# liulab-dfci/TRUST4

Measured on AMD Instinct MI355X. Metric: stage-1 assembly read pairs/sec (150 bp PE), whole stage 1, higher is better.
Workload: dtype int32/u64

## Files before the change

trust4_amd/build.py:

```python
import os
import subprocess
import sys

HERE = os.path.dirname(os.path.abspath(__file__))
SRC = os.path.join(HERE, "csrc", "t4_api.hip")
SRC_HOST = os.path.join(HERE, "csrc", "t4_assembler.cpp")
OUT = os.path.join(HERE, "libt4hip.so")
DEPS = [SRC, SRC_HOST, os.path.join(HERE, "host", "trust4_main.cpp"), os.path.join(HERE, "host", "fastq_extractor_main.cpp"),
        os.path.join(HERE, "host", "bam_extractor_main.cpp"), os.path.join(HERE, "host", "bam_reader.h"), os.path.join(HERE, "host", "read_format.h"),
        os.path.join(HERE, "host", "seq_reader.h"), os.path.join(HERE, "host", "process_read.h"), os.path.join(HERE, "csrc", "t4_internal.h"),
        os.path.join(HERE, "csrc", "t4_kernels.h"), os.path.join(HERE, "csrc", "t4_wide.h"), os.path.join(HERE, "csrc", "t4_device.h"),
        os.path.join(os.path.dirname(HERE), "include", "trust4_hip.h")]
FLAGS = ["--offload-arch=gfx950", "-O3", "-std=c++17", "-ffp-contract=off", "-fPIC", "-shared"]


def build(force=False, verbose=False):
    if not force and os.path.exists(OUT) and all(os.path.getmtime(OUT) >= os.path.getmtime(d) for d in DEPS):
        return OUT
    hipcc = os.environ.get("HIPCC", "/opt/rocm/bin/hipcc")
    cmd = [hipcc] + FLAGS + ["-o", OUT, SRC, SRC_HOST, "-lz", "-lpthread", "-ldl"]
    if verbose:
        print(" ".join(cmd))
    subprocess.run(cmd, check=True)
    build_driver(verbose)
    return OUT


def build_driver(verbose=False):
    out_dir = os.path.join(HERE, "bin")
    os.makedirs(out_dir, exist_ok=True)
    out = None
    for name, src in (("fastq-extractor-hip", "fastq_extractor_main.cpp"), ("bam-extractor-hip", "bam_extractor_main.cpp"), ("trust4-hip", "trust4_main.cpp")):
        out = os.path.join(out_dir, name)
        cmd = ["g++", "-O2", "-std=c++17", "-o", out, os.path.join(HERE, "host", src), "-L" + HERE, "-lt4hip", "-Wl,-rpath," + HERE,
               "-Wl,-rpath,$ORIGIN/..", "-lz", "-lpthread"]
        if verbose:
            print(" ".join(cmd))
        subprocess.run(cmd, check=True)
    return out


if __name__ == "__main__":
    build(force="--force" in sys.argv, verbose=True)
```

trust4_amd/csrc/t4_api.hip:

```cpp
#include <hip/hip_runtime.h>
#include <math.h>
#include <stdarg.h>
#include <stdio.h>
#include <string.h>
#include <zlib.h>

#include <algorithm>
#include <atomic>
#include <chrono>
#include <map>
#include <memory>
#include <mutex>
#include <string>
#include <thread>
#include <unordered_map>
#include <vector>

#ifdef __HIPCC__
#include <dlfcn.h>
#include <rccl/rccl.h>
#include <type_traits>
#include <unistd.h>
#endif
#include "../../include/trust4_hip.h"
#include "t4_kernels.h"
#include "t4_internal.h"

static_assert(sizeof(t4_overlap) == sizeof(T4OverlapOut), "overlap layout");
static_assert(sizeof(t4_hit) == sizeof(T4HitOut), "hit layout");
static_assert(sizeof(t4k::OvRec) == 40, "OvRec layout");
static_assert(sizeof(T4IndexView) % 16 == 0, "view stride");

namespace {

const int TIER_CAP[T4_NTIER - 1] = {1024, 2048, 3072, 4096, 8192};
const int TIER_THREADS[T4_NTIER] = {128, 256, 256, 256, 512, 512};
const int TIER_BLOCKS_PER_CU[T4_NTIER] = {8, 4, 3, 2, 1, 2};
const int G_CAP = 262144, G_MAXOV = 16384;
constexpr int G_THREADS = 512;

struct HostSeq {
  std::string name, cons;
  std::vector<int32_t> pw;
  int barcode;
  bool isRef;
};

}

struct AqCall {
  bool active = false;
  T4IndexView base; const T4IndexView *views = nullptr; bool hasViewOf = false, smallFirst = false, lean = false;
  int n = 0, skipRepeats = 0, wpk = 0, wnm = 0, attempt = 0, nFirst = 0, nDirect = 0, threads = 512;
  unsigned char *tierHint = nullptr;
  std::vector<unsigned char> allGlobal;
  size_t oPk, oNm, oLen, oBc, oSt, oLs, oVw, oFa, oOnly, oForce, oCs, oWide, oWideA, inBytes, pCb, pCc, pS8, pCnt, pSta, pNext, pNext2, pBase, pTick, pStab, pAux, pN4, pTail, pWctl, pWplan, pWstat, pWctlA, pWplanA, pWstatA, outBytes;
  bool hasOnly = false, hasForce = false, wantCands = false;
  bool keepExtAux = false;
  bool extendLater = false, wide = false, onlyRestricted = false;
  bool sweep2Done = false;
  int nWideSlots = 0;
  bool lazyDone = false, lazyStage = false;
  int wideSafety = 32;
  T4BatchView bv; T4QueryArgs qa; T4Work wk;
  std::chrono::steady_clock::time_point tf0;
};

struct t4_ctx {
  int device = 0, cus = 0;
  hipStream_t stream = 0;
  hipStream_t stream2 = 0;
  hipEvent_t evIn = 0, evG = 0;
  hipEvent_t ev[4] = {0, 0, 0, 0};
  std::string err;
  t4_stats stats;
  int maxGrid = 0;
  int *dpRows = nullptr;
  unsigned char *dpDir = nullptr;
  unsigned long long *gKeys = nullptr;
  unsigned *gPairs = nullptr, *gCand = nullptr;
  int *gOv = nullptr, *gFin = nullptr;
  unsigned short *gOrd = nullptr;
  int gGrid = 0;
  unsigned long long *hitsKeys = nullptr;
  int hitsGrid = 0;
  int *lists = nullptr, *listCounts = nullptr, *status = nullptr, *counts = nullptr;
  long long listCap = 0;
  unsigned long long *hitCounter = nullptr;
  T4OverlapOut *result = nullptr;
  size_t resultCap = 0, resultBytes = 0;
  int aqCap = 0, aqWpk = 0, aqWnm = 0, aqMax = 0;
  unsigned char *aqIn = nullptr, *aqOut = nullptr;
  unsigned char *aqInHost = nullptr, *aqOutHost = nullptr;
  unsigned char *aqInHostDev = nullptr, *aqOutHostDev = nullptr;
  unsigned *aqFlagHost = nullptr, *aqFlagDev = nullptr;
  unsigned *aqDoneCtr = nullptr;
  unsigned aqSeq = 0;
  size_t aqInBytes = 0, aqOutBytes = 0;
  unsigned char *aqPool = nullptr, *aqPoolDev = nullptr;
  int aqPoolCap = 0;
  unsigned char *candPool = nullptr; T4Cand *candPoolDev = nullptr;
  int candCap = 0, candGrows = 0;
  int64_t candRecords = 0;
  T4OverlapOut *aqRecDev = nullptr;
  int *aqRecRead = nullptr;
  int aqRecCap = 0;
  int *aqExtAux = nullptr;
  int aqExtAuxCap = 0;
  int64_t assignWide[2] = {0, 0};
  int64_t aqCalls = 0, aqReads = 0, aqGlobalLaunches = 0, aqGlobalReads = 0, aqRecords = 0;
  double aqSecPack = 0, aqSecFirst = 0, aqSecGlobal = 0;
  double aqSecLaunch[8] = {0, 0, 0, 0, 0, 0, 0, 0};
  int aqPoolGrows = 0;
  const int32_t *aqLastStable = nullptr;
  const int32_t *aqLastTicks = nullptr; int aqLastN = 0;
  double aqLastMs = 0;
  AqCall aq;
  uint64_t syncEpoch = 1;
  struct AqEnv {
    bool forceGlobal;
    int capLimit, extendDefer, poolCap, candCap, wideMinHits;
    AqEnv() {
      auto num = [](const char *n, int d) { const char *e = getenv(n); return e ? atoi(e) : d; };
      forceGlobal = getenv("T4_AQ_FORCE_GLOBAL") != nullptr;
      capLimit = num("T4_AQ_CAP_LIMIT", 0); poolCap = num("T4_AQ_POOL_CAP", 0); candCap = num("T4_AQ_CAND_CAP", 1 << 18);
      extendDefer = num("T4_AQ_EXTEND_DEFER", 16);
      wideMinHits = num("T4_WIDE_MIN_HITS", 3072);
    }
  } aqEnv;
  T4Wide wide;
  bool wideInit = false;
  unsigned char *grpPoolHost = nullptr;
  int64_t wideReads = 0, wideParts = 0, wideRetries = 0, wideGroups = 0;
  int64_t aqDeferredReads = 0;
  int64_t wideCalls = 0, wideCallsDeferred = 0, wideCallsDirect = 0;
  int wideSafetyKeep = 32, wideCallsSinceRepeat = 0;
  int64_t wideFlagCounts[6] = {0, 0, 0, 0, 0, 0};
  int wideRecentParts = 0;
  double aqKernelMs = 0;
  int64_t aqHits = 0;
};

struct t4_index {
  t4_ctx *ctx;
  int k, considerBarcode;
  int hitLenRequired = 31, radius = 10;
  double novelSim = 0.9, refSim = 0.75, repeatSim = 0.95;
  int nomatchGapLimit;
  std::vector<HostSeq> seqs;
  std::unordered_map<std::string, int> dedup;
  bool committed = false;
  uint2 *dTable = nullptr;
  T4HashEnt *dHtab = nullptr;
  int2 *dPost = nullptr;
  T4SeqInfo *dSeqs = nullptr;
  char *dCons = nullptr;
  T4PW *dPw = nullptr;
  T4IndexView view;
  bool live = false;
  T4HashEntC *dCtab = nullptr;
  int64_t capTable = 0, capPost = 0, capBase = 0;
  int capSeq = 0, liveNseq = 0;
  unsigned char *stHost = nullptr, *stDev = nullptr, *stHostDev = nullptr;
  size_t stCap = 0;
  hipEvent_t stEvent = 0;
  bool stPending = false;
  uint64_t stEpoch = 0;
};

struct t4_batch {
  t4_ctx *ctx;
  long long n = 0;
  int wpk = 0, wnm = 0, maxLen = 0;
  unsigned *dPk = nullptr, *dNm = nullptr;
  int *dLen = nullptr, *dBarcode = nullptr;
  T4BatchView view;
};

namespace {

int fail(t4_ctx *c, int code, const char *fmt, ...) {
  char buf[512];
  va_list ap;
  va_start(ap, fmt);
  vsnprintf(buf, sizeof buf, fmt, ap);
  va_end(ap);
  if (c) c->err = buf;
  return code;
}

#define HIPCHK(ctx, call)                                                                   \
  do {                                                                                      \
    hipError_t e_ = (call);                                                                 \
    if (e_ != hipSuccess) return fail((ctx), T4_ERR_HIP, "%s: %s", #call, hipGetErrorString(e_)); \
  } while (0)

template <class T> int devAlloc(t4_ctx *c, T **p, size_t count) {
  if (*p) { (void)hipFree(*p); *p = nullptr; }
  HIPCHK(c, hipMalloc(p, sizeof(T) * (count ? count : 1)));
  return T4_OK;
}
template <class T> struct DevBuf {
  T *p = nullptr;
  DevBuf() = default;
  DevBuf(DevBuf &&o) : p(o.p) { o.p = nullptr; }
  ~DevBuf() { if (p) (void)hipFree(p); }
  int alloc(t4_ctx *c, size_t count) { return devAlloc(c, &p, count); }
  operator T *() const { return p; }
};
template <class T> struct AsIs { typedef T type; };
template <class... P> void launch(void (*kernel)(P...), int grid, int block, hipStream_t stream, typename AsIs<P>::type... args) {
  hipLaunchKernelGGL(kernel, dim3(grid), dim3(block), 0, stream, args...);
}

int chainType(const char *n) {
  if (n[0] == 'I') { if (n[2] == 'H') return 0; if (n[2] == 'K') return 1; if (n[2] == 'L') return 2; }
  else if (n[0] == 'T') { if (n[2] == 'A') return 3; if (n[2] == 'B') return 4; if (n[2] == 'G') return 5; if (n[2] == 'D') return 6; }
  return 8;
}
// ... 118 lines not shown
  if (hipGetDeviceCount(&ndev) != hipSuccess || ndev <= 0 || device_ordinal < 0 || device_ordinal >= ndev) return T4_ERR_HIP;
  if (hipSetDevice(device_ordinal) != hipSuccess) return T4_ERR_HIP;
  t4_ctx *c = new t4_ctx();
  c->device = device_ordinal;
  hipDeviceProp_t prop;
  if (hipGetDeviceProperties(&prop, device_ordinal) != hipSuccess) { delete c; return T4_ERR_HIP; }
  c->cus = prop.multiProcessorCount;
  if (hipStreamCreate(&c->stream) != hipSuccess) { delete c; return T4_ERR_HIP; }
  for (int i = 0; i < 4; ++i) if (hipEventCreate(&c->ev[i]) != hipSuccess) { delete c; return T4_ERR_HIP; }
  memset(&c->stats, 0, sizeof c->stats);
  if (hipMalloc(&c->listCounts, sizeof(int) * 16) != hipSuccess || hipMalloc(&c->hitCounter, sizeof(unsigned long long)) != hipSuccess) { delete c; return T4_ERR_HIP; }
  if (hipHostMalloc(&c->aqFlagHost, 64, hipHostMallocMapped) != hipSuccess || hipHostGetDevicePointer((void **)&c->aqFlagDev, c->aqFlagHost, 0) != hipSuccess ||
      hipMalloc(&c->aqDoneCtr, sizeof(unsigned)) != hipSuccess || hipMemset(c->aqDoneCtr, 0, sizeof(unsigned)) != hipSuccess) { delete c; return T4_ERR_HIP; }
  *c->aqFlagHost = 0;
  *out = c;
  return T4_OK;
}

void t4_destroy(t4_ctx *c) {
  if (!c) return;
  (void)hipSetDevice(c->device);
#ifdef T4_PHASE_TIMING
  if (getenv("T4_PHASE_DUMP")) {
    unsigned long long ph[T4_NPHASE];
    if (hipMemcpyFromSymbol(ph, HIP_SYMBOL(t4k::g_phaseCycles), sizeof(ph)) == hipSuccess) {
      static const char *names[32] = {"other", "seed:lookup", "expand", "sort", "stats", "runs", "bigsort", "chain", "ovsort", "score", "prefilter", "final", "annotate", "score:quick", "score:banded", "score:finish", "extend:ungapped", "after-extend", "extend:list", "extend:dp4", "extend:dp1", "extend:combine", "seed:replay", "seed:scan", "extend:launch", "-", "-", "-", "-", "-", "-", "-"};
      unsigned long long tot = 0;
      for (int i = 0; i < T4_NPHASE; ++i) tot += ph[i];
      for (int i = 0; i < T4_NPHASE; ++i) if (ph[i]) fprintf(stderr, "phase %-16s %-7s %6.2f%%  %.3e cycles\n", names[i & 31], i < 32 ? "lds" : "global", 100.0 * (double)ph[i] / (double)tot, (double)ph[i]);
    }
    static unsigned long long cls[4 * T4_NPHASE];
    if (hipMemcpyFromSymbol(cls, HIP_SYMBOL(t4k::g_phaseByOverlaps), sizeof(cls)) == hipSuccess) {
      static const char *names[32] = {"other", "seed:lookup", "expand", "sort", "stats", "runs", "bigsort", "chain", "ovsort", "score", "prefilter", "final", "annotate", "score:quick", "score:banded", "score:finish", "extend:ungapped", "after-extend", "extend:list", "extend:dp4", "extend:dp1", "extend:combine", "seed:replay", "seed:scan", "extend:launch", "-", "-", "-", "-", "-", "-", "-"};
      static const char *cname[4] = {"<5 overlaps", "5-19 overlaps", "20-64 overlaps", ">64 overlaps"};
      for (int k = 0; k < 4; ++k) {
        unsigned long long tot = 0;
        for (int i = 0; i < T4_NPHASE; ++i) tot += cls[k * T4_NPHASE + i];
        if (!tot) continue;
        fprintf(stderr, "AddRead queries with %s: %.3e cycles in the query kernel\n", cname[k], (double)tot);
        for (int i = 0; i < T4_NPHASE; ++i) if (cls[k * T4_NPHASE + i] * 200 >= tot) fprintf(stderr, "   %-16s %-7s %6.2f%%\n", names[i & 31], i < 32 ? "lds" : "global", 100.0 * (double)cls[k * T4_NPHASE + i] / (double)tot);
      }
    }
    unsigned long long dc[8];
    if (hipMemcpyFromSymbol(dc, HIP_SYMBOL(t4k::g_dbgCount), sizeof(dc)) == hipSuccess)
      fprintf(stderr, "debug counters: gap jobs %llu, banded %llu, wave-DP steps %llu, scratch fallbacks %llu; overhang DPs %llu, of which %llu leave the diagonal\n", dc[0], dc[1], dc[2], dc[3], dc[6], dc[7]);
  }
#endif
  void *ptrs[] = {c->dpRows, c->dpDir, c->gKeys, c->gPairs, c->gCand, c->gOv, c->gFin, c->gOrd, c->hitsKeys, c->lists,
                  c->listCounts, c->status, c->counts, c->hitCounter, c->result, c->aqIn, c->aqOut};
  if (c->aqInHost) (void)hipHostFree(c->aqInHost);
  if (c->aqOutHost) (void)hipHostFree(c->aqOutHost);
  if (c->aqFlagHost) (void)hipHostFree(c->aqFlagHost);
  if (c->aqDoneCtr) (void)hipFree(c->aqDoneCtr);
  if (c->aqPool) (void)hipHostFree(c->aqPool);
  if (c->candPool) (void)hipHostFree(c->candPool);
  if (c->aqRecDev) (void)hipFree(c->aqRecDev);
  if (c->aqRecRead) (void)hipFree(c->aqRecRead);
  if (c->aqExtAux) (void)hipFree(c->aqExtAux);
  if (c->wideInit) {
    void *wp[] = {c->wide.seed, c->wide.bounds, c->wide.pCnt, c->wide.pRead, c->wide.pKeys, c->wide.gSize, c->wide.gInfo, c->wide.gCount, c->wide.gOff, c->wide.pRec,
                  c->wide.pRecCnt, c->wide.uniqPref, c->wide.mKeys, c->wide.mOrd, c->wide.sortTmp, c->wide.requeue};
    for (void *p : wp) if (p) (void)hipFree(p);
    if (c->grpPoolHost) (void)hipHostFree(c->grpPoolHost);
  }
  for (void *p : ptrs) if (p) (void)hipFree(p);
  for (int i = 0; i < 4; ++i) if (c->ev[i]) (void)hipEventDestroy(c->ev[i]);
  if (c->stream) (void)hipStreamDestroy(c->stream);
  if (c->stream2) (void)hipStreamDestroy(c->stream2);
  if (c->evIn) (void)hipEventDestroy(c->evIn);
  if (c->evG) (void)hipEventDestroy(c->evG);
  delete c;
}

int t4_sync(t4_ctx *c) {
  if (!c) return T4_ERR_ARG;
  HIPCHK(c, hipStreamSynchronize(c->stream));
  return T4_OK;
}
const char *t4_last_error(t4_ctx *c) { return c ? c->err.c_str() : "null ctx"; }
int t4_device_cus(t4_ctx *c) { return c ? c->cus : 0; }
int t4_ctx_device(t4_ctx *c) { return c ? c->device : 0; }
#ifdef T4_PHASE_TIMING
int t4_debug_phase_cycles(unsigned long long *out16) {
  unsigned long long zero[T4_NPHASE] = {0};
  if (hipMemcpyFromSymbol(out16, HIP_SYMBOL(t4k::g_phaseCycles), sizeof(zero)) != hipSuccess) return T4_ERR_HIP;
  if (hipMemcpyToSymbol(HIP_SYMBOL(t4k::g_phaseCycles), zero, sizeof(zero)) != hipSuccess) return T4_ERR_HIP;
  return T4_OK;
}
int t4_debug_counters(unsigned long long *out8) {
  unsigned long long zero[8] = {0};
  if (hipMemcpyFromSymbol(out8, HIP_SYMBOL(t4k::g_dbgCount), sizeof(zero)) != hipSuccess) return T4_ERR_HIP;
  if (hipMemcpyToSymbol(HIP_SYMBOL(t4k::g_dbgCount), zero, sizeof(zero)) != hipSuccess) return T4_ERR_HIP;
  return T4_OK;
}
#endif
int t4_debug_phase_reset(void) {
#ifdef T4_PHASE_TIMING
  unsigned long long zero[T4_NPHASE] = {0};
  if (hipMemcpyToSymbol(HIP_SYMBOL(t4k::g_phaseCycles), zero, sizeof(zero)) != hipSuccess) return T4_ERR_HIP;
#endif
  return T4_OK;
}
int t4_last_stats(t4_ctx *c, t4_stats *out) {
  if (!c || !out) return T4_ERR_ARG;
  *out = c->stats;
  return T4_OK;
// ... 209 lines not shown
    strncpy(nm, s.name.c_str(), 7);
    int gt = geneType(nm);
    f.geneType = gt < 0 ? 255 : (unsigned char)gt;
    f.name0 = (unsigned char)nm[0]; f.name1 = (unsigned char)nm[1]; f.name2 = (unsigned char)nm[2]; f.name3 = (unsigned char)nm[3];
    f.pwOff = -1;
    if (!s.isRef) {
      hasNovel = true;
      f.pwOff = (int)pw.size();
      for (int i = 0; i < f.len; ++i) pw.push_back(t4PwByte(s.pw[4 * i], s.pw[4 * i + 1], s.pw[4 * i + 2], s.pw[4 * i + 3]));
      pw.push_back(t4PwByte(0, 0, 0, 0));
    }
  }
  int r;
  void *old[] = {ix->dTable, ix->dHtab, ix->dPost, ix->dSeqs, ix->dCons, ix->dPw};
  for (void *p : old) if (p) (void)hipFree(p);
  ix->dTable = nullptr; ix->dHtab = nullptr; ix->dPost = nullptr; ix->dSeqs = nullptr; ix->dCons = nullptr; ix->dPw = nullptr;
  if ((r = devAlloc(c, &ix->dPost, post.size()))) return r;
  if ((r = devAlloc(c, &ix->dSeqs, infos.size()))) return r;
  if ((r = devAlloc(c, &ix->dCons, cons.size() + 16))) return r;
  if ((r = devAlloc(c, &ix->dPw, pw.size()))) return r;
  if (direct) { if ((r = devAlloc(c, &ix->dTable, table.size()))) return r; }
  else { if ((r = devAlloc(c, &ix->dHtab, htab.size()))) return r; }
  if (!post.empty()) HIPCHK(c, hipMemcpy(ix->dPost, post.data(), sizeof(int2) * post.size(), hipMemcpyHostToDevice));
  if (!infos.empty()) HIPCHK(c, hipMemcpy(ix->dSeqs, infos.data(), sizeof(T4SeqInfo) * infos.size(), hipMemcpyHostToDevice));
  if (!cons.empty()) HIPCHK(c, hipMemcpy(ix->dCons, cons.data(), cons.size(), hipMemcpyHostToDevice));
  if (!pw.empty()) HIPCHK(c, hipMemcpy(ix->dPw, pw.data(), sizeof(T4PW) * pw.size(), hipMemcpyHostToDevice));
  if (direct) HIPCHK(c, hipMemcpy(ix->dTable, table.data(), sizeof(uint2) * table.size(), hipMemcpyHostToDevice));
  else HIPCHK(c, hipMemcpy(ix->dHtab, htab.data(), sizeof(T4HashEnt) * htab.size(), hipMemcpyHostToDevice));
  T4IndexView &v = ix->view;
  memset(&v, 0, sizeof v);
  v.k = K; v.nseq = (int)ix->seqs.size(); v.direct = direct ? 1 : 0; v.considerBarcode = ix->considerBarcode;
  v.hashMask = hashMask; v.table = ix->dTable; v.htab = ix->dHtab; v.post = ix->dPost; v.seqs = ix->dSeqs;
  v.cons = ix->dCons; v.pw = ix->dPw;
  v.radius = ix->radius; v.hitLenRequired = ix->hitLenRequired; v.nomatchGapLimit = ix->nomatchGapLimit;
  v.firstIsRef = (!ix->seqs.empty() && ix->seqs[0].isRef) ? 1 : 0;
  for (const HostSeq &q : ix->seqs) if (q.isRef) { hasRef = true; break; }
  v.hasNovel = hasNovel ? (hasRef ? 1 : 2) : 0;
  { int maxLen = 0; for (const HostSeq &q : ix->seqs) if ((int)q.cons.size() > maxLen) maxLen = (int)q.cons.size(); v.key32 = t4Key32Bits(v.nseq, maxLen); }
  v.novelSim = ix->novelSim; v.refSim = ix->refSim; v.repeatSim = ix->repeatSim;
  ix->committed = true;
  return T4_OK;
}
}

namespace {
template <class T> int growKeep(t4_ctx *c, T **p, int64_t keep, int64_t want) {
  T *np = nullptr;
  HIPCHK(c, hipMalloc(&np, sizeof(T) * (size_t)(want > 0 ? want : 1)));
  if (*p && keep > 0) HIPCHK(c, hipMemcpyAsync(np, *p, sizeof(T) * (size_t)keep, hipMemcpyDeviceToDevice, c->stream));
  if (*p) { HIPCHK(c, hipStreamSynchronize(c->stream)); (void)hipFree(*p); }
  *p = np;
  return T4_OK;
}
}

extern "C" {

int t4_index_apply_delta(t4_index *ix, const t4_index_delta *d) {
  if (!ix || !d) return T4_ERR_ARG;
  t4_ctx *c = ix->ctx;
  (void)hipSetDevice(c->device);
  if (ix->considerBarcode) return fail(c, T4_ERR_ARG, "t4_index_apply_delta: the index of a live set is not keyed by barcode");
  if (!ix->live && (!ix->seqs.empty() || ix->committed)) return fail(c, T4_ERR_STATE, "t4_index_apply_delta on an index that was filled through t4_index_add_*");
  if (d->table_slots < 2 || (d->table_slots & (d->table_slots - 1))) return fail(c, T4_ERR_ARG, "table_slots must be a power of two");
  if (d->nseq < 0 || d->nseq > T4_MAX_SEQS) return fail(c, T4_ERR_UNSUPPORTED, "more than %d sequences", T4_MAX_SEQS);
  if (d->max_seq_len > T4_MAX_SEQLEN) return fail(c, T4_ERR_UNSUPPORTED, "contig longer than %d", T4_MAX_SEQLEN);
  if (d->post_cap > 0xFFFFFFFFll) return fail(c, T4_ERR_UNSUPPORTED, "more than 2^32 postings");
  int r;
  if (!ix->stEvent) HIPCHK(c, hipEventCreate(&ix->stEvent));
  if (d->table_slots != ix->capTable || d->table_rebuilt) {
    if (d->table_slots != ix->capTable) {
      if (ix->dCtab) { HIPCHK(c, hipStreamSynchronize(c->stream)); (void)hipFree(ix->dCtab); ix->dCtab = nullptr; }
      HIPCHK(c, hipMalloc(&ix->dCtab, sizeof(T4HashEntC) * (size_t)d->table_slots));
      ix->capTable = d->table_slots;
    }
    HIPCHK(c, hipMemsetAsync(ix->dCtab, 0xFF, sizeof(T4HashEntC) * (size_t)ix->capTable, c->stream));
  }
  if (d->post_cap > ix->capPost) { int64_t want = d->post_cap + d->post_cap / 2; if ((r = growKeep(c, &ix->dPost, ix->capPost, want))) return r; ix->capPost = want; }
  if (d->seq_cap > ix->capSeq) { int want = d->seq_cap + d->seq_cap / 2; if ((r = growKeep(c, &ix->dSeqs, (int64_t)ix->capSeq, (int64_t)want))) return r; ix->capSeq = want; }
  if (d->base_cap > ix->capBase) {
    int64_t want = d->base_cap + d->base_cap / 2;
    if ((r = growKeep(c, &ix->dCons, ix->capBase, want))) return r;
    if ((r = growKeep(c, &ix->dPw, ix->capBase, want))) return r;
    ix->capBase = want;
  }
  auto al8 = [](size_t x) { return (x + 7) & ~(size_t)7; };
  int64_t postTotal = 0, baseTotal = 0;
  for (int64_t i = 0; i < d->n_post_runs; ++i) {
    if (d->post_at[i] < 0 || d->post_len[i] < 0 || d->post_at[i] + d->post_len[i] > ix->capPost) return fail(c, T4_ERR_ARG, "posting run %lld outside the image", (long long)i);
    postTotal += d->post_len[i];
  }
  for (int64_t i = 0; i < d->n_base_runs; ++i) {
    if (d->base_at[i] < 0 || d->base_len[i] < 0 || d->base_at[i] + d->base_len[i] > ix->capBase) return fail(c, T4_ERR_ARG, "base run %lld outside the image", (long long)i);
    baseTotal += d->base_len[i];
  }
  const size_t nDesc = (size_t)d->n_slots + (size_t)d->n_post_runs + (size_t)d->n_seqs + 2 * (size_t)d->n_base_runs;
  if (nDesc == 0) goto view;
  {
    size_t bytes = al8(sizeof(T4CopyDesc) * nDesc) + sizeof(T4HashEntC) * (size_t)d->n_slots + 8 * (size_t)postTotal + al8(sizeof(T4SeqInfo)) * (size_t)d->n_seqs;
    for (int64_t i = 0; i < d->n_base_runs; ++i) bytes += 2 * al8((size_t)d->base_len[i]);
    if (ix->stPending && ix->stEpoch == c->syncEpoch) { HIPCHK(c, hipStreamSynchronize(c->stream)); ++c->syncEpoch; }
    ix->stPending = false;
    if (bytes > ix->stCap) {
      if (ix->stHost) (void)hipHostFree(ix->stHost);
      if (ix->stDev) { HIPCHK(c, hipStreamSynchronize(c->stream)); (void)hipFree(ix->stDev); }
      ix->stHost = nullptr; ix->stDev = nullptr;
      ix->stCap = bytes * 2 > ((size_t)1 << 20) ? bytes * 2 : ((size_t)1 << 20);
      HIPCHK(c, hipHostMalloc(&ix->stHost, ix->stCap, hipHostMallocMapped));
      HIPCHK(c, hipHostGetDevicePointer((void **)&ix->stHostDev, ix->stHost, 0));
      HIPCHK(c, hipMalloc(&ix->stDev, ix->stCap));
    }
    T4CopyDesc *desc = (T4CopyDesc *)ix->stHost;
    size_t at = al8(sizeof(T4CopyDesc) * nDesc), nd = 0;
    for (int64_t i = 0; i < d->n_slots; ++i) {
      if (d->slot[i] < 0 || d->slot[i] >= ix->capTable) return fail(c, T4_ERR_ARG, "table slot %lld outside the table", (long long)d->slot[i]);
      T4HashEntC e; e.code = d->slot_code[i]; e.start = d->slot_start[i]; e.cnt = d->slot_cnt[i];
      memcpy(ix->stHost + at, &e, sizeof e);
      desc[nd].srcOff = at; desc[nd].dst = (unsigned char *)(ix->dCtab + d->slot[i]); desc[nd].bytes = sizeof e; ++nd;
      at += sizeof e;
    }
    int64_t pAt = 0;
    for (int64_t i = 0; i < d->n_post_runs; ++i) {
      const size_t b = 8 * (size_t)d->post_len[i];
      memcpy(ix->stHost + at, d->post_data + 2 * pAt, b);
      desc[nd].srcOff = at; desc[nd].dst = (unsigned char *)(ix->dPost + d->post_at[i]); desc[nd].bytes = b; ++nd;
      at += b; pAt += d->post_len[i];
    }
    for (int i = 0; i < d->n_seqs; ++i) {
      const int id = d->seq_id[i];
      if (id < 0 || id >= ix->capSeq || id >= d->nseq) return fail(c, T4_ERR_ARG, "sequence id %d outside the image", id);
      const t4_seq_record &q = d->seq[i];
      if (q.len < 0 || q.base_off < 0 || q.base_off + q.len + 1 > ix->capBase || q.base_off > 0x7FFFFFFFll) return fail(c, T4_ERR_ARG, "sequence %d outside the base arena", id);
      T4SeqInfo f;
      memset(&f, 0, sizeof f);
      f.consOff = (int)q.base_off; f.len = q.len; f.pwOff = (int)q.base_off; f.barcode = q.barcode; f.isRef = 0;
      char nm[9] = {0, 0, 0, 0, 0, 0, 0, 0, 0};
      memcpy(nm, q.name, 8);
      const int gt = geneType(nm);
      f.geneType = gt < 0 ? 255 : (unsigned char)gt;
      f.name0 = (unsigned char)nm[0]; f.name1 = (unsigned char)nm[1]; f.name2 = (unsigned char)nm[2]; f.name3 = (unsigned char)nm[3];
      memset(ix->stHost + at, 0, al8(sizeof f));
      memcpy(ix->stHost + at, &f, sizeof f);
      desc[nd].srcOff = at; desc[nd].dst = (unsigned char *)(ix->dSeqs + id); desc[nd].bytes = sizeof f; ++nd;
      at += al8(sizeof f);
    }
    int64_t bAt = 0;
    for (int64_t i = 0; i < d->n_base_runs; ++i) {
      const size_t b = (size_t)d->base_len[i];
      memcpy(ix->stHost + at, d->base_cons + bAt, b);
      desc[nd].srcOff = at; desc[nd].dst = (unsigned char *)(ix->dCons + d->base_at[i]); desc[nd].bytes = b; ++nd;
      at += al8(b);
      memcpy(ix->stHost + at, d->base_pw + bAt, b);
      desc[nd].srcOff = at; desc[nd].dst = (unsigned char *)(ix->dPw + d->base_at[i]); desc[nd].bytes = b; ++nd;
      at += al8(b);
      bAt += d->base_len[i];
    }
    const bool direct = at <= ((size_t)1 << 18);
    if (!direct) HIPCHK(c, hipMemcpyAsync(ix->stDev, ix->stHost, at, hipMemcpyHostToDevice, c->stream));
    ix->stPending = true; ix->stEpoch = c->syncEpoch;
    int grid = (int)((nd + 3) / 4);
    if (grid > c->cus * 8) grid = c->cus * 8;
    const unsigned char *stg = direct ? ix->stHostDev : ix->stDev;
    hipLaunchKernelGGL(t4k::deltaKernel, dim3(grid), dim3(256), 0, c->stream, stg, (const T4CopyDesc *)stg, (int)nd);
    HIPCHK(c, hipGetLastError());
  }
view:
  ix->live = true; ix->committed = true; ix->liveNseq = d->nseq;
  T4IndexView &v = ix->view;
  memset(&v, 0, sizeof v);
  v.k = ix->k; v.nseq = d->nseq; v.direct = 3; v.considerBarcode = 0;
  v.hashMask = (unsigned long long)ix->capTable - 1; v.ctab = ix->dCtab; v.post = ix->dPost; v.seqs = ix->dSeqs; v.cons = ix->dCons; v.pw = ix->dPw;
  v.radius = ix->radius; v.hitLenRequired = ix->hitLenRequired; v.nomatchGapLimit = ix->nomatchGapLimit;
  v.firstIsRef = 0; v.hasNovel = 2;
  v.key32 = t4Key32Bits(d->nseq, d->max_seq_len);
  v.novelSim = ix->novelSim; v.refSim = ix->refSim; v.repeatSim = ix->repeatSim;
  return T4_OK;
}

int t4_index_size(const t4_index *ix) { return ix ? (ix->live ? ix->liveNseq : (int)ix->seqs.size()) : 0; }
int t4_index_seq_len(const t4_index *ix, int i) { return (ix && i >= 0 && i < (int)ix->seqs.size()) ? (int)ix->seqs[i].cons.size() : -1; }
const char *t4_index_seq_name(const t4_index *ix, int i) { return (ix && i >= 0 && i < (int)ix->seqs.size()) ? ix->seqs[i].name.c_str() : nullptr; }
const char *t4_index_seq_consensus(const t4_index *ix, int i) { return (ix && i >= 0 && i < (int)ix->seqs.size()) ? ix->seqs[i].cons.c_str() : nullptr; }

int t4_reads_upload(t4_ctx *c, const char *bases, const int64_t *offsets, const int32_t *barcode, int64_t n, t4_batch **out) {
  return t4_reads_upload_flags(c, bases, offsets, barcode, n, 0, out);
}

int t4_reads_upload_flags(t4_ctx *c, const char *bases, const int64_t *offsets, const int32_t *barcode, int64_t n, int flags, t4_batch **out) {
  if (!c || !out || n < 0 || (n > 0 && (!bases || !offsets))) return T4_ERR_ARG;
  *out = nullptr;
  (void)hipSetDevice(c->device);
  int maxLen = 0;
  for (int64_t i = 0; i < n; ++i) {
    int64_t l = offsets[i + 1] - offsets[i];
    if (l < 0) return fail(c, T4_ERR_ARG, "offsets not monotone at read %lld", (long long)i);
    if (l > T4_MAXL) return fail(c, T4_ERR_UNSUPPORTED, "read %lld is %lld bp; this engine takes reads up to %d bp", (long long)i, (long long)l, T4_MAXL);
    if (l > maxLen) maxLen = (int)l;
  }
  std::unique_ptr<t4_batch, void (*)(t4_batch *)> b(new t4_batch(), t4_batch_destroy);
  b->ctx = c; b->n = n; b->maxLen = maxLen;
  b->wpk = (maxLen + 15) / 16; b->wnm = (maxLen + 31) / 32;
  if (b->wpk == 0) b->wpk = 1;
  if (b->wnm == 0) b->wnm = 1;
  std::vector<unsigned> pk((size_t)n * b->wpk, 0u), nm((size_t)n * b->wnm, 0u);
  std::vector<int> len((size_t)n);
  std::atomic<long long> badRead(-1);
  auto packRange = [&](int64_t lo, int64_t hi) {
    for (int64_t i = lo; i < hi; ++i) {
      const char *s = bases + offsets[i];
      int l = (int)(offsets[i + 1] - offsets[i]);
      len[i] = l;
      unsigned *p = pk.data() + (size_t)i * b->wpk, *m = nm.data() + (size_t)i * b->wnm;
      for (int j = 0; j < l; ++j) {
        int v = nucNum(s[j]);
        if (v < 0) {
          if (s[j] == 'N') { m[j >> 5] |= 1u << (j & 31); v = 0; }
          else if ((flags & T4_READS_KMERS_ONLY) && s[j] >= 'A' && s[j] <= 'Z') v = 3;
          else { long long none = -1; badRead.compare_exchange_strong(none, (long long)i); return; }
        }
        p[j >> 4] |= (unsigned)v << ((j & 15) * 2);
      }
    }
  };
  {
    const int packThreads = getenv("T4_PACK_THREADS") ? atoi(getenv("T4_PACK_THREADS")) : 8;
    const long long packMin = getenv("T4_PACK_MIN") ? atoll(getenv("T4_PACK_MIN")) : 65536;
    int nt = n >= packMin ? packThreads : 1;
    const unsigned hw = std::thread::hardware_concurrency();
    if (hw > 0 && (unsigned)nt > hw) nt = (int)hw;
    if (nt <= 1) packRange(0, n);
    else {
      std::vector<std::thread> pool;
      for (int t = 0; t < nt; ++t) pool.emplace_back(packRange, n * t / nt, n * (t + 1) / nt);
      for (auto &th : pool) th.join();
    }
  }
  if (badRead.load() >= 0) {
    const long long i = badRead.load();
    char bad = '?';
    for (int64_t j = offsets[i]; j < offsets[i + 1]; ++j) { const char ch = bases[j]; if (nucNum(ch) < 0 && ch != 'N' && !((flags & T4_READS_KMERS_ONLY) && ch >= 'A' && ch <= 'Z')) { bad = ch; break; } }
    return fail(c, T4_ERR_UNSUPPORTED, "read %lld has base '%c' (alphabet is ACGTN)", i, bad);
  }
  int r;
  if ((r = devAlloc(c, &b->dPk, pk.size() + 4)) || (r = devAlloc(c, &b->dNm, nm.size() + 4)) || (r = devAlloc(c, &b->dLen, len.size()))) return r;
  if (n > 0) {
    HIPCHK(c, hipMemcpy(b->dPk, pk.data(), sizeof(unsigned) * pk.size(), hipMemcpyHostToDevice));
    HIPCHK(c, hipMemcpy(b->dNm, nm.data(), sizeof(unsigned) * nm.size(), hipMemcpyHostToDevice));
    HIPCHK(c, hipMemcpy(b->dLen, len.data(), sizeof(int) * len.size(), hipMemcpyHostToDevice));
  }
  if (barcode) {
    if ((r = devAlloc(c, &b->dBarcode, (size_t)n))) return r;
    if (n > 0) HIPCHK(c, hipMemcpy(b->dBarcode, barcode, sizeof(int) * (size_t)n, hipMemcpyHostToDevice));
  }
  b->view.pk = b->dPk; b->view.nm = b->dNm; b->view.len = b->dLen; b->view.barcode = b->dBarcode;
  b->view.wpk = b->wpk; b->view.wnm = b->wnm; b->view.n = n;
  *out = b.release();
  return T4_OK;
}

void t4_batch_destroy(t4_batch *b) {
  if (!b) return;
  void *ptrs[] = {b->dPk, b->dNm, b->dLen, b->dBarcode};
  for (void *p : ptrs) if (p) (void)hipFree(p);
  delete b;
}
int64_t t4_batch_size(const t4_batch *b) { return b ? b->n : 0; }

}

namespace {

template <int CAP, int MAXOV, int NT>
void launchTier(int grid, hipStream_t st, const T4IndexView &iv, const T4BatchView &bv, const T4Work &wk, const T4QueryArgs &qa) {
  if (qa.views) hipLaunchKernelGGL((t4k::queryKernel<CAP, MAXOV, NT, 2>), dim3(grid), dim3(NT), 0, st, iv, bv, wk, qa);
  else if (qa.mode == 5) hipLaunchKernelGGL((t4k::queryKernel<CAP, MAXOV, NT, 3>), dim3(grid), dim3(NT), 0, st, iv, bv, wk, qa);
  else if (qa.mode >= 2 && qa.mode <= 4) hipLaunchKernelGGL((t4k::queryKernel<CAP, MAXOV, NT, 1>), dim3(grid), dim3(NT), 0, st, iv, bv, wk, qa);
  else hipLaunchKernelGGL((t4k::queryKernel<CAP, MAXOV, NT, 0>), dim3(grid), dim3(NT), 0, st, iv, bv, wk, qa);
}

int runQuery(t4_index *ix, t4_batch *b, T4QueryArgs qa, bool useBarcode, bool noHits = false, std::vector<int> *statusOut = nullptr) {
  t4_ctx *c = ix->ctx;
  if (!ix->committed) return fail(c, T4_ERR_STATE, "index not committed");
  if (b->ctx != c) return fail(c, T4_ERR_ARG, "batch belongs to another ctx");
  (void)hipSetDevice(c->device);
  const long long n = b->n;
  memset(&c->stats, 0, sizeof c->stats);
  c->stats.reads = n;
  if (n == 0) return T4_OK;
  int r;
  int grids[T4_NTIER];
  int maxGrid = 1;
  for (int t = 0; t < T4_NTIER; ++t) {
    grids[t] = c->cus * TIER_BLOCKS_PER_CU[t];
    if (grids[t] * TIER_THREADS[t] > maxGrid) maxGrid = grids[t] * TIER_THREADS[t];
  }
  if ((r = ensureScratch(c, maxGrid))) return r;
  if ((r = ensurePerCall(c, n))) return r;
  HIPCHK(c, hipMemsetAsync(c->listCounts, 0, sizeof(int) * 16, c->stream));
  HIPCHK(c, hipMemsetAsync(c->status, 0, sizeof(int) * (size_t)n, c->stream));
  HIPCHK(c, hipMemsetAsync(c->hitCounter, 0, sizeof(unsigned long long), c->stream));
  HIPCHK(c, hipEventRecord(c->ev[0], c->stream));
  T4TierCaps caps;
  for (int t = 0; t < T4_NTIER - 1; ++t) caps.cap[t] = TIER_CAP[t];
  if (noHits) caps.cap[0] = 1 << 30;
  int binGrid = c->cus * 8;
  if ((long long)binGrid > n) binGrid = (int)n;
  hipLaunchKernelGGL(t4k::binKernel, dim3(binGrid), dim3(64), 0, c->stream, ix->view, b->view, useBarcode ? 1 : 0,
                     caps, c->lists, c->listCounts, (long long)n);
  HIPCHK(c, hipGetLastError());
  HIPCHK(c, hipEventRecord(c->ev[1], c->stream));
  c->stats.launches = 1;
  int hostCounts[8];
  for (int t = 0; t < T4_NTIER; ++t) {
    HIPCHK(c, hipMemcpyAsync(hostCounts, c->listCounts, sizeof(int) * 8, hipMemcpyDeviceToHost, c->stream));
    HIPCHK(c, hipStreamSynchronize(c->stream));
    int cnt = hostCounts[t];
    c->stats.tier_reads[t] = cnt;
    if (cnt == 0) continue;
    T4Work wk;
    memset(&wk, 0, sizeof wk);
    wk.list = c->lists + (size_t)t * n; wk.nList = cnt;
    wk.nextList = t + 1 < T4_NTIER ? c->lists + (size_t)(t + 1) * n : nullptr;
    wk.nextCount = t + 1 < T4_NTIER ? c->listCounts + (t + 1) : nullptr;
    wk.workNext = getenv("T4_STATIC_STRIDE") ? nullptr : c->listCounts + 8 + t;
    wk.status = c->status; wk.hitCounter = c->hitCounter;
    wk.dpRows = c->dpRows; wk.dpDir = c->dpDir;
    int grid = grids[t] < cnt ? grids[t] : cnt;
    if (t == T4_NTIER - 1) {
      if ((r = ensureGlobalTier(c, grids[T4_NTIER - 1]))) return r;
      wk.gKeys = c->gKeys; wk.gPairs = c->gPairs; wk.gCand = c->gCand; wk.gOv = c->gOv; wk.gFin = c->gFin; wk.gOrd = c->gOrd;
      wk.gCap = G_CAP; wk.gMaxOv = G_MAXOV;
      launchTier<0, 0, G_THREADS>(grid, c->stream, ix->view, b->view, wk, qa);
    }
    else if (t == 0) launchTier<1024, 64, 128>(grid, c->stream, ix->view, b->view, wk, qa);
    else if (t == 1) launchTier<2048, 128, 256>(grid, c->stream, ix->view, b->view, wk, qa);
// ... 17 lines not shown
  for (long long i = 0; i < n; ++i)
    if (status[i] != 0)
      return fail(c, T4_ERR_UNSUPPORTED, "read %lld exceeds the engine limits (status %d: %s)", i, status[i],
                  status[i] == 2 ? "more than 262144 k-mer hits or 16384 overlaps" : "a posting list beyond 10000 entries, or gap DP or contig count beyond scratch");
  return T4_OK;
}

int ensureResult(t4_ctx *c, size_t records) {
  if (records <= c->resultCap) return T4_OK;
  c->resultCap = 0;
  int r = devAlloc(c, &c->result, records);
  if (r) return r;
  c->resultCap = records;
  return T4_OK;
}

}

extern "C" {

int t4_overlaps(t4_index *ix, t4_batch *b, int strand, int skip_repeats, int max_per_read, int32_t *counts, t4_overlap *out) {
  if (!ix || !b || max_per_read <= 0) return T4_ERR_ARG;
  t4_ctx *c = ix->ctx;
  int r;
  if ((r = ensurePerCall(c, b->n))) return r;
  if ((r = ensureResult(c, (size_t)b->n * max_per_read))) return r;
  T4QueryArgs qa;
  memset(&qa, 0, sizeof qa);
  qa.mode = 0; qa.strand = strand; qa.skipRepeats = skip_repeats; qa.maxPerRead = max_per_read;
  qa.counts = c->counts; qa.out = c->result;
  if ((r = runQuery(ix, b, qa, true))) return r;
  if (counts && b->n) HIPCHK(c, hipMemcpy(counts, c->counts, sizeof(int) * (size_t)b->n, hipMemcpyDeviceToHost));
  if (out && b->n) HIPCHK(c, hipMemcpy(out, c->result, sizeof(t4_overlap) * (size_t)b->n * max_per_read, hipMemcpyDeviceToHost));
  return T4_OK;
}

int t4_annotate_rough(t4_index *ref, t4_batch *b, t4_overlap *out) {
  if (!ref || !b) return T4_ERR_ARG;
  t4_ctx *c = ref->ctx;
  int r;
  if ((r = ensureResult(c, (size_t)b->n * 4))) return r;
  T4QueryArgs qa;
  memset(&qa, 0, sizeof qa);
  qa.mode = 1; qa.strand = 0; qa.skipRepeats = 0; qa.maxPerRead = 4; qa.counts = nullptr; qa.out = c->result;
  if ((r = runQuery(ref, b, qa, false))) return r;
  if (out && b->n) HIPCHK(c, hipMemcpy(out, c->result, sizeof(t4_overlap) * (size_t)b->n * 4, hipMemcpyDeviceToHost));
  return T4_OK;
}

int t4_hits(t4_index *ix, t4_batch *b, int strand, int allow_total_skip, int64_t *hit_offsets, t4_hit *hits, int64_t hits_cap) {
  if (!ix || !b || !hit_offsets) return T4_ERR_ARG;
  t4_ctx *c = ix->ctx;
  if (!ix->committed) return fail(c, T4_ERR_STATE, "index not committed");
  (void)hipSetDevice(c->device);
  const long long n = b->n;
  hit_offsets[0] = 0;
  if (n == 0) return T4_OK;
  int r;
  int grid = c->cus * 2;
  if ((long long)grid > n) grid = (int)n;
  const int HCAP = 65536;
  if (grid > c->hitsGrid) { c->hitsGrid = 0; if ((r = devAlloc(c, &c->hitsKeys, (size_t)grid * HCAP))) return r; c->hitsGrid = grid; }
  if ((r = ensurePerCall(c, n))) return r;
  DevBuf<long long> dOff;
  DevBuf<T4HitOut> dHits;
  if ((r = dOff.alloc(c, (size_t)n + 1))) return r;
  HIPCHK(c, hipMemsetAsync(c->status, 0, sizeof(int) * (size_t)n, c->stream));
  launch(t4k::hitsKernel, grid, 64, c->stream, ix->view, b->view, strand, allow_total_skip, 0, dOff,
                     (T4HitOut *)nullptr, c->hitsKeys, HCAP, c->status);
  HIPCHK(c, hipGetLastError());
  std::vector<long long> off((size_t)n + 1);
  HIPCHK(c, hipMemcpyAsync(off.data(), dOff, sizeof(long long) * ((size_t)n + 1), hipMemcpyDeviceToHost, c->stream));
  HIPCHK(c, hipStreamSynchronize(c->stream));
  off[0] = 0;
  for (long long i = 0; i < n; ++i) off[i + 1] += off[i];
  for (long long i = 0; i <= n; ++i) hit_offsets[i] = off[i];
  std::vector<int> status((size_t)n);
  HIPCHK(c, hipMemcpy(status.data(), c->status, sizeof(int) * (size_t)n, hipMemcpyDeviceToHost));
  for (long long i = 0; i < n; ++i) if (status[i]) return fail(c, T4_ERR_UNSUPPORTED, "read %lld has more than %d hits", i, HCAP);
  if (hits) {
    if (hits_cap < off[n]) return fail(c, T4_ERR_ARG, "hits_cap %lld < %lld", (long long)hits_cap, off[n]);
    if ((r = dHits.alloc(c, (size_t)off[n]))) return r;
    HIPCHK(c, hipMemcpyAsync(dOff, off.data(), sizeof(long long) * ((size_t)n + 1), hipMemcpyHostToDevice, c->stream));
    launch(t4k::hitsKernel, grid, 64, c->stream, ix->view, b->view, strand, allow_total_skip, 1, dOff,
                       dHits, c->hitsKeys, HCAP, c->status);
    HIPCHK(c, hipGetLastError());
    if (off[n]) HIPCHK(c, hipMemcpyAsync(hits, dHits, sizeof(t4_hit) * (size_t)off[n], hipMemcpyDeviceToHost, c->stream));
    HIPCHK(c, hipStreamSynchronize(c->stream));
  }
  return T4_OK;
}


int t4_gap_dp_align(t4_ctx *c, int kind, int impl, int n, const int64_t *t_off, const int64_t *p_off, const void *t_data,
                    const char *p_chars, int32_t *out4, signed char *align, int align_stride);
int t4_gap_dp(t4_ctx *c, int kind, int impl, int n, const int64_t *t_off, const int64_t *p_off, const void *t_data,
              const char *p_chars, int32_t *out4) {
  return t4_gap_dp_align(c, kind, impl, n, t_off, p_off, t_data, p_chars, out4, nullptr, 0);
}
int t4_gap_dp_align(t4_ctx *c, int kind, int impl, int n, const int64_t *t_off, const int64_t *p_off, const void *t_data,
                    const char *p_chars, int32_t *out4, signed char *align, int align_stride) {
  if (!c || n < 0 || (n > 0 && (!t_off || !p_off || !t_data || !p_chars || !out4)) || (kind != 0 && kind != 1)) return T4_ERR_ARG;
  if (align && (align_stride < 2 || impl != 4 || kind != 1)) return T4_ERR_ARG;
  if (n == 0) return T4_OK;
  (void)hipSetDevice(c->device);
  int grid = (n + 63) / 64;
// ... 350 lines not shown

int t4_assign(t4_index *ix, t4_batch *b, int strand, int32_t *ret, t4_overlap *out) {
  if (!ix || !b) return T4_ERR_ARG;
  t4_ctx *c = ix->ctx;
  if (ix->committed && ix->view.firstIsRef) return fail(c, T4_ERR_UNSUPPORTED, "t4_assign needs a contig set (ExtendOverlap aligns against posWeight)");
  int r;
  if ((r = ensurePerCall(c, b->n))) return r;
  if ((r = ensureResult(c, (size_t)b->n))) return r;
  T4QueryArgs qa;
  memset(&qa, 0, sizeof qa);
  qa.mode = 2; qa.strand = strand; qa.skipRepeats = 0; qa.maxPerRead = 1; qa.counts = nullptr; qa.out = c->result; qa.ret = c->counts;
  if ((r = runQuery(ix, b, qa, true))) return r;
  if (ret && b->n) HIPCHK(c, hipMemcpy(ret, c->counts, sizeof(int) * (size_t)b->n, hipMemcpyDeviceToHost));
  if (out && b->n) HIPCHK(c, hipMemcpy(out, c->result, sizeof(t4_overlap) * (size_t)b->n, hipMemcpyDeviceToHost));
  return T4_OK;
}

int t4_assign_strands(t4_index *ix, t4_batch *b, const int32_t *strands, int32_t *ret, t4_overlap *out) {
  if (!ix || !b || (b->n > 0 && !strands)) return T4_ERR_ARG;
  t4_ctx *c = ix->ctx;
  if (ix->committed && ix->view.firstIsRef) return fail(c, T4_ERR_UNSUPPORTED, "t4_assign_strands needs a contig set (ExtendOverlap aligns against posWeight)");
  if (b->n == 0) return T4_OK;
  (void)hipSetDevice(c->device);
  int r;
  if ((r = ensurePerCall(c, b->n))) return r;
  if ((r = ensureResult(c, (size_t)b->n))) return r;
  DevBuf<int> dSt;
  if ((r = dSt.alloc(c, (size_t)b->n))) return r;
  HIPCHK(c, hipMemcpy(dSt, strands, sizeof(int) * (size_t)b->n, hipMemcpyHostToDevice));
  T4QueryArgs qa;
  memset(&qa, 0, sizeof qa);
  qa.mode = 2; qa.strand = 0; qa.strandPerRead = dSt; qa.skipRepeats = 0; qa.maxPerRead = 1; qa.counts = nullptr; qa.out = c->result; qa.ret = c->counts;
  if ((r = runQuery(ix, b, qa, true))) return r;
  if (ret) HIPCHK(c, hipMemcpy(ret, c->counts, sizeof(int) * (size_t)b->n, hipMemcpyDeviceToHost));
  if (out) HIPCHK(c, hipMemcpy(out, c->result, sizeof(t4_overlap) * (size_t)b->n, hipMemcpyDeviceToHost));
  return T4_OK;
}

}

namespace {
int assignWidePass2(t4_index *ix, t4_batch *b, const std::vector<int64_t> &todo, int strand, const int32_t *strands, int32_t *ret, t4_overlap *out);
const int ASSIGN_WIDE_BATCH = 256;
}

extern "C" {

int t4_assign_wide(t4_index *ix, t4_batch *b, int strand, const int32_t *strands, int32_t *ret, t4_overlap *out) {
  if (!ix || !b) return T4_ERR_ARG;
  t4_ctx *c = ix->ctx;
  c->assignWide[0] = c->assignWide[1] = 0;
  if (ix->committed && ix->view.firstIsRef) return fail(c, T4_ERR_UNSUPPORTED, "t4_assign_wide needs a contig set (ExtendOverlap aligns against posWeight)");
  if (!ix->committed) return fail(c, T4_ERR_STATE, "index not committed");
  if (b->ctx != c) return fail(c, T4_ERR_ARG, "batch belongs to another ctx");
  if (c->aq.active) return fail(c, T4_ERR_STATE, "an AddRead query is already in flight on this ctx");
  if (b->n == 0) return T4_OK;
  (void)hipSetDevice(c->device);
  const size_t n = (size_t)b->n;
  std::vector<int64_t> todo;
  if (getenv("T4_ASSIGN_WIDE_ALL")) {
    todo.resize(n);
    for (size_t i = 0; i < n; ++i) todo[i] = (int64_t)i;
  } else {
    int r;
    if ((r = ensurePerCall(c, b->n))) return r;
    if ((r = ensureResult(c, n))) return r;
    DevBuf<int> dSt;
    if (strands) {
      if ((r = dSt.alloc(c, n))) return r;
      HIPCHK(c, hipMemcpy(dSt, strands, sizeof(int) * n, hipMemcpyHostToDevice));
    }
    T4QueryArgs qa;
    memset(&qa, 0, sizeof qa);
    qa.mode = 2; qa.strand = strands ? 0 : strand; qa.strandPerRead = strands ? (const int *)dSt : nullptr; qa.skipRepeats = 0; qa.maxPerRead = 1;
    qa.counts = nullptr; qa.out = c->result; qa.ret = c->counts;
    std::vector<int> status;
    if ((r = runQuery(ix, b, qa, true, false, &status))) return r;
    if (ret) HIPCHK(c, hipMemcpy(ret, c->counts, sizeof(int) * n, hipMemcpyDeviceToHost));
    if (out) HIPCHK(c, hipMemcpy(out, c->result, sizeof(t4_overlap) * n, hipMemcpyDeviceToHost));
    for (size_t i = 0; i < n; ++i) if (status[i] != 0) todo.push_back((int64_t)i);
  }
  c->assignWide[0] = (int64_t)(n - todo.size()); c->assignWide[1] = (int64_t)todo.size();
  if (todo.empty()) return T4_OK;
  return assignWidePass2(ix, b, todo, strand, strands, ret, out);
}

int t4_assign_wide_stats(t4_ctx *c, int64_t *out2) {
  if (!c || !out2) return T4_ERR_ARG;
  out2[0] = c->assignWide[0]; out2[1] = c->assignWide[1];
  return T4_OK;
}

int t4_posweight_recompute(t4_index *ix, t4_batch *b, const t4_overlap *assign, const int32_t *mult, int32_t *posweight, int64_t posweight_cap) {
  return t4_consensus_recompute(ix, b, assign, mult, posweight, posweight_cap, nullptr, 0, nullptr);
}

int t4_consensus_recompute(t4_index *ix, t4_batch *b, const t4_overlap *assign, const int32_t *mult, int32_t *posweight, int64_t posweight_cap,
                           char *consensus, int64_t consensus_cap, int64_t *changed) {
  if (!ix || !b || (b->n > 0 && !assign) || !posweight) return T4_ERR_ARG;
  t4_ctx *c = ix->ctx;
  if (!ix->committed) return fail(c, T4_ERR_STATE, "index not committed");
  if (ix->live) return fail(c, T4_ERR_UNSUPPORTED, "t4_posweight_recompute takes a committed contig set (the extendedSeq of main.cpp:2047), not a live one");
  if (b->ctx != c) return fail(c, T4_ERR_ARG, "batch belongs to another ctx");
  int64_t bases = 0;
  for (const HostSeq &q : ix->seqs) { if (q.isRef) return fail(c, T4_ERR_UNSUPPORTED, "t4_posweight_recompute needs a contig set"); bases += (int64_t)q.cons.size(); }
  if (posweight_cap < 4 * bases) return fail(c, T4_ERR_ARG, "posweight buffer holds %lld values, the set needs %lld", (long long)posweight_cap, (long long)(4 * bases));
  if (consensus && consensus_cap < bases) return fail(c, T4_ERR_ARG, "consensus buffer holds %lld bases, the set has %lld", (long long)consensus_cap, (long long)bases);
  if (changed) *changed = 0;
  if (bases == 0) return T4_OK;
  (void)hipSetDevice(c->device);
  int r;
  DevBuf<int> dCnt, dMult;
  DevBuf<T4OverlapOut> dAs;
  DevBuf<char> dCons;
  DevBuf<unsigned long long> dChanged;
  const size_t n = (size_t)b->n;
  const size_t cols = (size_t)bases + ix->seqs.size();
  if ((r = dCnt.alloc(c, cols * 4))) return r;
  HIPCHK(c, hipMemsetAsync(dCnt, 0, sizeof(int) * cols * 4, c->stream));
  if (n > 0) {
    if ((r = dAs.alloc(c, n))) return r;
    HIPCHK(c, hipMemcpyAsync(dAs, assign, sizeof(t4_overlap) * n, hipMemcpyHostToDevice, c->stream));
    if (mult) {
      if ((r = dMult.alloc(c, n))) return r;
      HIPCHK(c, hipMemcpyAsync(dMult, mult, sizeof(int) * n, hipMemcpyHostToDevice, c->stream));
    }
    const int grid = (int)(n < (size_t)c->cus * 32 ? n : (size_t)c->cus * 32);
    launch(t4k::posWeightAccumulateKernel, grid, 64, c->stream, ix->view, b->view, (const T4OverlapOut *)dAs, (const int *)dMult, dCnt);
    HIPCHK(c, hipGetLastError());
  }
  {
    const int nseq = (int)ix->seqs.size();
    const int grid = nseq < c->cus * 8 ? nseq : c->cus * 8;
    launch(t4k::posWeightFinishKernel, grid > 0 ? grid : 1, 256, c->stream, ix->view, dCnt);
    HIPCHK(c, hipGetLastError());
  }
  std::vector<char> allCons;
  unsigned long long nChanged = 0;
  if (consensus) {
    if ((r = dCons.alloc(c, cols))) return r;
    if ((r = dChanged.alloc(c, 1))) return r;
    HIPCHK(c, hipMemsetAsync(dChanged, 0, sizeof(unsigned long long), c->stream));
    const int nseq = (int)ix->seqs.size();
    const int grid = nseq < c->cus * 8 ? nseq : c->cus * 8;
    launch(t4k::consensusArgmaxKernel, grid > 0 ? grid : 1, 256, c->stream, ix->view, (const int *)dCnt, dCons, dChanged);
    HIPCHK(c, hipGetLastError());
    allCons.resize(cols);
    HIPCHK(c, hipMemcpyAsync(allCons.data(), dCons, cols, hipMemcpyDeviceToHost, c->stream));
    HIPCHK(c, hipMemcpyAsync(&nChanged, dChanged, sizeof nChanged, hipMemcpyDeviceToHost, c->stream));
  }
  std::vector<int32_t> all(cols * 4);
  HIPCHK(c, hipMemcpyAsync(all.data(), dCnt, sizeof(int) * cols * 4, hipMemcpyDeviceToHost, c->stream));
  HIPCHK(c, hipStreamSynchronize(c->stream));
  if (changed) *changed = (int64_t)nChanged;
  {
    size_t from = 0, to = 0;
    for (const HostSeq &q : ix->seqs) {
      const size_t ln = q.cons.size();
      if (ln) memcpy(posweight + 4 * to, all.data() + 4 * from, sizeof(int32_t) * 4 * ln);
      if (ln && consensus) memcpy(consensus + to, allCons.data() + from, ln);
      from += ln + 1; to += ln;
    }
  }
  return T4_OK;
}

int t4_extend(t4_index *ix, t4_batch *b, int max_per_read, const int32_t *counts, const t4_overlap *in, double mismatch_factor,
              int32_t *ret, t4_overlap *out) {
  if (!ix || !b || max_per_read <= 0 || (b->n > 0 && (!counts || !in))) return T4_ERR_ARG;
  t4_ctx *c = ix->ctx;
  if (ix->committed && ix->view.firstIsRef) return fail(c, T4_ERR_UNSUPPORTED, "t4_extend needs a contig set (ExtendOverlap aligns against posWeight)");
  if (max_per_read > 128) return fail(c, T4_ERR_UNSUPPORTED, "t4_extend takes at most 128 overlaps per read");
  const size_t n = (size_t)b->n, m = n * max_per_read;
  if (n == 0) return T4_OK;
  (void)hipSetDevice(c->device);
  int r;
  if ((r = ensurePerCall(c, b->n))) return r;
  if ((r = ensureResult(c, m))) return r;
  DevBuf<T4OverlapOut> dIn;
  DevBuf<int> dCnt, dRet;
  if ((r = dIn.alloc(c, m)) || (r = dCnt.alloc(c, n)) || (r = dRet.alloc(c, m))) return r;
  HIPCHK(c, hipMemcpy(dIn, in, sizeof(t4_overlap) * m, hipMemcpyHostToDevice));
  HIPCHK(c, hipMemcpy(dCnt, counts, sizeof(int) * n, hipMemcpyHostToDevice));
  HIPCHK(c, hipMemset(dRet, 0, sizeof(int) * m));
  T4QueryArgs qa;
  memset(&qa, 0, sizeof qa);
  qa.mode = 3; qa.maxPerRead = max_per_read; qa.out = c->result; qa.in = dIn; qa.inCounts = dCnt; qa.ret = dRet; qa.mismatchFactor = mismatch_factor;
  if ((r = runQuery(ix, b, qa, true, true))) return r;
  if (ret) HIPCHK(c, hipMemcpy(ret, dRet, sizeof(int) * m, hipMemcpyDeviceToHost));
  if (out) HIPCHK(c, hipMemcpy(out, c->result, sizeof(t4_overlap) * m, hipMemcpyDeviceToHost));
  return T4_OK;
}

}

namespace {
struct AqResult { const int32_t *counts, *base; const t4_overlap *ov, *ext; const int32_t *ret; };
int aqLaunch(t4_ctx *c);
int aqBegin(t4_ctx *c, const T4IndexView &base, const T4IndexView *views, const int32_t *viewOf, bool smallFirst, int n, const char *bases,
            const int64_t *offsets, const int32_t *barcodes, const int32_t *strands, int skip_repeats, const double *factors,
            unsigned char *tierHint = nullptr, bool lean = false, const int32_t *onlySeq = nullptr, const int32_t *forceMin = nullptr, int wantCands = 0) {
  (void)hipSetDevice(c->device);
  AqCall &q = c->aq;
  if (q.active) return fail(c, T4_ERR_STATE, "an AddRead query is already in flight on this ctx");
  int maxLen = 1;
  for (int i = 0; i < n; ++i) {
    int64_t l = offsets[i + 1] - offsets[i];
    if (l < 0 || l > T4_MAXL) return fail(c, T4_ERR_UNSUPPORTED, "read %d is %lld bp; this engine takes reads up to %d bp", i, (long long)l, T4_MAXL);
    if (l > maxLen) maxLen = (int)l;
  }
  q.lean = lean;
  q.base = base; q.views = views; q.hasViewOf = viewOf != nullptr; q.smallFirst = smallFirst; q.n = n; q.skipRepeats = skip_repeats; q.tierHint = tierHint; q.attempt = 0;
  const int wpk = (maxLen + 15) / 16, wnm = (maxLen + 31) / 32;
  q.wpk = wpk; q.wnm = wnm;
  auto al8 = [](size_t x) { return (x + 7) & ~(size_t)7; };
  q.oPk = 0; q.oNm = al8(q.oPk + sizeof(unsigned) * (size_t)n * wpk); q.oLen = al8(q.oNm + sizeof(unsigned) * (size_t)n * wnm);
  q.oBc = al8(q.oLen + sizeof(int) * (size_t)n); q.oSt = al8(q.oBc + sizeof(int) * (size_t)n); q.oLs = al8(q.oSt + sizeof(int) * (size_t)n);
  q.oVw = al8(q.oLs + sizeof(int) * (size_t)n); q.oFa = al8(q.oVw + sizeof(int) * (size_t)n); q.oOnly = al8(q.oFa + sizeof(double) * (size_t)n);
  q.oForce = al8(q.oOnly + sizeof(int) * (size_t)n);
  q.oCs = al8(q.oForce + sizeof(int) * (size_t)n);
  q.oWide = al8(q.oCs + sizeof(T4CandArgs)); q.hasOnly = onlySeq != nullptr; q.hasForce = forceMin != nullptr; q.wantCands = (wantCands & 1) != 0; q.keepExtAux = (wantCands & 2) != 0;
  q.oWideA = al8(q.oWide + sizeof(T4Wide)); q.inBytes = al8(q.oWideA + sizeof(T4Wide));
  q.pCnt = 0; q.pSta = al8(q.pCnt + sizeof(int) * (size_t)n); q.pNext = al8(q.pSta + sizeof(int) * (size_t)n);
  q.pNext2 = al8(q.pNext + sizeof(int) * (size_t)n); q.pBase = al8(q.pNext2 + sizeof(int) * (size_t)n);
  q.pTick = al8(q.pBase + sizeof(int) * (size_t)n); q.pStab = al8(q.pTick + sizeof(int) * (size_t)n); q.pAux = al8(q.pStab + sizeof(int) * (size_t)n);
  q.pN4 = al8(q.pAux + sizeof(int) * (size_t)n); q.pCb = al8(q.pN4 + sizeof(int) * (size_t)n); q.pCc = al8(q.pCb + sizeof(int) * (size_t)n);
  q.pS8 = al8(q.pCc + sizeof(int) * (size_t)n); q.pTail = al8(q.pS8 + sizeof(int) * T4_QSTATS * (size_t)n);
  const size_t nW = (size_t)n * (skip_repeats ? 2 : 1);
  q.nWideSlots = (int)nW;
  q.pWctl = q.pTail + 48; q.pWplan = q.pWctl + 32; q.pWstat = al8(q.pWplan + sizeof(T4WidePlan) * nW);
  q.pWctlA = al8(q.pWstat + sizeof(int) * T4_WIDE_STAT * nW); q.pWplanA = q.pWctlA + 32; q.pWstatA = al8(q.pWplanA + sizeof(T4WidePlan) * nW);
  q.outBytes = al8(q.pWstatA + sizeof(int) * T4_WIDE_STAT * nW);
  q.wideSafety = c->wideSafetyKeep;
  if (q.inBytes > c->aqInBytes) {
    if (c->aqIn) (void)hipFree(c->aqIn);
    if (c->aqInHost) (void)hipHostFree(c->aqInHost);
    c->aqIn = nullptr; c->aqInHost = nullptr;
    HIPCHK(c, hipMalloc(&c->aqIn, q.inBytes * 2));
    HIPCHK(c, hipHostMalloc(&c->aqInHost, q.inBytes * 2, hipHostMallocMapped));
    HIPCHK(c, hipHostGetDevicePointer((void **)&c->aqInHostDev, c->aqInHost, 0));
    c->aqInBytes = q.inBytes * 2;
  }
  if (q.outBytes > c->aqOutBytes) {
    if (c->aqOut) (void)hipFree(c->aqOut);
    if (c->aqOutHost) (void)hipHostFree(c->aqOutHost);
    c->aqOut = nullptr; c->aqOutHost = nullptr;
    HIPCHK(c, hipMalloc(&c->aqOut, q.outBytes * 2));
    HIPCHK(c, hipHostMalloc(&c->aqOutHost, q.outBytes * 2, hipHostMallocMapped));
    HIPCHK(c, hipHostGetDevicePointer((void **)&c->aqOutHostDev, c->aqOutHost, 0));
    c->aqOutBytes = q.outBytes * 2;
  }
  auto tNow = [] { return std::chrono::steady_clock::now(); };
  auto tSince = [](std::chrono::steady_clock::time_point t0) { return std::chrono::duration<double>(std::chrono::steady_clock::now() - t0).count(); };
  auto tp0 = tNow();
  unsigned char *h = c->aqInHost;
  memset(h, 0, q.inBytes);
  unsigned *pk = (unsigned *)(h + q.oPk), *nm = (unsigned *)(h + q.oNm);
  int *len = (int *)(h + q.oLen), *bc = (int *)(h + q.oBc), *st = (int *)(h + q.oSt), *ls = (int *)(h + q.oLs), *vw = (int *)(h + q.oVw);
  double *fa = (double *)(h + q.oFa);
  for (int i = 0; i < n; ++i) {
    const char *s = bases + offsets[i];
    int l = (int)(offsets[i + 1] - offsets[i]);
    len[i] = l; bc[i] = barcodes ? barcodes[i] : -1; st[i] = strands[i]; fa[i] = factors[i]; vw[i] = viewOf ? viewOf[i] : 0;
    ((int *)(h + q.oOnly))[i] = onlySeq ? onlySeq[i] : -1;
    ((int *)(h + q.oForce))[i] = forceMin ? forceMin[i] : 0;
    unsigned *p = pk + (size_t)i * wpk, *qn = nm + (size_t)i * wnm;
    for (int j = 0; j < l; ++j) {
      int v = nucNum(s[j]);
      if (v < 0) {
        if (s[j] != 'N') return fail(c, T4_ERR_UNSUPPORTED, "read %d has base '%c' (alphabet is ACGTN)", i, s[j]);
        qn[j >> 5] |= 1u << (j & 31); v = 0;
      }
      p[j >> 4] |= (unsigned)v << ((j & 15) * 2);
    }
  }
  q.wide = !views && !smallFirst && base.hasNovel == 2 && !getenv("T4_WIDE_OFF");
  q.onlyRestricted = false;
  if (onlySeq) {
    bool anyWhole = false;
    for (int i = 0; i < n && !anyWhole; ++i) anyWhole = onlySeq[i] < 0;
    if (!anyWhole) { q.wide = false; q.onlyRestricted = !views && !smallFirst; }
  }
  const bool forceGlobal = c->aqEnv.forceGlobal;
  if (forceGlobal && !smallFirst) { q.allGlobal.assign((size_t)n, 1); q.tierHint = tierHint = q.allGlobal.data(); q.wide = false; }
  auto direct = [&](int i) { return tierHint && tierHint[i] && !smallFirst && !(onlySeq && onlySeq[i] >= 0) && !(q.wide && base.considerBarcode && barcodes && barcodes[i] != -1); };
  int nFirst = 0, nDirect = 0;
  for (int i = 0; i < n; ++i) if (!direct(i)) ls[nFirst++] = i;
  for (int i = 0; i < n; ++i) if (direct(i)) ls[nFirst + nDirect++] = i;
  q.nFirst = nFirst; q.nDirect = nDirect;
  c->aqSecPack += tSince(tp0);
  const int r = aqLaunch(c);
  if (r == T4_OK) q.active = true;
  return r;
}

void aqLaunchDeferredWide(t4_ctx *c) {
  AqCall &q = c->aq;
  T4Wide w;
  memcpy(&w, c->aqInHost + q.oWide, sizeof w);
  const int cus = c->cus > 0 ? c->cus : 1;
  auto clampi = [](int v, int lo, int hi) { return v < lo ? lo : v > hi ? hi : v; };
  const int *ctl = (const int *)(c->aqOutHost + q.pWctl);
  const int gParts = clampi(ctl[1] + 1, 4, cus * 2), gReads = clampi(ctl[0], 1, cus < 64 ? cus : 64);
  hipLaunchKernelGGL(t4k::wideScatterKernel, dim3(clampi(8 * gParts, 16, cus * 8)), dim3(256), 0, c->stream, q.base, w);
  hipLaunchKernelGGL((t4k::wideSortKernel<8192>), dim3(gParts), dim3(512), 0, c->stream, q.base, w);
  hipLaunchKernelGGL(t4k::wideStatsKernel, dim3(gReads), dim3(512), 0, c->stream, q.base, w);
  hipLaunchKernelGGL((t4k::wideChainKernel<8192, 1 << T4_WIDE_OVBITS>), dim3(gParts < cus ? gParts : cus), dim3(512), 0, c->stream, q.base, q.bv, q.wk, q.qa, w);
  hipLaunchKernelGGL(t4k::wideMergeKernel, dim3(gReads), dim3(512), 0, c->stream, q.base, q.bv, q.wk, q.qa, w);
}
int aqLaunchEpilogue(t4_ctx *c) {
  AqCall &q = c->aq;
  const unsigned long long outW = q.outBytes >> 3;
  int grid = (int)((outW + 4095) / 4096);
  if (grid < 1) grid = 1;
  if (grid > 64) grid = 64;
  ++c->aqSeq;
  if (c->aqSeq == 0) c->aqSeq = 1;
  hipLaunchKernelGGL(t4k::aqEpilogueKernel, dim3(grid), dim3(256), 0, c->stream, (const unsigned long long *)c->aqOut, (unsigned long long *)c->aqOutHostDev, outW,
                     c->aqDoneCtr, c->aqFlagDev, c->aqSeq);
  HIPCHK(c, hipGetLastError());
  return T4_OK;
}

int aqLaunch(t4_ctx *c) {
  AqCall &q = c->aq;
  const int n = q.n, nFirst = q.nFirst, nDirect = q.nDirect;
  const bool smallFirst = q.smallFirst;
  int r;
  if (!c->aqPool) {
    const int poolCap0 = c->aqEnv.poolCap;
    if (!c->aqPoolCap) c->aqPoolCap = poolCap0 > 0 ? poolCap0 : 1 << 16;
    const size_t rec = (size_t)c->aqPoolCap;
    HIPCHK(c, hipHostMalloc(&c->aqPool, rec * (2 * sizeof(t4_overlap) + sizeof(int32_t)), hipHostMallocMapped));
    HIPCHK(c, hipHostGetDevicePointer((void **)&c->aqPoolDev, c->aqPool, 0));
  }
  const size_t rec = (size_t)c->aqPoolCap;
  if (q.wantCands && !c->candPool) {
    if (!c->candCap) c->candCap = c->aqEnv.candCap > 0 ? c->aqEnv.candCap : 1 << 18;
    HIPCHK(c, hipHostMalloc(&c->candPool, sizeof(T4Cand) * (size_t)c->candCap, hipHostMallocMapped));
    HIPCHK(c, hipHostGetDevicePointer((void **)&c->candPoolDev, c->candPool, 0));
  }
  q.tf0 = std::chrono::steady_clock::now();
  auto tl_ = q.tf0;
  auto lapL = [&](int i) { const auto t = std::chrono::steady_clock::now(); c->aqSecLaunch[i] += std::chrono::duration<double>(t - tl_).count(); tl_ = t; };
  if (q.wide) {
    if ((r = ensureWide(c, q.nWideSlots, 1, 1))) return r;
    T4Wide w = wideHalf(c, 0), wa = wideHalf(c, 1);
    w.enabled = 1; w.safetyNum = q.wideSafety; w.firstRead = w.firstPart = 0;
    { const int lim = c->aqEnv.capLimit; w.minHits = lim > 0 ? lim : c->aqEnv.wideMinHits; }
    w.ctl = (int *)(c->aqOut + q.pWctl); w.plan = (T4WidePlan *)(c->aqOut + q.pWplan); w.stat = (int *)(c->aqOut + q.pWstat);
    memcpy(c->aqInHost + q.oWide, &w, sizeof w);
    wa.enabled = 1; wa.safetyNum = w.safetyNum; wa.minHits = w.minHits; wa.firstRead = wa.firstPart = 0;
    wa.ctl = (int *)(c->aqOut + q.pWctlA); wa.plan = (T4WidePlan *)(c->aqOut + q.pWplanA); wa.stat = (int *)(c->aqOut + q.pWstatA);
    memcpy(c->aqInHost + q.oWideA, &wa, sizeof wa);
  }
  {
    T4CandArgs cs;
    memset(&cs, 0, sizeof cs);
    cs.stats8 = (int *)(c->aqOut + q.pS8);
    if (q.hasForce) cs.forceMin = (const int *)(c->aqIn + q.oForce);
    if (q.keepExtAux) {
      if (c->aqExtAuxCap < c->aqPoolCap) {
        c->aqExtAuxCap = 0;
        if ((r = devAlloc(c, &c->aqExtAux, (size_t)c->aqPoolCap))) return r;
        c->aqExtAuxCap = c->aqPoolCap;
      }
      cs.extAux = c->aqExtAux;
    }
    if (q.wantCands) {
      cs.candOut = c->candPoolDev; cs.candCap = c->candCap; cs.candCursor = (unsigned *)(c->aqOut + q.pTail + 32); cs.candOverflow = (int *)(c->aqOut + q.pTail + 36);
      cs.candBase = (int *)(c->aqOut + q.pCb); cs.candCnt = (int *)(c->aqOut + q.pCc);
    }
    memcpy(c->aqInHost + q.oCs, &cs, sizeof cs);
  }
  lapL(0);
  {
    const unsigned long long inW = q.inBytes >> 3, outW = q.outBytes >> 3;
    const unsigned long long most = inW > outW ? inW : outW;
// ... 67 lines not shown
    if (q.wide) {
      T4Wide wa;
      memcpy(&wa, c->aqInHost + q.oWideA, sizeof wa);
      const int cus = c->cus > 0 ? c->cus : 1;
      auto clampi = [](int v, int lo, int hi) { return v < lo ? lo : v > hi ? hi : v; };
      const int gParts = clampi(2 * c->wideRecentParts + 4 * nDirect + 4, 4, cus * 2), gReads = clampi(nDirect, 1, cus < 64 ? cus : 64);
      hipLaunchKernelGGL(t4k::wideSeedKernel, dim3(nDirect < cus ? nDirect : cus), dim3(512), 0, c->stream2, q.base, bv, wd, qa, wa, wd.list, nDirect, q.skipRepeats ? 1 : 0);
      hipLaunchKernelGGL(t4k::wideScatterKernel, dim3(clampi(8 * gParts, 16, cus * 8)), dim3(256), 0, c->stream2, q.base, wa);
      hipLaunchKernelGGL((t4k::wideSortKernel<8192>), dim3(gParts), dim3(512), 0, c->stream2, q.base, wa);
      hipLaunchKernelGGL(t4k::wideStatsKernel, dim3(gReads), dim3(512), 0, c->stream2, q.base, wa);
      hipLaunchKernelGGL((t4k::wideChainKernel<8192, 1 << T4_WIDE_OVBITS>), dim3(gParts < cus ? gParts : cus), dim3(512), 0, c->stream2, q.base, bv, wd, qa, wa);
      hipLaunchKernelGGL(t4k::wideMergeKernel, dim3(gReads), dim3(512), 0, c->stream2, q.base, bv, wd, qa, wa);
    } else {
      wd.gKeys = c->gKeys; wd.gPairs = c->gPairs; wd.gCand = c->gCand; wd.gOv = c->gOv; wd.gFin = c->gFin; wd.gOrd = c->gOrd;
      wd.gCap = G_CAP; wd.gMaxOv = G_MAXOV;
      launchTier<0, 0, G_THREADS>(nDirect, c->stream2, q.base, bv, wd, qa);
      ++c->aqGlobalLaunches; c->aqGlobalReads += nDirect;
    }
    HIPCHK(c, hipGetLastError());
    HIPCHK(c, hipEventRecord(c->evG, c->stream2));
  }
  lapL(2);
  if (nFirst > 0) {
    if (smallFirst) launchTier<1024, 128, 256>(grid0, c->stream, q.base, bv, wk, qa);
    else {
      T4Work wf = wk;
      const size_t skip = q.wide ? 0 : (size_t)nDirect;
      wf.gKeys = c->gKeys + skip * G_CAP; wf.gPairs = c->gPairs + skip * G_CAP * 2; wf.gCand = c->gCand;
      wf.gOv = c->gOv + skip * G_MAXOV * 10; wf.gFin = c->gFin + skip * G_MAXOV * 10; wf.gOrd = c->gOrd + skip * G_MAXOV;
      wf.gCap = G_CAP; wf.gMaxOv = G_MAXOV;
      launchTier<8192, 512, 512>(grid0, c->stream, q.base, bv, wf, qa);
    }
    HIPCHK(c, hipGetLastError());
  }
  lapL(3);
  if (nDirect > 0 && !q.wide) HIPCHK(c, hipStreamWaitEvent(c->stream, c->evG, 0));
  q.lazyDone = false; q.lazyStage = false; q.sweep2Done = false;
  if (q.wide) {
    if (nDirect > 0) HIPCHK(c, hipStreamWaitEvent(c->stream, c->evG, 0));
  }
  if (extendLater) {
    const int grid = c->cus * 16;
    hipLaunchKernelGGL(t4k::extendKernel, dim3(grid), dim3(64), 0, c->stream, q.base, bv, qa, 0);
    HIPCHK(c, hipGetLastError());
  }
  lapL(4);
  HIPCHK(c, hipEventRecord(c->ev[1], c->stream));
  lapL(5);
  r = aqLaunchEpilogue(c);
  lapL(6);
  return r;
}

int aqWait(t4_ctx *c) {
  const unsigned want = c->aqSeq;
  for (unsigned long long spin = 1;; ++spin) {
    if (__atomic_load_n(c->aqFlagHost, __ATOMIC_ACQUIRE) == want) return T4_OK;
    if ((spin & 0xFFFFull) == 0) {
      const hipError_t e = hipStreamQuery(c->stream);
      if (e == hipSuccess) {
        if (__atomic_load_n(c->aqFlagHost, __ATOMIC_ACQUIRE) == want) return T4_OK;
        return fail(c, T4_ERR_HIP, "the stream of an AddRead query call is idle but its epilogue never reported (word %u, expected %u)", *c->aqFlagHost, want);
      }
      if (e != hipErrorNotReady) return fail(c, T4_ERR_HIP, "AddRead query call: %s", hipGetErrorString(e));
    }
  }
}

int aqDone(t4_ctx *c) {
  if (!c->aq.active) return 1;
  return __atomic_load_n(c->aqFlagHost, __ATOMIC_ACQUIRE) == c->aqSeq ? 1 : 0;
}

int aqEnd(t4_ctx *c, AqResult *res) {
  AqCall &q = c->aq;
  if (!q.active) return fail(c, T4_ERR_STATE, "no AddRead query in flight on this ctx");
  q.active = false;
  (void)hipSetDevice(c->device);
  auto tNow = [] { return std::chrono::steady_clock::now(); };
  auto tSince = [](std::chrono::steady_clock::time_point t0) { return std::chrono::duration<double>(std::chrono::steady_clock::now() - t0).count(); };
  const int n = q.n;
  const bool smallFirst = q.smallFirst;
  const size_t pTail = q.pTail, pNext = q.pNext, pNext2 = q.pNext2, outBytes = q.outBytes;
  T4Work &wk = q.wk;
  T4QueryArgs &qa = q.qa;
  T4BatchView &bv = q.bv;
  int r;
  for (;;) {
    if ((r = aqWait(c))) return r;
    if ((c->aqSeq & 255u) == 0) HIPCHK(c, hipStreamSynchronize(c->stream));
    ++c->syncEpoch;
    {
      float ms = 0;
      hipError_t ee = hipEventElapsedTime(&ms, c->ev[0], c->ev[1]);
      if (ee == hipErrorNotReady) { (void)hipEventSynchronize(c->ev[1]); ee = hipEventElapsedTime(&ms, c->ev[0], c->ev[1]); }
      if (ee == hipSuccess) { c->aqKernelMs += ms; c->aqLastMs = q.lazyStage ? c->aqLastMs + ms : ms; }
    }
    if (q.wide && !q.lazyDone) {
      q.lazyDone = true;
      const int *ctl0 = (const int *)(c->aqOutHost + q.pWctl);
      if (ctl0[0] > 0 && !ctl0[2] && !*(const int *)(c->aqOutHost + q.pWctlA + 8)) {
        const int recsBefore = (int)*(const unsigned *)(c->aqOutHost + pTail + 24);
        q.lazyStage = true;
        HIPCHK(c, hipEventRecord(c->ev[0], c->stream));
        aqLaunchDeferredWide(c);
        HIPCHK(c, hipGetLastError());
        if (q.extendLater) {
          hipLaunchKernelGGL(t4k::extendKernel, dim3(c->cus * 16), dim3(64), 0, c->stream, q.base, bv, qa, recsBefore < c->aqPoolCap ? recsBefore : c->aqPoolCap);
          HIPCHK(c, hipGetLastError());
        }
        HIPCHK(c, hipEventRecord(c->ev[1], c->stream));
        if ((r = aqLaunchEpilogue(c))) return r;
        continue;
      }
    }
    if (q.wide && q.skipRepeats && !q.sweep2Done) {
      q.sweep2Done = true;
      const int *ctl0 = (const int *)(c->aqOutHost + q.pWctl), *ctlA0 = (const int *)(c->aqOutHost + q.pWctlA);
      const int nq0 = ctl0[4], nqA = ctlA0[4];
      if (nq0 + nqA > 0 && !ctl0[2] && !ctlA0[2]) {
        T4Wide w, wa;
        memcpy(&w, c->aqInHost + q.oWide, sizeof w);
        memcpy(&wa, c->aqInHost + q.oWideA, sizeof wa);
        const int *list0 = w.requeue, *listA = wa.requeue;
        w.firstRead = ctl0[0]; w.firstPart = ctl0[1];
        const int recsBefore = (int)*(const unsigned *)(c->aqOutHost + pTail + 24);
        const int cus = c->cus > 0 ? c->cus : 1;
        auto clampi = [](int v, int lo, int hi) { return v < lo ? lo : v > hi ? hi : v; };
        const int nq = nq0 + nqA;
        const int gParts = clampi(2 * c->wideRecentParts + 4 * nq + 4, 4, cus * 2), gReads = clampi(nq, 1, cus < 64 ? cus : 64);
        q.lazyStage = true;
        HIPCHK(c, hipEventRecord(c->ev[0], c->stream));
        if (nq0 > 0) hipLaunchKernelGGL(t4k::wideSeedKernel, dim3(nq0 < cus ? nq0 : cus), dim3(512), 0, c->stream, q.base, bv, wk, qa, w, list0, nq0, 0);
        if (nqA > 0) hipLaunchKernelGGL(t4k::wideSeedKernel, dim3(nqA < cus ? nqA : cus), dim3(512), 0, c->stream, q.base, bv, wk, qa, w, listA, nqA, 0);
        hipLaunchKernelGGL(t4k::wideScatterKernel, dim3(clampi(8 * gParts, 16, cus * 8)), dim3(256), 0, c->stream, q.base, w);
        hipLaunchKernelGGL((t4k::wideSortKernel<8192>), dim3(gParts), dim3(512), 0, c->stream, q.base, w);
        hipLaunchKernelGGL(t4k::wideStatsKernel, dim3(gReads), dim3(512), 0, c->stream, q.base, w);
        hipLaunchKernelGGL((t4k::wideChainKernel<8192, 1 << T4_WIDE_OVBITS>), dim3(gParts < cus ? gParts : cus), dim3(512), 0, c->stream, q.base, bv, wk, qa, w);
        hipLaunchKernelGGL(t4k::wideMergeKernel, dim3(gReads), dim3(512), 0, c->stream, q.base, bv, wk, qa, w);
        HIPCHK(c, hipGetLastError());
        if (q.extendLater) {
          hipLaunchKernelGGL(t4k::extendKernel, dim3(c->cus * 16), dim3(64), 0, c->stream, q.base, bv, qa, recsBefore < c->aqPoolCap ? recsBefore : c->aqPoolCap);
          HIPCHK(c, hipGetLastError());
        }
        HIPCHK(c, hipEventRecord(c->ev[1], c->stream));
// ... 169 lines not shown
  if (b->dBarcode) { bc.resize(n); HIPCHK(c, hipMemcpy(bc.data(), b->dBarcode, sizeof(int) * n, hipMemcpyDeviceToHost)); }
  DevBuf<int> dRet;
  DevBuf<T4OverlapOut> dOut;
  int r;
  if ((r = dRet.alloc(c, ASSIGN_WIDE_BATCH)) || (r = dOut.alloc(c, ASSIGN_WIDE_BATCH))) return r;
  std::string bases;
  std::vector<int64_t> off;
  std::vector<int32_t> bcs, sts, hRet(ASSIGN_WIDE_BATCH);
  std::vector<double> factors;
  std::vector<t4_overlap> hOut(ASSIGN_WIDE_BATCH);
  for (size_t at = 0; at < todo.size(); at += ASSIGN_WIDE_BATCH) {
    const int m = (int)(todo.size() - at < (size_t)ASSIGN_WIDE_BATCH ? todo.size() - at : (size_t)ASSIGN_WIDE_BATCH);
    bases.clear(); off.assign(1, 0); bcs.clear(); sts.clear(); factors.clear();
    for (int j = 0; j < m; ++j) {
      const size_t i = (size_t)todo[at + j];
      const unsigned *p = pk.data() + i * wpk, *q = nm.data() + i * wnm;
      for (int x = 0; x < len[i]; ++x) bases.push_back(((q[x >> 5] >> (x & 31)) & 1u) ? 'N' : "ACGT"[(p[x >> 4] >> ((x & 15) * 2)) & 3u]);
      off.push_back((int64_t)bases.size());
      const int barcode = bc.empty() ? -1 : bc[i];
      bcs.push_back(barcode); sts.push_back(strands ? strands[i] : strand); factors.push_back(barcode == -1 ? 1.0 : 2.0);
    }
    if ((r = aqBegin(c, ix->view, nullptr, nullptr, false, m, bases.c_str(), off.data(), bc.empty() ? nullptr : bcs.data(), sts.data(), 0, factors.data(),
                     nullptr, false, nullptr, nullptr, 2))) return r;
    AqResult res;
    if ((r = aqEnd(c, &res))) return r;
    const AqCall &q = c->aq;
    const size_t rec = (size_t)c->aqPoolCap;
    const T4OverlapOut *ov = (const T4OverlapOut *)c->aqPoolDev;
    launch(t4k::assignPickKernel, m, T4_PICK_THREADS, c->stream, m, (const int *)(c->aqOut + q.pCnt), (const int *)(c->aqOut + q.pBase),
           (const int *)(c->aqIn + q.oLen), ov, ov + rec, (const int *)(ov + 2 * rec), c->aqExtAux, c->aqPoolCap, dRet, dOut);
    HIPCHK(c, hipGetLastError());
    HIPCHK(c, hipMemcpyAsync(hRet.data(), dRet, sizeof(int) * (size_t)m, hipMemcpyDeviceToHost, c->stream));
    HIPCHK(c, hipMemcpyAsync(hOut.data(), dOut, sizeof(t4_overlap) * (size_t)m, hipMemcpyDeviceToHost, c->stream));
    HIPCHK(c, hipStreamSynchronize(c->stream));
    ++c->syncEpoch;
    for (int j = 0; j < m; ++j) {
      if (ret) ret[todo[at + j]] = hRet[j];
      if (out) out[todo[at + j]] = hOut[j];
    }
  }
  return T4_OK;
}
}

extern "C" {

int t4_add_query_stats(t4_ctx *c, int64_t *out5) {
  if (!c || !out5) return T4_ERR_ARG;
  out5[0] = c->aqCalls; out5[1] = c->aqReads; out5[2] = c->aqGlobalLaunches; out5[3] = c->aqGlobalReads; out5[4] = c->aqRecords;
  out5[5] = (int64_t)(c->aqKernelMs * 1e3); out5[6] = c->aqHits;
  if (getenv("T4_TIMING")) fprintf(stderr, "timing: AddRead query path host seconds: pack %.3f, first launch to sync %.3f, overflow tiers %.3f; result pool grown %d times\n", c->aqSecPack, c->aqSecFirst, c->aqSecGlobal, c->aqPoolGrows);
  if (getenv("T4_TIMING")) fprintf(stderr, "timing: AddRead query path, host seconds inside the launch: preparation %.3f, prologue %.3f, second stream %.3f, query kernel %.3f, wide + extension %.3f, two event records %.3f, epilogue %.3f\n",
                                   c->aqSecLaunch[0], c->aqSecLaunch[1], c->aqSecLaunch[2], c->aqSecLaunch[3], c->aqSecLaunch[4], c->aqSecLaunch[5], c->aqSecLaunch[6]);
  if (getenv("T4_TIMING")) fprintf(stderr, "timing: wide query: %lld calls with the wide pipeline behind the query kernel, %lld of them had a read deferred to it; %lld with reads on the second stream\n", (long long)c->wideCalls, (long long)c->wideCallsDeferred, (long long)c->wideCallsDirect);
  if (getenv("T4_TIMING")) fprintf(stderr, "timing: wide query: %lld calls repeated -- partition pool %lld, keys of a partition %lld, overlaps of a partition %lld, dependency records %lld; partitions planned %d/16 full at the end\n",
                                   (long long)c->wideRetries, (long long)c->wideFlagCounts[1], (long long)c->wideFlagCounts[2], (long long)c->wideFlagCounts[3], (long long)c->wideFlagCounts[4], 16 * 16 / (c->wideSafetyKeep > 0 ? c->wideSafetyKeep : 32));
  return T4_OK;
}

int t4_add_query_last_call(t4_ctx *c, double *kernel_ms, const int32_t **ticks10ns, int *n) {
  if (!c) return T4_ERR_ARG;
  if (kernel_ms) *kernel_ms = c->aqLastMs;
  if (ticks10ns) *ticks10ns = c->aqLastTicks;
  if (n) *n = c->aqLastN;
  return T4_OK;
}

int t4_add_query_groups(t4_ctx *c, int i, const t4_grp **groups, int *n, int *huge, int *n4) {
  if (!c || !groups || !n) return T4_ERR_ARG;
  const AqCall &q = c->aq;
  if (!q.wide || !c->aqOutHost) return 0;
  const unsigned char *o = c->aqOutHost;
  for (int half = 0; half < 2; ++half) {
    const int *ctl = (const int *)(o + (half ? q.pWctlA : q.pWctl));
    const T4WidePlan *plan = (const T4WidePlan *)(o + (half ? q.pWplanA : q.pWplan));
    const int *stat = (const int *)(o + (half ? q.pWstatA : q.pWstat));
    const int nw = ctl[0] < q.nWideSlots ? ctl[0] : q.nWideSlots;
    for (int w = 0; w < nw; ++w) {
      if (plan[w].read != i) continue;
      *groups = (const t4_grp *)c->grpPoolHost + (half ? (size_t)c->wide.grpCap : 0) + plan[w].grpBase;
      *n = stat[(size_t)w * T4_WIDE_STAT + WS_GROUPS];
      if (huge) *huge = plan[w].huge;
      if (n4) *n4 = stat[(size_t)w * T4_WIDE_STAT + WS_N4];
      return 1;
    }
  }
  return 0;
}

int t4_add_query_last_aux(t4_ctx *c, const int32_t **aux, const int32_t **n4, const int32_t **status, int *n) {
  if (!c || !c->aqOutHost) return T4_ERR_ARG;
  const AqCall &q = c->aq;
  if (aux) *aux = (const int32_t *)(c->aqOutHost + q.pAux);
  if (n4) *n4 = (const int32_t *)(c->aqOutHost + q.pN4);
  if (status) *status = (const int32_t *)(c->aqOutHost + q.pSta);
  if (n) *n = q.n;
  return T4_OK;
}

int t4_add_query_wide_stats(t4_ctx *c, int64_t *out4) {
  if (!c || !out4) return T4_ERR_ARG;
  out4[0] = c->wideReads; out4[1] = c->wideParts; out4[2] = c->wideRetries; out4[3] = c->wideGroups;
  return T4_OK;
}

int t4_add_query_defer_stats(t4_ctx *c, int64_t *out1) {
  if (!c || !out1) return T4_ERR_ARG;
  out1[0] = c->aqDeferredReads;
  return T4_OK;
}

int t4_add_query_last_stable(t4_ctx *c, const int32_t **flags, int *n) {
  if (!c || !flags) return T4_ERR_ARG;
  *flags = c->aqLastStable;
  if (n) *n = c->aqLastN;
  return T4_OK;
}

int t4_assign_pick(t4_ctx *c, int n_reads, const int32_t *counts, const int32_t *base, const int32_t *lens, int64_t n_rec, const t4_overlap *ov,
                   const t4_overlap *ext, const int32_t *ret, const int32_t *aux, int32_t *out_ret, t4_overlap *out) {
  if (!c || n_reads < 0 || n_rec < 0 || n_rec > 0x7FFFFFFF || (n_reads > 0 && (!counts || !base || !lens || !out_ret || !out)) || (n_rec > 0 && (!ov || !ext || !ret || !aux))) return T4_ERR_ARG;
  if (n_reads == 0) return T4_OK;
  (void)hipSetDevice(c->device);
  const size_t n = (size_t)n_reads, m = (size_t)n_rec;
  DevBuf<int> dCnt, dBase, dLen, dRet, dAux, dOutRet;
  DevBuf<T4OverlapOut> dOv, dExt, dOut;
  int r;
  if ((r = dCnt.alloc(c, n)) || (r = dBase.alloc(c, n)) || (r = dLen.alloc(c, n)) || (r = dOutRet.alloc(c, n)) || (r = dOut.alloc(c, n)) ||
      (r = dOv.alloc(c, m)) || (r = dExt.alloc(c, m)) || (r = dRet.alloc(c, m)) || (r = dAux.alloc(c, m))) return r;
  HIPCHK(c, hipMemcpy(dCnt, counts, sizeof(int) * n, hipMemcpyHostToDevice));
  HIPCHK(c, hipMemcpy(dBase, base, sizeof(int) * n, hipMemcpyHostToDevice));
  HIPCHK(c, hipMemcpy(dLen, lens, sizeof(int) * n, hipMemcpyHostToDevice));
  if (m) {
    HIPCHK(c, hipMemcpy(dOv, ov, sizeof(t4_overlap) * m, hipMemcpyHostToDevice));
    HIPCHK(c, hipMemcpy(dExt, ext, sizeof(t4_overlap) * m, hipMemcpyHostToDevice));
    HIPCHK(c, hipMemcpy(dRet, ret, sizeof(int) * m, hipMemcpyHostToDevice));
    HIPCHK(c, hipMemcpy(dAux, aux, sizeof(int) * m, hipMemcpyHostToDevice));
  }
  launch(t4k::assignPickKernel, n_reads, T4_PICK_THREADS, c->stream, n_reads, dCnt, dBase, dLen, dOv, dExt, dRet, dAux, (int)n_rec, dOutRet, dOut);
  HIPCHK(c, hipGetLastError());
  HIPCHK(c, hipStreamSynchronize(c->stream));
  HIPCHK(c, hipMemcpy(out_ret, dOutRet, sizeof(int) * n, hipMemcpyDeviceToHost));
  HIPCHK(c, hipMemcpy(out, dOut, sizeof(t4_overlap) * n, hipMemcpyDeviceToHost));
  return T4_OK;
}

int t4_add_query_pool(t4_index *ix, int n, const char *bases, const int64_t *offsets, const int32_t *barcodes, const int32_t *strands,
                      int skip_repeats, const double *factors, const int32_t **counts, const int32_t **base, const t4_overlap **ov,
                      const t4_overlap **ext, const int32_t **ext_ret, unsigned char *tier_hint) {
  if (!ix || n <= 0 || !bases || !offsets || !strands || !factors || !counts || !base || !ov || !ext || !ext_ret) return T4_ERR_ARG;
  t4_ctx *c = ix->ctx;
  if (!ix->committed) return fail(c, T4_ERR_STATE, "index not committed");
  if (ix->view.firstIsRef) return fail(c, T4_ERR_UNSUPPORTED, "t4_add_query needs a contig set");
  AqResult res;
  int r = addQueryPool(c, ix->view, nullptr, nullptr, false, n, bases, offsets, barcodes, strands, skip_repeats, factors, &res, tier_hint, true);
  if (r) return r;
  *counts = res.counts; *base = res.base; *ov = res.ov; *ext = res.ext; *ext_ret = res.ret;
  return T4_OK;
}

int t4_add_query_pool_begin2(t4_index *ix, int n, const char *bases, const int64_t *offsets, const int32_t *barcodes, const int32_t *strands,
                             int skip_repeats, const double *factors, unsigned char *tier_hint, const int32_t *only_seq, const int32_t *force_min, int want_cands) {
  if (!ix || n <= 0 || !bases || !offsets || !strands || !factors) return T4_ERR_ARG;
  t4_ctx *c = ix->ctx;
  if (!ix->committed) return fail(c, T4_ERR_STATE, "index not committed");
  if (ix->view.firstIsRef) return fail(c, T4_ERR_UNSUPPORTED, "t4_add_query needs a contig set");
  return aqBegin(c, ix->view, nullptr, nullptr, false, n, bases, offsets, barcodes, strands, skip_repeats, factors, tier_hint, true, only_seq, force_min, want_cands);
}
int t4_add_query_last_cands(t4_ctx *c, const t4_cand **pool, const int32_t **base, const int32_t **cnt, const int32_t **stats8, int *n) {
  if (!c || !c->aqOutHost) return T4_ERR_ARG;
  const AqCall &q = c->aq;
  static_assert(sizeof(t4_cand) == sizeof(T4Cand) && sizeof(T4Cand) == 24 && T4_QUERY_STATS == T4_QSTATS, "candidate record layout");
  if (pool) *pool = q.wantCands ? (const t4_cand *)c->candPool : nullptr;
  if (base) *base = (const int32_t *)(c->aqOutHost + q.pCb);
  if (cnt) *cnt = q.wantCands ? (const int32_t *)(c->aqOutHost + q.pCc) : nullptr;
  if (stats8) *stats8 = (const int32_t *)(c->aqOutHost + q.pS8);
  if (n) *n = q.n;
  return T4_OK;
}
int t4_add_query_pool_done(t4_ctx *c) { return c ? aqDone(c) : 1; }
int t4_add_query_pool_end(t4_ctx *c, const int32_t **counts, const int32_t **base, const t4_overlap **ov, const t4_overlap **ext, const int32_t **ext_ret) {
  if (!c || !counts || !base || !ov || !ext || !ext_ret) return T4_ERR_ARG;
  AqResult res;
  int r = aqEnd(c, &res);
  if (r) return r;
  *counts = res.counts; *base = res.base; *ov = res.ov; *ext = res.ext; *ext_ret = res.ret;
  return T4_OK;
}

int t4_add_query(t4_index *ix, int n, const char *bases, const int64_t *offsets, const int32_t *barcodes, const int32_t *strands,
                 int skip_repeats, const double *factors, int max_per_read, int32_t *counts, t4_overlap *ov, t4_overlap *ext, int32_t *ext_ret) {
  if (!ix || n < 0 || max_per_read <= 0 || (n > 0 && (!bases || !offsets || !strands || !factors || !counts || !ov || !ext || !ext_ret))) return T4_ERR_ARG;
  t4_ctx *c = ix->ctx;
  if (!ix->committed) return fail(c, T4_ERR_STATE, "index not committed");
  if (ix->view.firstIsRef) return fail(c, T4_ERR_UNSUPPORTED, "t4_add_query needs a contig set");
  if (n == 0) return T4_OK;
  return addQueryImpl(c, ix->view, nullptr, nullptr, false, n, bases, offsets, barcodes, strands, skip_repeats, factors, max_per_read, counts, ov, ext, ext_ret);
}

}

struct t4_cellstore {
  t4_ctx *ctx = nullptr;
  int k = 9, hitLenRequired = 31, radius = 10, nomatchGapLimit = 0;
  double novelSim = 0.9;
  struct Slot { unsigned char *base = nullptr; size_t cap = 0, imgBytes = 0; bool live = false; bool pending = false; };
  std::vector<Slot> slots;
  std::vector<int> freeIds;
  std::vector<unsigned char *> chunks;
  size_t chunkUsed = 0;
  std::map<size_t, std::vector<unsigned char *>> freeBySize;
  T4IndexView *dViews = nullptr;
  int viewCap = 0;
  unsigned char *stHost = nullptr, *stDev = nullptr;
  size_t stCap = 0, stUsed = 0;
  std::vector<T4CopyDesc> descs;
  T4CopyDesc *dDescs = nullptr;
  size_t descCap = 0;
  std::vector<T4TableBuild> builds;
  std::vector<int> buildSlots;
  std::vector<unsigned char> ctlHost;
  int *dBuildErr = nullptr, *hBuildErr = nullptr;
  int64_t imagesBuilt = 0, keysShipped = 0, tableBytesBuilt = 0;
  std::vector<T4BytePatch> patches;
  T4BytePatch *dPatches = nullptr;
  size_t patchCap = 0;
  int64_t bytesPatched = 0;
  int64_t bytesStaged = 0;
  bool bigFirst = false;
  std::mutex mu;
  static constexpr size_t CHUNK = (size_t)256 << 20;
};

namespace {
int cellAlloc(t4_cellstore *cs, size_t cap, unsigned char **out) {
  auto it = cs->freeBySize.find(cap);
  if (it != cs->freeBySize.end() && !it->second.empty()) { *out = it->second.back(); it->second.pop_back(); return T4_OK; }
  if (cap > t4_cellstore::CHUNK) return fail(cs->ctx, T4_ERR_UNSUPPORTED, "a per-barcode set image of %zu bytes exceeds the arena chunk", cap);
  if (cs->chunks.empty() || cs->chunkUsed + cap > t4_cellstore::CHUNK) {
    unsigned char *p = nullptr;
    HIPCHK(cs->ctx, hipMalloc(&p, t4_cellstore::CHUNK));
    cs->chunks.push_back(p); cs->chunkUsed = 0;
  }
  *out = cs->chunks.back() + cs->chunkUsed;
  cs->chunkUsed += cap;
  return T4_OK;
}
// ... 590 lines not shown
```

trust4_amd/csrc/t4_assembler.cpp:

```cpp
#include <stdio.h>
#include <string.h>

#include <algorithm>
#include <atomic>
#include <chrono>
#include <condition_variable>
#include <deque>
#include <functional>
#include <mutex>
#include <thread>
#include <map>
#include <memory>
#include <string>
#include <unordered_map>
#include <tuple>
#include <vector>

#include "../../include/trust4_hip.h"
#include "t4_internal.h"

namespace {

inline unsigned char t4PwByte(int a, int c, int g, int t) {
  const int sum = a + c + g + t;
// ... 715 lines not shown
    int sum = w.c[0] + w.c[1] + w.c[2] + w.c[3];
    {
      const int s1 = sum + 1;
      bool flip = sum == 0 || (unsigned)(sum - 3 * w.c[base]) < 2u;
      for (int x = 0; x < 4; ++x) flip = flip || (x != base && 3 * w.c[x] == s1);
      if (!flip) { ++w.c[base]; return; }
    }
    unsigned before = sum == 0 ? 16u : 0u, after = 0;
    for (int x = 0; x < 4; ++x) before |= (sum < 3 * w.c[x]) ? (1u << x) : 0u;
    ++w.c[base]; ++sum;
    for (int x = 0; x < 4; ++x) after |= (sum < 3 * w.c[x]) ? (1u << x) : 0u;
    if (before == after) return;
    const int pos = (int)(&w - seqs[seqIdx].pw.data());
    if (live()) { markBaseDirty(seqIdx, pos); evRegion(seqIdx, pos, pos + 1); return; }
    if (owner && !dirty && slot >= 0) {
      invalidateCell();
      patches.push_back(PwPatch{seqIdx, pos, (unsigned char)after});
      return;
    }
    structuralChange(seqIdx);
  }
  int prefetch(int n, const char *const *reads, const int *strands, const int *barcodes, int repetitive);
  int prefetchLive(int n, const char *const *reads, const int *strands, const int *barcodes, int repetitive);
  void buildGroups(Cached &e);
  void registerKmers(Cached &e, int slot, int shard = -1);
  struct DeltaRec {
    std::vector<int64_t> slot; std::vector<uint64_t> slotCode; std::vector<uint32_t> slotStart, slotCnt;
    std::vector<int64_t> postAt; std::vector<int32_t> postLen, postData;
    std::vector<int32_t> seqId; std::vector<t4_seq_record> seqRec;
    std::vector<int64_t> baseAt; std::vector<int32_t> baseLen; std::string baseCons; std::vector<uint8_t> basePw;
    t4_index_delta d;
    int64_t version = 0;
    void reset() {
      slot.clear(); slotCode.clear(); slotStart.clear(); slotCnt.clear(); postAt.clear(); postLen.clear(); postData.clear(); seqId.clear(); seqRec.clear();
      baseAt.clear(); baseLen.clear(); baseCons.clear(); basePw.clear(); version = 0;
    }
  };
  std::vector<std::unique_ptr<DeltaRec>> deltaSpare;
  struct Lane {
    t4_ctx *ctx = nullptr; bool ownCtx = false;
    t4_index *dev = nullptr;
    int64_t version = 0;
    bool busy = false;
    int polls = 0;
    std::vector<int> slots; std::vector<int64_t> uids; std::vector<unsigned char> hint;
    std::string bases; std::vector<int64_t> offs; std::vector<int32_t> bcs, sts, only, force; std::vector<double> fac;
    int repetitive = 0;
  };
  std::vector<Lane> lanes;
  std::deque<std::unique_ptr<DeltaRec>> deltaLog;
  int64_t deltaVersion = 0;
  int64_t launches = 0, launchesUrgent = 0, headWaits = 0, killedInFlight = 0, lightRounds = 0, restrictedOnlyRounds = 0, wholeQueries = 0, restrictedQueries = 0;
  std::vector<float> roundKernelMs, roundWallMs;
  std::chrono::steady_clock::time_point laneT0;
  double secHeadWait = 0, secLaunch = 0, secHarvest = 0;
  int ensureLanes();
  int flushLive(Lane **out);
  int makeDelta();
  int bringUpToDate(Lane &L);
  int launchOn(Lane &L, const std::vector<int> &todo, int repetitive);
  int harvest(Lane &L);
  void abandonJobs();
  int pumpLive(bool needHead, int repetitive);
  void announceLive(int n, const char *const *reads, const int *strands, const int *barcodes, int repetitive);
  int verifyServed(const Cached &c);
  int64_t verified = 0, verifiedMerged = 0;
  void beginWindow(int n, const char *const *reads, const int *strands, const int *barcodes, int repetitive);
  void endWindow(const int32_t *cnts, const t4_overlap *ov, const t4_overlap *ex, const int32_t *rets, int stride);
  int stageImage();
  int releaseFinishedBarcode(int barcode, int contigMinCov);
  bool isContigShallow(int i, int minCov) const;
  void releaseShallowContigs(int minCov);

  void setPrev(int seqIdx, int rs, int re, int ss, int se, int strand) {
    prevAdd.seqIdx = seqIdx; prevAdd.readStart = rs; prevAdd.readEnd = re; prevAdd.seqStart = ss; prevAdd.seqEnd = se; prevAdd.strand = strand;
  }

  int refreshDevice() {
    if (!dirty) return T4_OK;
    auto t0_ = std::chrono::steady_clock::now();
    struct Tm { double &acc; std::chrono::steady_clock::time_point t0; ~Tm() { acc += std::chrono::duration<double>(std::chrono::steady_clock::now() - t0).count(); } } tm_{secRefresh, t0_};
    int r;
    if (!dev) { if ((r = t4_index_create(ctx, k, index.considerBarcode ? 1 : 0, &dev))) return r; }
    if ((r = t4_index_clear(dev))) return r;
    if ((r = t4_index_set_params(dev, hitLenRequired, radius, novelSim))) return r;
    for (const Seq &s : seqs) {
      int id;
      const char *cons = s.released ? "" : s.cons.c_str();
      if ((r = t4_index_add_contig(dev, s.released ? "" : s.name.c_str(), cons, s.barcode,
                                   s.released || s.pw.empty() ? nullptr : (const int32_t *)s.pw.data(), &id))) return r;
    }
    std::vector<uint64_t> code; std::vector<int32_t> bucket, idx, off;
    code.reserve(index.total); bucket.reserve(index.total); idx.reserve(index.total); off.reserve(index.total);
    for (const auto &kv : index.map)
      for (uint32_t t = 0; t < kv.second.cnt; ++t) {
        const Post &p = index.arena[kv.second.start + t];
        code.push_back(kv.first.code); bucket.push_back(kv.first.h); idx.push_back(p.idx); off.push_back(p.offset);
      }
    if ((r = t4_index_commit_postings(dev, (int64_t)code.size(), code.data(), bucket.data(), idx.data(), off.data()))) return r;
    dirty = false; ++refreshes;
    return T4_OK;
  }

  int inputNovelRead(const char *id, const char *read, int strand, int barcode) {
    Seq ns;
    ns.name = id; ns.cons = read;
    if (strand == -1) reverseComplement(ns.cons, std::string(read));
    ns.barcode = barcode; ns.numRead = 1;
    int len = (int)ns.cons.size();
    ns.pw.assign(len, PosWeight{{0, 0, 0, 0}});
    for (int i = 0; i < len; ++i) if (ns.cons[i] != 'N') ns.pw[i].c[nucNum(ns.cons[i])] = 1;
    int seqIdx = (int)seqs.size();
// ... 514 lines not shown
    size_t j = i + 1;
    while (j < index.dirtyPost.size() && index.dirtyPost[j] == index.dirtyPost[j - 1] + 1) ++j;
    R.postAt.push_back(index.dirtyPost[i]); R.postLen.push_back((int32_t)(j - i));
    for (size_t t = i; t < j; ++t) { const Post &p = index.arena[index.dirtyPost[t]]; R.postData.push_back(p.idx); R.postData.push_back(p.offset); if (index.dirtyPost[t] < index.dirtyPostFlag.size()) index.dirtyPostFlag[index.dirtyPost[t]] = 0; }
    i = j;
  }
  index.dirtyPost.clear();
  int maxLen = 0;
  for (int c : dirtySeqs) {
    Seq &q = seqs[c];
    q.devDirty = false;
    const int len = q.released ? 0 : (int)q.cons.size();
    if (len > maxLen) maxLen = len;
    int lo = q.dLo, hi = q.dHi;
    if (len + 1 > q.baseCap) {
      q.baseCap = len + 1 + (len < 512 ? 256 : len / 2);
      q.baseOff = baseUsed; baseUsed += q.baseCap;
      lo = 0; hi = len + 1;
    }
    if (hi > len + 1) hi = len + 1;
    if (lo < 0) lo = 0;
    t4_seq_record rec;
    memset(&rec, 0, sizeof rec);
    rec.base_off = q.baseOff; rec.len = len; rec.barcode = q.barcode;
    for (int t = 0; t < 8 && t < (int)q.name.size() && !q.released; ++t) rec.name[t] = q.name[t];
    R.seqId.push_back(c); R.seqRec.push_back(rec);
    if (hi > lo) {
      R.baseAt.push_back(q.baseOff + lo); R.baseLen.push_back(hi - lo);
      const size_t at0 = R.baseCons.size();
      R.baseCons.resize(at0 + (size_t)(hi - lo)); R.basePw.resize(at0 + (size_t)(hi - lo));
      char *bc = &R.baseCons[at0];
      uint8_t *bp = &R.basePw[at0];
      const int nMarks = (int)q.postCnt.size();
      for (int t = lo; t < hi; ++t) {
        unsigned char mark = 0;
        if (t < nMarks) mark = (unsigned char)((q.postCnt[(size_t)t] > 3 ? 3 : q.postCnt[(size_t)t]) << 5);
        if (t == 0 && q.marksBad) mark |= 128;
        if (t < len) { bc[t - lo] = q.cons[t]; bp[t - lo] = (uint8_t)(t4PwByte(q.pw[t].c[0], q.pw[t].c[1], q.pw[t].c[2], q.pw[t].c[3]) | mark); }
        else { bc[t - lo] = '\0'; bp[t - lo] = (uint8_t)(t4PwByte(0, 0, 0, 0) | mark); }
      }
    }
  }
  dirtySeqs.clear();
  if (maxLen > maxSeqLenSeen) maxSeqLenSeen = maxLen;
  maxLen = maxSeqLenSeen;
  d.table_slots = index.tabSlots; d.table_rebuilt = index.tabRebuilt ? 1 : 0;
  d.post_cap = (int64_t)index.arena.size(); d.base_cap = baseUsed + 1024; d.seq_cap = (int32_t)seqs.size() + 64;
  d.nseq = (int32_t)seqs.size(); d.max_seq_len = maxLen;
  d.n_slots = (int64_t)R.slot.size(); d.slot = R.slot.data(); d.slot_code = R.slotCode.data(); d.slot_start = R.slotStart.data(); d.slot_cnt = R.slotCnt.data();
  d.n_post_runs = (int64_t)R.postAt.size(); d.post_at = R.postAt.data(); d.post_len = R.postLen.data(); d.post_data = R.postData.data();
  d.n_seqs = (int32_t)R.seqId.size(); d.seq_id = R.seqId.data(); d.seq = R.seqRec.data();
  d.n_base_runs = (int64_t)R.baseAt.size(); d.base_at = R.baseAt.data(); d.base_len = R.baseLen.data(); d.base_cons = R.baseCons.data(); d.base_pw = R.basePw.data();
  index.tabRebuilt = false; liveReset = false;
  R.version = ++deltaVersion;
  ++deltas; deltaBytes += (int64_t)(R.slot.size() * 16 + R.postData.size() * 4 + R.seqRec.size() * sizeof(t4_seq_record) + R.baseCons.size() * 2);
  deltaLog.push_back(std::move(recp));
  return T4_OK;
}

int t4_assembler::ensureLanes() {
  if (!lanes.empty()) return T4_OK;
  const int nLanes = knobs.lanes;
  lanes.resize(nLanes < 1 ? 1 : (nLanes > 8 ? 8 : nLanes));
  lanes[0].ctx = ctx;
  for (size_t i = 1; i < lanes.size(); ++i) {
    const int r = t4_init(t4_ctx_device(ctx), &lanes[i].ctx);
    if (r) { err = "a query lane could not be created"; lanes.resize(i); return lanes.size() > 0 ? T4_OK : r; }
    lanes[i].ownCtx = true;
  }
  for (Lane &L : lanes) L.version = deltaVersion - (int64_t)deltaLog.size();
  return T4_OK;
}

int t4_assembler::bringUpToDate(Lane &L) {
  int r;
  if (!L.dev) { if ((r = t4_index_create(L.ctx, k, 0, &L.dev))) return r; }
  if ((r = t4_index_set_params(L.dev, hitLenRequired, radius, novelSim))) return r;
  for (const auto &rec : deltaLog) {
    if (rec->version <= L.version) continue;
    if ((r = t4_index_apply_delta(L.dev, &rec->d))) return r;
    L.version = rec->version;
  }
  int64_t minV = deltaVersion;
  for (const Lane &x : lanes) if (x.version < minV) minV = x.version;
  while (!deltaLog.empty() && deltaLog.front()->version <= minV) { if (deltaSpare.size() < 8) deltaSpare.push_back(std::move(deltaLog.front())); deltaLog.pop_front(); }
  return T4_OK;
}

void t4_assembler::abandonJobs() {
  for (Lane &L : lanes) {
    if (!L.busy) continue;
    const int32_t *a = nullptr, *b = nullptr, *e = nullptr; const t4_overlap *c = nullptr, *d2 = nullptr;
    (void)t4_add_query_pool_end(L.ctx, &a, &b, &c, &d2, &e);
    L.busy = false;
    for (size_t i = 0; i < L.slots.size(); ++i) { Cached &en = *pool[L.slots[i]]; if (en.uid == L.uids[i]) { en.inflight = false; en.killed = false; en.shifts.clear(); } }
  }
}

int t4_assembler::flushLive(Lane **out) {
  int r;
  if ((r = ensureLanes())) return r;
  Lane *L = nullptr;
  for (Lane &x : lanes) if (!x.busy) { L = &x; break; }
  if (!L) { L = &lanes.back(); if ((r = harvest(*L))) return r; }
  if ((r = makeDelta())) return r;
  if ((r = bringUpToDate(*L))) return r;
  *out = L;
  return T4_OK;
}

int t4_assembler::verifyServed(const Cached &c) {
  if (index.total == 0) return c.cnt == 0 ? T4_OK : T4_ERR_STATE;
  int rc;
  Lane *L = nullptr;
  if ((rc = flushLive(&L))) return rc;
  const char *bases = c.read.empty() ? "A" : c.read.c_str();
  const int64_t offs[2] = {0, (int64_t)c.read.size()};
  const int32_t bc = c.barcode, st = c.strand;
  const double fac = (c.barcode == -1 && !c.skip) ? 1.0 : 2.0;
  const int32_t *cnts = nullptr, *bas = nullptr, *rets = nullptr;
  const t4_overlap *ov = nullptr, *ex = nullptr;
  unsigned char hint = c.tier;
  if ((rc = t4_add_query_pool(L->dev, 1, bases, offs, &bc, &st, c.skip, &fac, &cnts, &bas, &ov, &ex, &rets, &hint))) return rc;
  ++verified;
  auto same = [](const t4_overlap &a, const t4_overlap &b) {
    return a.seqIdx == b.seqIdx && a.readStart == b.readStart && a.readEnd == b.readEnd && a.seqStart == b.seqStart && a.seqEnd == b.seqEnd &&
           a.strand == b.strand && a.matchCnt == b.matchCnt && a.indelCnt == b.indelCnt && a.similarity == b.similarity;
  };
  const int n = c.cnt > 0 ? c.cnt : 0;
  bool ok = c.merged ? (cnts[0] > 0 ? cnts[0] : 0) == n : cnts[0] == c.cnt;
  if (ok && c.merged) {
    std::vector<int> pa(n), pb(n);
    for (int i = 0; i < n; ++i) pa[i] = pb[i] = i;
// ... 377 lines not shown
      e.checkPending = false;
      if (!e.valid) { e.editedKeys.clear(); continue; }
      int T[2], e4[2], e5[2], big[2];
      bool ror[2] = {false, false}, headTouched = false;
      ++toleranceChecks;
      const int headLen = e.smhi[0] > e.smhi[1] ? e.smhi[0] : e.smhi[1];
      bool ok = !e.inexact && exactStats(e, -1, nullptr, T, e4, e5, big, e.fragile ? ror : nullptr, headLen, e.fragile ? &headTouched : nullptr) && T[0] == e.minT[0] && T[1] == e.minT[1];
      if (ok && e.fragile) { ++fragileChecks; ok = e.rorOk && ror[0] == e.ror0[0] && ror[1] == e.ror0[1] && !headTouched; if (!ok) ++invLongLists; }
      e.editedKeys.clear();
      if (!ok) { kill(e, invFragile); ++toleranceCheckKills; }
    }
    idxEvents.clear();
    ts.lap(TS_EVENTS_INDEX);
  }
}

void t4_assembler::announceLive(int n, const char *const *reads, const int *strands, const int *barcodes, int repetitive) {
  size_t keep = 0;
  for (; keep < order.size() && keep < (size_t)n; ++keep) {
    const Cached &c = *pool[order[keep]];
    if (c.read != reads[keep] || c.strand != strands[keep] || c.barcode != (barcodes ? barcodes[keep] : -1) || c.skip != repetitive) break;
  }
  while (order.size() > keep && keep < (size_t)n) {
    const int sl = order.back(); order.pop_back();
    pool[sl]->valid = false; pool[sl]->partial = false; pool[sl]->inflight = false; pool[sl]->uid = 0; freeSlots.push_back(sl);
    if (pool[sl]->registered) { --winKmerLive; pool[sl]->registered = false; }
  }
  if (winKmerRefs > 64 * 142 && winKmerRefs > 4 * (winKmerLive + 1) * 142) {
    for (WinKmers &w : winShard) w.clear(); winKmerRefs = 0; winKmerLive = 0;
    for (int sl : order) if (pool[sl]->registered) registerKmers(*pool[sl], sl);
  }
  for (size_t i = keep; i < (size_t)n; ++i) {
    int sl;
    if (!freeSlots.empty()) { sl = freeSlots.back(); freeSlots.pop_back(); }
    else { sl = (int)pool.size(); pool.push_back(new Cached()); }
    Cached &c = *pool[sl];
    c.read = reads[i]; c.strand = strands[i]; c.barcode = barcodes ? barcodes[i] : -1; c.skip = repetitive; c.cnt = 0; c.valid = false;
    c.inflight = false; c.killed = false; c.shifts.clear();
    c.ov.clear(); c.ext.clear(); c.extRet.clear();
    c.uid = nextUid++; c.tier = 0; c.hintPredicted = false; c.lastUs = 0; c.registered = false; c.lastKill = 0;
    c.hasDev = false; c.hostRecords = false; c.expectWide = false; c.conservative = false; c.sawCommit = false; c.devGroups.clear(); c.dbgGroups.clear(); c.devInfo.clear(); c.rorOk = false; c.editedKeys.clear();
    c.partial = false; c.pendingContig = -1; c.merged = false; c.auxOk = false; c.restrictedCount = 0; c.kmerPos.clear();
    c.cands.clear(); c.candOk = false; c.exactKeys.clear(); c.morePending.clear(); c.inexact = false; c.repeatNear = false; c.checkPending = false; c.maskOk = false;
    order.push_back(sl);
  }
}

int t4_assembler::launchOn(Lane &L, const std::vector<int> &todo, int repetitive) {
  auto tl0_ = std::chrono::steady_clock::now();
  struct Tl { double &acc; std::chrono::steady_clock::time_point t0; ~Tl() { acc += std::chrono::duration<double>(std::chrono::steady_clock::now() - t0).count(); } } tl_{secLaunch, tl0_};
  int rc;
  ts.lap(TS_PUMP_OTHER);
  if ((rc = makeDelta())) return rc;
  { auto t0 = std::chrono::steady_clock::now(); rc = bringUpToDate(L); secDelta += std::chrono::duration<double>(std::chrono::steady_clock::now() - t0).count(); if (rc) return rc; }
  const int m = (int)todo.size();
  ts.lap(TS_DELTA);
  wideQueries = knobs.wideQueries; wideHitLimit = knobs.wideHitLimit;
  L.slots.clear(); L.uids.clear(); L.hint.clear(); L.bcs.clear(); L.sts.clear(); L.fac.clear(); L.only.clear(); L.force.clear();
  L.bases.clear(); L.offs.assign(1, 0); L.repetitive = repetitive;
  bool anyOnly = false;
  for (int i = 0; i < m; ++i) {
    Cached &c = *pool[todo[i]];
    const int nItems = c.partial ? 1 + (int)c.morePending.size() : 1;
    for (int t = 0; t < nItems; ++t) {
      L.slots.push_back(todo[i]); L.uids.push_back(c.uid); L.hint.push_back(c.tier);
      L.bases += c.read; L.offs.push_back((int64_t)L.bases.size()); L.bcs.push_back(c.barcode); L.sts.push_back(c.strand);
      L.fac.push_back((c.barcode == -1 && !repetitive) ? 1.0 : 2.0);
      L.only.push_back(c.partial ? (t == 0 ? c.pendingContig : c.morePending[(size_t)t - 1]) : -1);
      L.force.push_back((c.partial && c.candOk) ? ((c.minT[0] & 0xFFFF) | ((c.minT[1] & 0xFFFF) << 16)) : 0);
    }
    c.inflight = true; c.killed = false; c.shifts.clear();
    if (c.partial) { anyOnly = true; continue; }
    c.statsStable = false;
    c.hasDev = false; c.hostRecords = false; c.expectWide = false; c.conservative = false; c.sawCommit = false; c.devGroups.clear(); c.dbgGroups.clear(); c.devInfo.clear(); c.rorOk = false; c.editedKeys.clear();
    c.auxOk = false; c.merged = false; c.restrictedCount = 0;
    c.cands.clear(); c.candOk = false; c.exactKeys.clear();
  }
  const int mi = (int)L.slots.size();
  bool anyOnlyAll = true;
  for (int v : L.only) if (v < 0) { anyOnlyAll = false; break; }
  { int nOnly = 0; for (int v : L.only) nOnly += v >= 0 ? 1 : 0; restrictedQueries += nOnly; wholeQueries += mi - nOnly; if (nOnly == mi) ++restrictedOnlyRounds; }
  laneT0 = tl0_;
  if (L.bases.empty()) L.bases.push_back('A');
  ts.lap(TS_LAUNCH_PACK);
  {
    auto tq0 = std::chrono::steady_clock::now();
    candStore = knobs.candStore;
    rc = t4_add_query_pool_begin2(L.dev, mi, L.bases.data(), L.offs.data(), L.bcs.data(), L.sts.data(), repetitive, L.fac.data(), L.hint.data(), anyOnly ? L.only.data() : nullptr,
                                  anyOnly ? L.force.data() : nullptr, candStore ? 1 : 0);
    secQuery += std::chrono::duration<double>(std::chrono::steady_clock::now() - tq0).count();
  }
  ts.lap(TS_LAUNCH_CALL);
  if (rc) { for (int sl : todo) pool[sl]->inflight = false; return rc; }
  L.busy = true; L.polls = 0;
  ++queries; ++rounds; ++launches; readsQueried += m;
  auto tg1 = std::chrono::steady_clock::now();
  std::atomic<int> nextG(0);
  std::atomic<int> regShard(0);
  std::vector<int> regList;
  for (int sl : todo) if (!pool[sl]->registered) regList.push_back(sl);
  const auto registerNew = [&]() {
    for (;;) {
      const int sh = regShard.fetch_add(1);
      if (sh >= WK_SHARDS) break;
      for (int sl : regList) registerKmers(*pool[sl], sl, sh);
    }
  };
  const std::function<void()> groupWorker = [&]() {
    if (!regList.empty() && regShard.load() < WK_SHARDS) registerNew();
    for (;;) {
      int i = nextG.fetch_add(1);
      if (i >= m) break;
      Cached &e = *pool[todo[i]];
      if (e.partial) continue;
      if (wideQueries && emittedHits(e) > wideHitLimit) {
        if (knobs.verifyWindow && !e.skip) { buildGroups(e); e.dbgGroups.swap(e.devGroups); e.devGroups.clear(); e.hasDev = false; e.hostRecords = false; }
        e.expectWide = true; e.groups.reset(16); e.slack = -1; e.fragile = true;
      }
      else buildGroups(e);
    }
  };
  std::vector<int> predict;
  std::atomic<int> nextP(0);
  if (wideQueries && mi > 0 && !anyOnlyAll) {
    size_t seen = 0;
    for (size_t i = 0; i < order.size() && seen < 48; ++i) {
      Cached &e = *pool[order[i]];
      if (e.valid || e.inflight || e.partial || e.hintPredicted || e.tier || e.lastUs) continue;
      predict.push_back(order[i]); ++seen;
    }
  }
  const std::function<void()> worker2 = [&]() {
    groupWorker();
    for (;;) {
// ... 236 lines not shown
    if (keep && anyRecut) for (size_t q = 0; q < items.size() && keep; ++q) if (items[q].src < 0 && !items[q].wasCut && cut[q] && sameGeom(c.ov[t], items[q].o)) keep = false;
    if (keep) for (size_t q = 0; q < droppedKept.size() && keep; ++q) if (sameGeom(c.ov[t], droppedKept[q])) keep = false;
    if (!keep) continue;
    if (w != t) { c.ov[w] = c.ov[t]; c.ext[w] = c.ext[t]; c.extRet[w] = c.extRet[t]; }
    ++w;
  }
  c.ov.resize(w); c.ext.resize(w); c.extRet.resize(w);
  for (size_t t = 0; t < items.size(); ++t) {
    const int j = items[t].src;
    if (j < 0 || cut[t]) continue;
    if (ov[j].similarity < novelSim) continue;
    c.ov.push_back(ov[j]); c.ext.push_back(ex[j]); c.extRet.push_back(rets[j]);
  }
  (void)k2;
  if (anyRecut) ++candRecut;
  if (items.size() > 50) ++candMergesBig;
  if (n4hi[0] > 100 || n4hi[1] > 100) ++candMergesStats;
  c.cnt = (int32_t)c.ov.size();
  c.cands.resize(items.size());
  for (size_t t = 0; t < items.size(); ++t) { c.cands[t] = items[t].o; if (cut[t]) c.cands[t].flags |= 4; else c.cands[t].flags &= (unsigned short)~4u; }
  for (int t = 0; t < 2; ++t) { c.n4lo[t] = n4lo[t]; c.n4hi[t] = n4hi[t]; c.n5lo[t] = n5lo[t]; c.n5hi[t] = n5hi[t]; c.smlo[t] = smlo[t]; c.smhi[t] = smhi[t]; c.minT[t] = newT[t]; }
  if (raisedT) ++candRaised;
  c.nAll = c.nAllBound = (int)c.cands.size();
  for (int t = 0; t < 2; ++t) {
    const uint32_t key = (uint32_t)pc * 2u + (uint32_t)t;
    if (s8[4 + t] > 0 || c.findGroup(key)) { Grp &g = c.getGroup(key); g.cnt = (uint32_t)s8[4 + t]; g.lo = s8[8 + t]; g.hi = s8[10 + t]; }
    if (std::find(c.exactKeys.begin(), c.exactKeys.end(), key) == c.exactKeys.end()) c.exactKeys.push_back(key);
  }
  c.statsStable = exactStable && !knobs.noStableStats; c.n4 = c.n4hi[0] + c.n4hi[1]; c.slack = 99 - c.n4;
  ++candMerges;
  return true;
}

int t4_assembler::harvest(Lane &L) {
  if (!L.busy) return T4_OK;
  auto th0_ = std::chrono::steady_clock::now();
  struct Th { double &acc; std::chrono::steady_clock::time_point t0; ~Th() { acc += std::chrono::duration<double>(std::chrono::steady_clock::now() - t0).count(); } } th_{secHarvest, th0_};
  const int32_t *cnts = nullptr, *bas = nullptr, *rets = nullptr;
  const t4_overlap *ov = nullptr, *ex = nullptr;
  int rc;
  ts.lap(TS_PUMP_OTHER);
  {
    auto tq0 = std::chrono::steady_clock::now();
    rc = t4_add_query_pool_end(L.ctx, &cnts, &bas, &ov, &ex, &rets);
    secQuery += std::chrono::duration<double>(std::chrono::steady_clock::now() - tq0).count();
  }
  ts.lap(TS_HARVEST_WAIT);
  L.busy = false;
  const int m = (int)L.slots.size();
  if (!rc && lanes.size() == 1) {
    double ms_ = 0; (void)t4_add_query_last_call(L.ctx, &ms_, nullptr, nullptr);
    roundKernelMs.push_back((float)ms_);
    roundWallMs.push_back((float)(std::chrono::duration<double>(std::chrono::steady_clock::now() - laneT0).count() * 1e3));
  }
  if (rc) {
    if (L.ctx != ctx) err = t4_last_error(L.ctx);
    for (int i = 0; i < m; ++i) { Cached &c = *pool[L.slots[i]]; if (c.uid == L.uids[i]) { c.inflight = false; c.killed = false; } }
    dropWindow();
    return rc;
  }
  FILE *roundLog = knobs.roundLog;
  if (roundLog) {
    double ms = 0; const int32_t *ticks = nullptr; int nn = 0;
    t4_add_query_last_call(L.ctx, &ms, &ticks, &nn);
    fprintf(roundLog, "%lld %d %.4f %d |", (long long)rounds, m, ms, (int)seqs.size());
    for (int i = 0; i < m && i < nn; ++i) fprintf(roundLog, " %d/%d/%d/%d", ticks ? ticks[i] / 100 : -1, cnts[i], (int)L.hint[i], pool[L.slots[i]]->uid == L.uids[i] ? (int)pool[L.slots[i]]->killed : 2);
    fputc('\n', roundLog);
  }
  const int32_t *ticks10ns = nullptr; int nTicks = 0;
  { double ms_ = 0; (void)t4_add_query_last_call(L.ctx, &ms_, &ticks10ns, &nTicks); }
  const int32_t *stable = nullptr; int nStable = 0;
  const bool noStable = knobs.noStableStats;
  if (!noStable) (void)t4_add_query_last_stable(L.ctx, &stable, &nStable);
  const int32_t *aux = nullptr, *n4s = nullptr, *qstatus = nullptr; int nAux = 0;
  (void)t4_add_query_last_aux(L.ctx, &aux, &n4s, &qstatus, &nAux);
  const t4_cand *candPool = nullptr; const int32_t *candBase = nullptr, *candCnt = nullptr, *stats8 = nullptr; int nCand = 0;
  (void)t4_add_query_last_cands(L.ctx, &candPool, &candBase, &candCnt, &stats8, &nCand);
  std::vector<unsigned char> groupsCopied((size_t)m, 0);
  if (threads > 1 && m >= 2) {
    std::vector<int> big; size_t total = 0;
    for (int i = 0; i < m; ++i) {
      if (L.only[i] >= 0) continue;
      const Cached &c = *pool[L.slots[i]];
      if (c.uid != L.uids[i] || !c.inflight || c.killed) continue;
      const t4_grp *dg = nullptr; int ng = 0;
      if (t4_add_query_groups(L.ctx, i, &dg, &ng, nullptr, nullptr) == 1 && ng >= 1024) { big.push_back(i); total += (size_t)ng; }
    }
    if (big.size() >= 2 && total >= 16384) {
      std::atomic<int> next(0);
      const std::function<void()> copier = [&]() {
        for (;;) {
          const int t = next.fetch_add(1);
          if (t >= (int)big.size()) break;
          const int i = big[(size_t)t];
          Cached &c = *pool[L.slots[i]];
          const t4_grp *dg = nullptr; int ng = 0;
          if (t4_add_query_groups(L.ctx, i, &dg, &ng, nullptr, nullptr) == 1) { c.devGroups.assign((const Grp *)dg, (const Grp *)dg + ng); groupsCopied[(size_t)i] = 1; }
        }
      };
      const int nHelp = (int)big.size() - 1 < threads - 1 ? (int)big.size() - 1 : threads - 1;
      if (!helpers) helpers.reset(new HelperPool());
      helpers->start(nHelp, copier);
      copier();
      helpers->wait();
    }
  }
// ... 393 lines not shown
int t4_assembler_prefetch(t4_assembler *a, int n, const char *const *reads, const int *strands, const int *barcodes, int repetitive_data) {
  if (!a || n < 0 || (n > 0 && (!reads || !strands))) return T4_ERR_ARG;
  return a->prefetch(n, reads, strands, barcodes, repetitive_data ? 1 : 0);
}
int t4_assembler_window_valid(const t4_assembler *a) {
  if (!a) return 0;
  if (a->live()) return a->idxEvents.empty() && a->structEvents.empty() && !a->order.empty() && a->pool[a->order.front()]->valid;
  return a->cacheHead < a->cache.size() && a->cache[a->cacheHead].valid;
}
int t4_assembler_counters(const t4_assembler *a, int64_t *queries, int64_t *refreshes, int64_t *window_hits) {
  if (!a) return T4_ERR_ARG;
  if (queries) *queries = a->queries;
  if (refreshes) *refreshes = a->refreshes;
  if (window_hits) *window_hits = a->cacheHits;
  return T4_OK;
}
int t4_assembler_timers(const t4_assembler *a, double *sec_refresh, double *sec_query) {
  if (!a) return T4_ERR_ARG;
  if (sec_refresh) *sec_refresh = a->secRefresh;
  if (sec_query) *sec_query = a->secQuery;
  return T4_OK;
}
int t4_assembler_repeat_add_read(t4_assembler *a, const char *read) {
  if (!a) return T4_ERR_ARG - 100;
  a->ts.begin();
  const int r = a->repeatAddRead(read);
  a->ts.lap(TS_REPEAT);
  a->processEvents();
  return r;
}
int t4_assembler_update_all_consensus(t4_assembler *a) { if (!a) return T4_ERR_ARG; a->ts.begin(); a->updateAllConsensus(); a->ts.lap(TS_UPDATE_CONS); a->processEvents(); return T4_OK; }
int t4_assembler_set_threads(t4_assembler *a, int host_threads) { if (!a || host_threads < 1) return T4_ERR_ARG; a->threads = host_threads > 64 ? 64 : host_threads; return T4_OK; }
int t4_assembler_live_counters(const t4_assembler *a, int64_t *out, int n) {
  if (!a || !out || n < 1) return T4_ERR_ARG;
  const int64_t v[16] = {a->rounds, a->readsQueried, a->deltas, a->deltaBytes, a->invalidations, a->invKey, a->invCross, a->invRegion, a->invShift,
                         a->invContig, a->invFragile, a->tolerated, (int64_t)(a->secDelta * 1e6), (int64_t)(a->secGroups * 1e6), (int64_t)(a->secEvents * 1e6), (int64_t)(a->secQuery * 1e6)};
  for (int i = 0; i < n && i < 16; ++i) out[i] = v[i];
  if (n >= 23) t4_add_query_stats(a->ctx, out + 16);
  if (n >= 27) t4_add_query_wide_stats(a->ctx, out + 23);
  if (n >= 28) out[27] = a->wideServed;
  if (getenv("T4_VERIFY_WINDOW")) fprintf(stderr, "T4_VERIFY_WINDOW: the host's replay of the emitted hits equals the wide query's dependency records for all %lld reads it was held against\n", (long long)a->groupSelfChecks);
  if (getenv("T4_VERIFY_WINDOW")) fprintf(stderr, "T4_VERIFY_WINDOW: %lld served window entries queried again at serve time, all equal to their cached results (%lld of them put together from restricted re-queries)\n", (long long)a->verified, (long long)a->verifiedMerged);
  if (getenv("T4_TIMING")) {
    fprintf(stderr, "timing: assembler host seconds: add_read calls %.3f (incl. waits for the head), prefetch calls %.3f; launching %.3f (of which deltas %.3f, dependency sets %.3f, registering k-mers %.3f), harvesting %.3f, event examination %.3f, index edits %.3f\n",
            a->secAddTotal, a->secPrefetch, a->secLaunch, a->secDelta, a->secGroups, a->secRegister, a->secHarvest, a->secEvents, a->index.secOps);
    {
      const double spt = a->ts.secondsPerTick();
      fprintf(stderr, "timing: the chain's host thread by section (seconds):");
      for (int i = 0; i < TS_N; ++i) fprintf(stderr, " %s %.3f%s", TS_NAMES[i], (double)a->ts.acc[i] * spt, i + 1 < TS_N ? ";" : "\n");
      fprintf(stderr, "timing: host index: %lld postings found through their hint, %lld by walking a list (%lld postings walked over)\n", (long long)a->index.hintHits, (long long)a->index.hintWalks, (long long)a->index.walkSteps);
    }
    fprintf(stderr, "timing: query lanes %d: %lld launches (%lld for a head without a result, %lld of them without the whole queries of entries further back), %lld waits for the head's lane in %.3f s, %lld queries killed in flight\n",
            (int)a->lanes.size(), (long long)a->launches, (long long)a->launchesUrgent, (long long)a->lightRounds, (long long)a->headWaits, a->secHeadWait, (long long)a->killedInFlight);
    fprintf(stderr, "timing: rounds whose head waited for a WHOLE query: %lld never queried before, fallen to a change of: a key %lld, a list crossing 100 / 10000 postings %lld, a region %lld, a shift %lld, a whole contig %lld, the tolerance budget %lld, a restricted re-query that fell back %lld\n",
            (long long)a->headWholeWhy[0], (long long)a->headWholeWhy[1], (long long)a->headWholeWhy[2], (long long)a->headWholeWhy[3], (long long)a->headWholeWhy[4], (long long)a->headWholeWhy[5], (long long)a->headWholeWhy[6], (long long)a->headWholeWhy[7]);
    fprintf(stderr, "timing: thresholds checked after an edit of a small group by repeating the statistics loop: %lld entries, %lld of them fell (%lld of the checks for reads with lists beyond 10000 postings: removeOnlyRepeats and the head of the hit array as well)\n", (long long)a->toleranceChecks, (long long)a->toleranceCheckKills, (long long)a->fragileChecks);
    fprintf(stderr, "timing: tolerated index edits %lld, of which %lld met an entry whose group statistics cannot move (no budget spent); tolerance kills %lld, of which %lld for lists beyond 10000 postings\n",
            (long long)a->tolerated, (long long)a->toleratedStable, (long long)a->invFragile, (long long)a->invLongLists);
    fprintf(stderr, "timing: restricted re-queries: %lld entries kept their other contigs when one contig changed, %lld merged, %lld fell back to the whole query, %lld in flight met another change of their contig\n",
            (long long)a->restrictedMarks, (long long)a->restrictedMerged, (long long)a->restrictedFallbacks, (long long)a->restrictedStale);
    fprintf(stderr, "timing: entries that fell whole when one contig changed: %lld with lists beyond 10000 postings, %lld with overlaps on the other strand, %lld with more than 44 candidate overlaps, %lld with ~100 groups of four hits, %lld without the query's report, %lld other\n",
            (long long)a->whyNot[0], (long long)a->whyNot[1], (long long)a->whyNot[2], (long long)a->whyNot[3], (long long)a->whyNot[4], (long long)a->whyNot[5]);
    fprintf(stderr, "timing: candidate store: %lld candidate records kept with whole queries, %lld restricted re-queries merged through the replay of the scan (%lld with more than 50 candidates, %lld with more than 100 groups of four hits on a strand, %lld cut a candidate of another contig), fell back to the whole query: %lld a cut candidate of another contig passes now, %lld the group statistics could move the threshold, %lld an overlap on the other strand, %lld other; %lld whole queries checked against the host's scan; %lld thresholds settled by repeating the statistics loop over the entry's groups, %lld raised thresholds served by dropping the candidates of shorter runs\n",
            (long long)a->candRecords, (long long)a->candMerges, (long long)a->candMergesBig, (long long)a->candMergesStats, (long long)a->candRecut, (long long)a->candFallbackUncut, (long long)a->candFallbackStats, (long long)a->candFallbackStrand, (long long)a->candFallbackOther, (long long)a->candSelfChecks, (long long)a->candExactStats, (long long)a->candRaised);
    fprintf(stderr, "timing: wide query served %lld window entries (%lld dependency records came back with them), %lld reads it was expected for stayed on the LDS tier\n", (long long)a->wideServed, (long long)a->wideGroupRecords, (long long)a->wideMispredicted);
  }
  return T4_OK;
}
int t4_assembler_chain_stats(const t4_assembler *a, double *out, int n) {
  if (!a || !out || n < 1) return T4_ERR_ARG;
  auto pct = [](std::vector<float> v, double p) { if (v.empty()) return 0.0; std::sort(v.begin(), v.end()); return (double)v[(size_t)(p * (double)(v.size() - 1))]; };
  const double v[10] = {(double)a->rounds, (double)a->restrictedOnlyRounds, pct(a->roundKernelMs, 0.05), pct(a->roundKernelMs, 0.5), pct(a->roundWallMs, 0.05), pct(a->roundWallMs, 0.5),
                        (double)a->wholeQueries, (double)a->restrictedQueries, (double)a->candRecords, (double)a->candMerges};
  for (int i = 0; i < n && i < 10; ++i) out[i] = v[i];
  return T4_OK;
}
int t4_assembler_output(t4_assembler *a, const char *path) { return a ? a->output(path) : T4_ERR_ARG; }
int t4_assembler_size(const t4_assembler *a) { return a ? (int)a->seqs.size() : 0; }
int t4_assembler_contig(const t4_assembler *a, int i, t4_contig_view *out) {
  if (!a || !out || i < 0 || i >= (int)a->seqs.size()) return T4_ERR_ARG;
  const Seq &s = a->seqs[i];
  memset(out, 0, sizeof *out);
  out->name = s.name.c_str();
  out->consensus = s.released ? nullptr : s.cons.c_str();
  out->posweight = s.released || s.pw.empty() ? nullptr : (const int32_t *)s.pw.data();
  out->len = s.released ? 0 : (int32_t)s.cons.size(); out->barcode = s.barcode; out->num_read = s.numRead;
  out->min_left_ext_anchor = s.minLeftExtAnchor; out->min_right_ext_anchor = s.minRightExtAnchor; out->in_index = s.frozen ? 0 : 1;
  return T4_OK;
}
int t4_assembler_change_kmer_length(t4_assembler *a, int kmer_length) {
  if (!a || kmer_length < 2 || kmer_length > 31) return T4_ERR_ARG;
  return a->changeKmerLength(kmer_length);
}
int64_t t4_assembler_index_postings(const t4_assembler *a) { return a ? (int64_t)a->index.total : 0; }
int t4_assembler_release_finished_barcode(t4_assembler *a, int barcode, int contig_min_cov) {
  if (!a) return T4_ERR_ARG;
  const int r = a->releaseFinishedBarcode(barcode, contig_min_cov);
  a->processEvents();
  return r;
}
int t4_assembler_release_shallow_contigs(t4_assembler *a, int min_cov) { if (!a) return T4_ERR_ARG; a->releaseShallowContigs(min_cov); a->processEvents(); return T4_OK; }
int t4_assembler_output_barcodes(t4_assembler *a, const char *path, const char *const *barcode_names, int n_names) {
  if (!a || !path) return T4_ERR_ARG;
  FILE *fp = fopen(path, "w");
  if (!fp) return T4_ERR_IO;
  for (int i = 0; i < (int)a->seqs.size(); ++i) {
// ... 194 lines not shown
```

trust4_amd/csrc/t4_device.h:

```cpp
#pragma once
#include <stdint.h>

#define T4_MAXL 384
#define T4_MAXPOS (2 * T4_MAXL)
#define T4_MAXGAP 320
#define T4_DIR_BYTES 49152
#define T4_NTIER 6

#define T4_IDX_BITS 22
#define T4_C_BITS 21
#define T4_B_BITS 20
#define T4_C_BIAS (1 << 20)
#define T4_MAX_SEQS (1 << T4_IDX_BITS)
#define T4_MAX_SEQLEN (1 << T4_B_BITS)

struct T4SeqInfo {
  int consOff;
  int len;
  int pwOff;
  int barcode;
  unsigned char isRef, geneType , name0, name1, name2, name3;
  unsigned short pad1;
};

// ... 133 lines not shown
  unsigned short flags;
};
#define T4_QSTATS 12
struct T4CandArgs {
  T4Cand *candOut;
  unsigned *candCursor;
  int *candOverflow;
  int candCap;
  int *candBase, *candCnt;
  int *stats8;
  const int *forceMin;
  int *extAux;
};
#define T4_PW_MARK_SHIFT 5
#define T4_PW_MARK_BAD 128
#define T4_CAND_PLUS 1
#define T4_CAND_SIMZERO 2
#define T4_CAND_CUT 4
#define T4_CAND_RUN_SHIFT 3

struct T4QueryArgs {
  int mode;
  int strand;
  int skipRepeats;
  int maxPerRead;
  int *counts;
  T4OverlapOut *out;
  const T4OverlapOut *in;
  const int *inCounts;
  int *ret;
  double mismatchFactor;
  const int *strandPerRead;
  const double *factorPerRead;
  T4OverlapOut *outExt;
  int *outBase;
  unsigned *poolCursor;
  int poolCap;
  int extendLater;
  T4OverlapOut *outDev;
  int *recRead;
  int leanExt;
  int *readTicks;
  int *statsStable;
  const int *onlySeq;
  int *aux;
  int *n4;
  const struct T4CandArgs *cs;
  const T4IndexView *views;
  const int *viewOf;
};

struct T4BytePatch { unsigned char *dst; unsigned long long val; };
struct T4CopyDesc { unsigned long long srcOff; unsigned char *dst; unsigned long long bytes; };
struct T4TableBuild { T4HashEntC *table; unsigned long long tableSlots, srcOff, nKeys; };
```

trust4_amd/csrc/t4_internal.h:

```cpp
#pragma once
#include <stddef.h>
#include <stdint.h>
#include "../../include/trust4_hip.h"

extern "C" {

typedef struct t4_cellstore t4_cellstore;
int t4_cellstore_create(t4_ctx *ctx, int kmer_length, t4_cellstore **out);
void t4_cellstore_destroy(t4_cellstore *cs);
int t4_cellstore_set_params(t4_cellstore *cs, int hit_len_required, int radius, double novel_seq_similarity);
int t4_cellstore_open(t4_cellstore *cs, int *slot);
int t4_cellstore_close(t4_cellstore *cs, int slot);
int t4_cellstore_stage(t4_cellstore *cs, int slot, int barcode, int nseq, const char *const *names, const char *const *cons,
                       const int32_t *const *pw, int64_t nkeys, const uint64_t *key_code, const int32_t *key_bucket,
                       const int32_t *key_cnt, const int32_t *post, int64_t *pw_offset_in_image,
                       const int32_t *seq_barcodes );
int t4_cellstore_stage_compact(t4_cellstore *cs, int slot, int barcode, int nseq, const char *const *names, const char *const *cons,
                               const int32_t *const *pw, int64_t nkeys, const uint64_t *key_code, const int32_t *key_bucket,
                               const int32_t *key_cnt, const int32_t *post, int64_t *pw_offset_in_image, const int32_t *seq_barcodes);
int t4_cellstore_patch(t4_cellstore *cs, int slot, int n, const int64_t *byte_offsets, const unsigned char *values);
size_t t4_cellstore_image_bytes(int nseq, int64_t nkeys, int64_t npost, int64_t cons_bytes);
size_t t4_cellstore_full_image_bytes(int nseq, int64_t nkeys, int64_t npost, int64_t cons_bytes);
int t4_cellstore_prepare(t4_cellstore *cs, int max_slot, size_t bytes);
int t4_cellstore_query(t4_cellstore *cs, int n, const int32_t *slots, const char *bases, const int64_t *offsets,
                       const int32_t *barcodes, const int32_t *strands, int skip_repeats, const double *factors,
                       int max_per_read, int32_t *counts, t4_overlap *ov, t4_overlap *ext, int32_t *ext_ret);
int t4_cellstore_set_big_first(t4_cellstore *cs, int on);
int64_t t4_cellstore_bytes_staged(const t4_cellstore *cs);
int t4_cellstore_image_stats(const t4_cellstore *cs, int64_t *out4);
int64_t t4_cellset_live_keys_staged(const t4_cellset *cs);
int t4_cellstore_read_image(t4_cellstore *cs, int slot, void *buf, size_t cap, size_t *bytes, void *view);

int t4_add_query_pool(t4_index *ix, int n, const char *bases, const int64_t *offsets, const int32_t *barcodes, const int32_t *strands,
                      int skip_repeats, const double *factors, const int32_t **counts, const int32_t **base, const t4_overlap **ov,
                      const t4_overlap **ext, const int32_t **ext_ret, unsigned char *tier_hint);

#define T4_QUERY_STATS 12
typedef struct { int32_t seqIdx, ss, se; int16_t rs, re, m0, matchCnt, indelCnt; uint16_t flags; } t4_cand;
int t4_add_query_pool_begin2(t4_index *ix, int n, const char *bases, const int64_t *offsets, const int32_t *barcodes, const int32_t *strands,
                             int skip_repeats, const double *factors, unsigned char *tier_hint, const int32_t *only_seq, const int32_t *force_min, int want_cands);
int t4_add_query_last_cands(t4_ctx *ctx, const t4_cand **pool, const int32_t **base, const int32_t **cnt, const int32_t **stats8, int *n);
int t4_add_query_last_aux(t4_ctx *ctx, const int32_t **aux, const int32_t **n4, const int32_t **status, int *n);
int t4_add_query_pool_done(t4_ctx *ctx);
int t4_ctx_device(t4_ctx *ctx);
int t4_add_query_pool_end(t4_ctx *ctx, const int32_t **counts, const int32_t **base, const t4_overlap **ov, const t4_overlap **ext, const int32_t **ext_ret);

int t4_add_query_stats(t4_ctx *ctx, int64_t *out7);
int t4_add_query_last_stable(t4_ctx *ctx, const int32_t **flags, int *n);
typedef struct { uint32_t key, cnt; int32_t lo, hi; } t4_grp;
int t4_add_query_groups(t4_ctx *ctx, int i, const t4_grp **groups, int *n, int *huge, int *n4);
int t4_add_query_wide_stats(t4_ctx *ctx, int64_t *out4);
int t4_add_query_defer_stats(t4_ctx *ctx, int64_t *out1);
int t4_add_query_last_call(t4_ctx *ctx, double *kernel_ms, const int32_t **ticks10ns, int *n);
int t4_assign_pick(t4_ctx *ctx, int n_reads, const int32_t *counts, const int32_t *base, const int32_t *lens, int64_t n_rec, const t4_overlap *ov,
                   const t4_overlap *ext, const int32_t *ret, const int32_t *aux, int32_t *out_ret, t4_overlap *out);

}
```

trust4_amd/csrc/t4_kernels.h:

```cpp
#pragma once
#include <hip/hip_runtime.h>

#include "t4_device.h"

namespace t4k {

#ifdef T4_INLINE_ALL
#define T4_NI
#else
#define T4_NI __attribute__((noinline))
#endif
#ifndef T4_OPT_JOBSORT
#define T4_OPT_JOBSORT 1
#endif
#ifndef T4_OPT_ROWWALK
#define T4_OPT_ROWWALK 1
#endif
#ifndef T4_NI_R3
#define T4_NI_R3 0
#endif
#ifdef __HIPCC__
#define T4_LDS_AS __attribute__((address_space(3)))
#else
#define T4_LDS_AS
// ... 3833 lines not shown
    const T4HashEntC *keys = (const T4HashEntC *)(staging + tb.srcOff);
    const unsigned long long mask = tb.tableSlots - 1;
    for (unsigned long long k = threadIdx.x; k < tb.nKeys; k += blockDim.x) {
      const T4HashEntC key = keys[k];
      unsigned long long s = mix64(key.code) & mask, probes = 0;
      bool placed = false;
      for (; probes < tb.tableSlots; ++probes) {
        const unsigned long long seen = atomicCAS(&tb.table[s].code, ~0ull, key.code);
        if (seen == ~0ull) { *(uint2 *)&tb.table[s].start = make_uint2(key.start, key.cnt); placed = true; break; }
        if (seen == key.code) break;
        s = (s + 1) & mask;
      }
      if (!placed) *err = b + 1;
    }
  }
}

__global__ __launch_bounds__(256) void deltaKernel(const unsigned char *staging, const T4CopyDesc *desc, int nDesc) {
  const int wavesPerBlock = blockDim.x >> 6, lane = threadIdx.x & 63;
  for (int d = blockIdx.x * wavesPerBlock + (threadIdx.x >> 6); d < nDesc; d += gridDim.x * wavesPerBlock) {
    const T4CopyDesc cd = desc[d];
    const unsigned char *src = staging + cd.srcOff;
    unsigned char *dst = cd.dst;
    if ((((unsigned long long)dst | (unsigned long long)src | cd.bytes) & 7ull) == 0) {
      const unsigned long long n8 = cd.bytes >> 3;
      for (unsigned long long i = lane; i < n8; i += 64) ((unsigned long long *)dst)[i] = ((const unsigned long long *)src)[i];
    } else
      for (unsigned long long i = lane; i < cd.bytes; i += 64) dst[i] = src[i];
  }
}

__global__ __launch_bounds__(256) void aqPrologueKernel(const unsigned long long *hostIn, unsigned long long *devIn, unsigned long long inWords,
                                                        unsigned long long *devOut, unsigned long long outWords) {
  const unsigned long long t = (unsigned long long)blockIdx.x * blockDim.x + threadIdx.x, nt = (unsigned long long)gridDim.x * blockDim.x;
  for (unsigned long long i = t; i < inWords; i += nt) devIn[i] = hostIn[i];
  for (unsigned long long i = t; i < outWords; i += nt) devOut[i] = 0ull;
}
__global__ __launch_bounds__(256) void aqEpilogueKernel(const unsigned long long *devOut, unsigned long long *hostOut, unsigned long long outWords,
                                                        unsigned *done, unsigned *hostFlag, unsigned seq) {
  const unsigned long long t = (unsigned long long)blockIdx.x * blockDim.x + threadIdx.x, nt = (unsigned long long)gridDim.x * blockDim.x;
  for (unsigned long long i = t; i < outWords; i += nt) hostOut[i] = devOut[i];
  __threadfence_system();
  __syncthreads();
  if (threadIdx.x == 0) {
    const unsigned before = atomicAdd(done, 1u);
    if (before + 1u == gridDim.x) {
      *done = 0u;
      __threadfence_system();
      __atomic_store_n(hostFlag, seq, __ATOMIC_RELEASE);
    }
  }
}

__global__ __launch_bounds__(256) void patchKernel(const T4BytePatch *patches, int n) {
  for (int i = blockIdx.x * blockDim.x + threadIdx.x; i < n; i += gridDim.x * blockDim.x) *patches[i].dst = (unsigned char)patches[i].val;
}

__global__ __launch_bounds__(64) void binKernel(T4IndexView ix, T4BatchView bv, int useBarcode, T4TierCaps caps,
                                               int *lists, int *counts, long long listStride) {
  __shared__ unsigned s_posStart[T4_MAXPOS + 8];
  __shared__ unsigned s_posPref[T4_MAXPOS + 8];
  __shared__ char s_seg[T4_MAXL + 8];
  __shared__ char s_rc[T4_MAXL + 8];
  __shared__ int s_red[16];
  __shared__ int s_buf[T4_NTIER][64];
  __shared__ int s_cnt[T4_NTIER];
  WaveMem wm;
  wm.seg = s_seg; wm.rc = s_rc;
  if (laneId() < T4_NTIER) s_cnt[laneId()] = 0;
  __syncthreads();
  for (long long r = blockIdx.x; r < bv.n; r += gridDim.x) {
    int len = bv.len[r];
    int H = 0;
    if (len >= ix.k) {
      loadSegment(bv, r, 0, len, wm);
      int barcode = (useBarcode && bv.barcode) ? bv.barcode[r] : -1;
      H = seedPositions(ix, wm, len, 0, barcode, false, s_posStart, s_posPref, s_red);
    }
    H = __shfl(H, 0);
    int t = 0;
    while (t < T4_NTIER - 1 && H > caps.cap[t]) ++t;
    if (laneId() == 0) { s_buf[t][s_cnt[t]] = (int)r; ++s_cnt[t]; }
    __syncthreads();
    const int filled = s_cnt[t];
    __syncthreads();
    if (filled == 64) {
      int base = 0;
      if (laneId() == 0) { base = atomicAdd(&counts[t], 64); s_cnt[t] = 0; }
      base = __shfl(base, 0);
      lists[t * listStride + base + laneId()] = s_buf[t][laneId()];
      __syncthreads();
    }
  }
  for (int t = 0; t < T4_NTIER; ++t) {
    const int n = s_cnt[t];
    if (n == 0) continue;
    int base = 0;
    if (laneId() == 0) base = atomicAdd(&counts[t], n);
    base = __shfl(base, 0);
    if (laneId() < n) lists[t * listStride + base + laneId()] = s_buf[t][laneId()];
  }
}

__device__ __forceinline__ unsigned long long kcMix(unsigned long long z) {
  z = (z ^ (z >> 30)) * 0xBF58476D1CE4E5B9ULL; z = (z ^ (z >> 27)) * 0x94D049BB133111EBULL; return z ^ (z >> 31);
}
// ... 421 lines not shown
```

Baseline: 19730.

## Fuse deferred index delta, input staging and readback into one light query kernel

Adds a single-kernel "light" AddRead round for restricted queries with no direct reads. That one kernel applies a pending index delta, copies the inputs from host-mapped memory and zeroes the header arrays. It then runs processRead and has the last block write results back to host memory and raise the completion flag. Index deltas can now be deferred and folded into the next query instead of getting their own launch, and the host spin loop gains a pause instruction. The intent is to remove several kernel launches and copies per small round. The cost is more complex ordering logic, a kernel limited to one wave per EU with large LDS use, and flushes of the pending delta that every other entry point must remember.

After: 19140. 0.97x the previous value.

```diff
diff --git a/trust4_amd/build.py b/trust4_amd/build.py
--- a/trust4_amd/build.py
+++ b/trust4_amd/build.py
@@ -14,14 +14,27 @@
 FLAGS = ["--offload-arch=gfx950", "-O3", "-std=c++17", "-ffp-contract=off", "-fPIC", "-shared"]
 
 
+KNOBS_OUT = os.path.join(HERE, "variants", "libt4hip_knobs.so")
+
+
 def build(force=False, verbose=False):
-    if not force and os.path.exists(OUT) and all(os.path.getmtime(OUT) >= os.path.getmtime(d) for d in DEPS):
+    def fresh(out):
+        return not force and os.path.exists(out) and all(os.path.getmtime(out) >= os.path.getmtime(d) for d in DEPS)
+    if fresh(OUT) and fresh(KNOBS_OUT):
         return OUT
     hipcc = os.environ.get("HIPCC", "/opt/rocm/bin/hipcc")
-    cmd = [hipcc] + FLAGS + ["-o", OUT, SRC, SRC_HOST, "-lz", "-lpthread", "-ldl"]
-    if verbose:
-        print(" ".join(cmd))
-    subprocess.run(cmd, check=True)
+    os.makedirs(os.path.dirname(KNOBS_OUT), exist_ok=True)
+    jobs = []
+    for out, extra in ((OUT, []), (KNOBS_OUT, ["-DT4_TEST_KNOBS"])):
+        if fresh(out):
+            continue
+        cmd = [hipcc] + FLAGS + extra + ["-o", out, SRC, SRC_HOST, "-lz", "-lpthread", "-ldl"]
+        if verbose:
+            print(" ".join(cmd))
+        jobs.append((cmd, subprocess.Popen(cmd)))
+    failed = [cmd for cmd, p in jobs if p.wait() != 0]
+    if failed:
+        raise subprocess.CalledProcessError(1, failed[0])
     build_driver(verbose)
     return OUT
 
@@ -37,6 +50,11 @@
         if verbose:
             print(" ".join(cmd))
         subprocess.run(cmd, check=True)
+    cmd = ["g++", "-O2", "-std=c++17", "-DT4_TEST_KNOBS", "-o", os.path.join(os.path.dirname(KNOBS_OUT), "trust4-hip-knobs"), os.path.join(HERE, "host", "trust4_main.cpp"),
+           "-L" + os.path.dirname(KNOBS_OUT), "-lt4hip_knobs", "-Wl,-rpath," + os.path.dirname(KNOBS_OUT), "-Wl,-rpath,$ORIGIN", "-lz", "-lpthread"]
+    if verbose:
+        print(" ".join(cmd))
+    subprocess.run(cmd, check=True)
     return out
 
 
diff --git a/trust4_amd/csrc/t4_api.hip b/trust4_amd/csrc/t4_api.hip
--- a/trust4_amd/csrc/t4_api.hip
+++ b/trust4_amd/csrc/t4_api.hip
@@ -58,6 +58,8 @@
   bool hasOnly = false, hasForce = false, wantCands = false;
   bool keepExtAux = false;
   bool extendLater = false, wide = false, onlyRestricted = false;
+  bool light = false;
+  t4_index *lightIx = nullptr;
   bool sweep2Done = false;
   int nWideSlots = 0;
   bool lazyDone = false, lazyStage = false;
@@ -96,6 +98,12 @@
   unsigned *aqFlagHost = nullptr, *aqFlagDev = nullptr;
   unsigned *aqDoneCtr = nullptr;
   unsigned aqSeq = 0;
+  unsigned *aqLightTail = nullptr;
+  double wallClockKHz = 0;
+  double aqLightEmuMs = 0;
+  bool lightOff = false;
+  int lightMaxItems = T4_LIGHT_MAX_ITEMS; size_t lightMaxBytes = T4_LIGHT_MAX_DELTA_BYTES;
+  int64_t lightRounds = 0, lightFallback[4] = {0, 0, 0, 0};
   size_t aqInBytes = 0, aqOutBytes = 0;
   unsigned char *aqPool = nullptr, *aqPoolDev = nullptr;
   int aqPoolCap = 0;
@@ -118,11 +126,14 @@
   AqCall aq;
   uint64_t syncEpoch = 1;
   struct AqEnv {
-    bool forceGlobal;
+    bool forceGlobal, lightOff = false;
     int capLimit, extendDefer, poolCap, candCap, wideMinHits;
     AqEnv() {
       auto num = [](const char *n, int d) { const char *e = getenv(n); return e ? atoi(e) : d; };
       forceGlobal = getenv("T4_AQ_FORCE_GLOBAL") != nullptr;
+#ifdef T4_TEST_KNOBS
+      lightOff = getenv("T4_TEST_LIGHT_OFF") != nullptr;
+#endif
       capLimit = num("T4_AQ_CAP_LIMIT", 0); poolCap = num("T4_AQ_POOL_CAP", 0); candCap = num("T4_AQ_CAND_CAP", 1 << 18);
       extendDefer = num("T4_AQ_EXTEND_DEFER", 16);
       wideMinHits = num("T4_WIDE_MIN_HITS", 3072);
@@ -165,6 +176,9 @@
   size_t stCap = 0;
   hipEvent_t stEvent = 0;
   bool stPending = false;
+  bool deltaPending = false;
+  bool deltaAppliedSinceQuery = false;
+  size_t deltaNd = 0, deltaBytes = 0;
   uint64_t stEpoch = 0;
 };
 
@@ -389,6 +403,7 @@
   if (c->aqOutHost) (void)hipHostFree(c->aqOutHost);
   if (c->aqFlagHost) (void)hipHostFree(c->aqFlagHost);
   if (c->aqDoneCtr) (void)hipFree(c->aqDoneCtr);
+  if (c->aqLightTail) (void)hipFree(c->aqLightTail);
   if (c->aqPool) (void)hipHostFree(c->aqPool);
   if (c->candPool) (void)hipHostFree(c->candPool);
   if (c->aqRecDev) (void)hipFree(c->aqRecDev);
@@ -704,14 +719,36 @@
   *p = np;
   return T4_OK;
 }
+int launchDelta(t4_ctx *c, const unsigned char *stg, size_t nd) {
+  int grid = (int)((nd + 3) / 4);
+  if (grid > c->cus * 8) grid = c->cus * 8;
+  hipLaunchKernelGGL(t4k::deltaKernel, dim3(grid), dim3(256), 0, c->stream, stg, (const T4CopyDesc *)stg, (int)nd);
+  HIPCHK(c, hipGetLastError());
+  return T4_OK;
+}
+int flushPendingDelta(t4_index *ix) {
+  if (!ix->deltaPending) return T4_OK;
+  ix->deltaPending = false;
+  return launchDelta(ix->ctx, ix->stHostDev, ix->deltaNd);
+}
+int applyDelta(t4_index *ix, const t4_index_delta *d, bool defer);
 }
 
 extern "C" {
 
-int t4_index_apply_delta(t4_index *ix, const t4_index_delta *d) {
+int t4_index_apply_delta(t4_index *ix, const t4_index_delta *d) { return applyDelta(ix, d, false); }
+int t4_index_apply_delta_deferred(t4_index *ix, const t4_index_delta *d) { return applyDelta(ix, d, true); }
+
+}
+
+namespace {
+int applyDelta(t4_index *ix, const t4_index_delta *d, bool defer) {
   if (!ix || !d) return T4_ERR_ARG;
   t4_ctx *c = ix->ctx;
   (void)hipSetDevice(c->device);
+  { const int rf = flushPendingDelta(ix); if (rf) return rf; }
+  const int64_t capTable0 = ix->capTable, capPost0 = ix->capPost, capBase0 = ix->capBase;
+  const int capSeq0 = ix->capSeq;
   if (ix->considerBarcode) return fail(c, T4_ERR_ARG, "t4_index_apply_delta: the index of a live set is not keyed by barcode");
   if (!ix->live && (!ix->seqs.empty() || ix->committed)) return fail(c, T4_ERR_STATE, "t4_index_apply_delta on an index that was filled through t4_index_add_*");
   if (d->table_slots < 2 || (d->table_slots & (d->table_slots - 1))) return fail(c, T4_ERR_ARG, "table_slots must be a power of two");
@@ -810,11 +847,13 @@
     const bool direct = at <= ((size_t)1 << 18);
     if (!direct) HIPCHK(c, hipMemcpyAsync(ix->stDev, ix->stHost, at, hipMemcpyHostToDevice, c->stream));
     ix->stPending = true; ix->stEpoch = c->syncEpoch;
-    int grid = (int)((nd + 3) / 4);
-    if (grid > c->cus * 8) grid = c->cus * 8;
-    const unsigned char *stg = direct ? ix->stHostDev : ix->stDev;
-    hipLaunchKernelGGL(t4k::deltaKernel, dim3(grid), dim3(256), 0, c->stream, stg, (const T4CopyDesc *)stg, (int)nd);
-    HIPCHK(c, hipGetLastError());
+    if (defer && direct && !d->table_rebuilt && capTable0 == ix->capTable && capPost0 == ix->capPost && capBase0 == ix->capBase && capSeq0 == ix->capSeq) {
+      ix->deltaPending = true; ix->deltaNd = nd; ix->deltaBytes = at;
+    } else {
+      const int rl = launchDelta(c, direct ? ix->stHostDev : ix->stDev, nd);
+      if (rl) return rl;
+      if (defer) ix->deltaAppliedSinceQuery = true;
+    }
   }
 view:
   ix->live = true; ix->committed = true; ix->liveNseq = d->nseq;
@@ -828,6 +867,9 @@
   v.novelSim = ix->novelSim; v.refSim = ix->refSim; v.repeatSim = ix->repeatSim;
   return T4_OK;
 }
+}
+
+extern "C" {
 
 int t4_index_size(const t4_index *ix) { return ix ? (ix->live ? ix->liveNseq : (int)ix->seqs.size()) : 0; }
 int t4_index_seq_len(const t4_index *ix, int i) { return (ix && i >= 0 && i < (int)ix->seqs.size()) ? (int)ix->seqs[i].cons.size() : -1; }
@@ -933,6 +975,7 @@
 int runQuery(t4_index *ix, t4_batch *b, T4QueryArgs qa, bool useBarcode, bool noHits = false, std::vector<int> *statusOut = nullptr) {
   t4_ctx *c = ix->ctx;
   if (!ix->committed) return fail(c, T4_ERR_STATE, "index not committed");
+  { const int rf_ = flushPendingDelta(ix); if (rf_) return rf_; }
   if (b->ctx != c) return fail(c, T4_ERR_ARG, "batch belongs to another ctx");
   (void)hipSetDevice(c->device);
   const long long n = b->n;
@@ -1056,6 +1099,7 @@
   if (!ix || !b || !hit_offsets) return T4_ERR_ARG;
   t4_ctx *c = ix->ctx;
   if (!ix->committed) return fail(c, T4_ERR_STATE, "index not committed");
+  { const int rf_ = flushPendingDelta(ix); if (rf_) return rf_; }
   (void)hipSetDevice(c->device);
   const long long n = b->n;
   hit_offsets[0] = 0;
@@ -1512,6 +1556,7 @@
   c->assignWide[0] = c->assignWide[1] = 0;
   if (ix->committed && ix->view.firstIsRef) return fail(c, T4_ERR_UNSUPPORTED, "t4_assign_wide needs a contig set (ExtendOverlap aligns against posWeight)");
   if (!ix->committed) return fail(c, T4_ERR_STATE, "index not committed");
+  { const int rf_ = flushPendingDelta(ix); if (rf_) return rf_; }
   if (b->ctx != c) return fail(c, T4_ERR_ARG, "batch belongs to another ctx");
   if (c->aq.active) return fail(c, T4_ERR_STATE, "an AddRead query is already in flight on this ctx");
   if (b->n == 0) return T4_OK;
@@ -1560,6 +1605,7 @@
   if (!ix || !b || (b->n > 0 && !assign) || !posweight) return T4_ERR_ARG;
   t4_ctx *c = ix->ctx;
   if (!ix->committed) return fail(c, T4_ERR_STATE, "index not committed");
+  { const int rf_ = flushPendingDelta(ix); if (rf_) return rf_; }
   if (ix->live) return fail(c, T4_ERR_UNSUPPORTED, "t4_posweight_recompute takes a committed contig set (the extendedSeq of main.cpp:2047), not a live one");
   if (b->ctx != c) return fail(c, T4_ERR_ARG, "batch belongs to another ctx");
   int64_t bases = 0;
@@ -1659,7 +1705,8 @@
 int aqLaunch(t4_ctx *c);
 int aqBegin(t4_ctx *c, const T4IndexView &base, const T4IndexView *views, const int32_t *viewOf, bool smallFirst, int n, const char *bases,
             const int64_t *offsets, const int32_t *barcodes, const int32_t *strands, int skip_repeats, const double *factors,
-            unsigned char *tierHint = nullptr, bool lean = false, const int32_t *onlySeq = nullptr, const int32_t *forceMin = nullptr, int wantCands = 0) {
+            unsigned char *tierHint = nullptr, bool lean = false, const int32_t *onlySeq = nullptr, const int32_t *forceMin = nullptr, int wantCands = 0,
+            t4_index *lightIx = nullptr) {
   (void)hipSetDevice(c->device);
   AqCall &q = c->aq;
   if (q.active) return fail(c, T4_ERR_STATE, "an AddRead query is already in flight on this ctx");
@@ -1749,6 +1796,9 @@
   for (int i = 0; i < n; ++i) if (direct(i)) ls[nFirst + nDirect++] = i;
   q.nFirst = nFirst; q.nDirect = nDirect;
   c->aqSecPack += tSince(tp0);
+  q.light = lightIx != nullptr && q.onlyRestricted && !q.wide && nDirect == 0 && !(wantCands & 2);
+  q.lightIx = lightIx;
+  if (lightIx && !q.light) { const int rf = flushPendingDelta(lightIx); if (rf) return rf; }
   const int r = aqLaunch(c);
   if (r == T4_OK) q.active = true;
   return r;
@@ -1782,8 +1832,10 @@
   return T4_OK;
 }
 
+int aqLaunchLight(t4_ctx *c);
 int aqLaunch(t4_ctx *c) {
   AqCall &q = c->aq;
+  if (q.light) return aqLaunchLight(c);
   const int n = q.n, nFirst = q.nFirst, nDirect = q.nDirect;
   const bool smallFirst = q.smallFirst;
   int r;
@@ -1957,10 +2009,119 @@
   return r;
 }
 
+int aqLaunchLight(t4_ctx *c) {
+  AqCall &q = c->aq;
+  t4_index *ix = q.lightIx;
+  const int n = q.n;
+  int r;
+  if (!c->aqPool) {
+    const int poolCap0 = c->aqEnv.poolCap;
+    if (!c->aqPoolCap) c->aqPoolCap = poolCap0 > 0 ? poolCap0 : 1 << 16;
+    HIPCHK(c, hipHostMalloc(&c->aqPool, (size_t)c->aqPoolCap * (2 * sizeof(t4_overlap) + sizeof(int32_t)), hipHostMallocMapped));
+    HIPCHK(c, hipHostGetDevicePointer((void **)&c->aqPoolDev, c->aqPool, 0));
+  }
+  const size_t rec = (size_t)c->aqPoolCap;
+  if (q.wantCands && !c->candPool) {
+    if (!c->candCap) c->candCap = c->aqEnv.candCap > 0 ? c->aqEnv.candCap : 1 << 18;
+    HIPCHK(c, hipHostMalloc(&c->candPool, sizeof(T4Cand) * (size_t)c->candCap, hipHostMallocMapped));
+    HIPCHK(c, hipHostGetDevicePointer((void **)&c->candPoolDev, c->candPool, 0));
+  }
+  if (!c->aqLightTail) {
+    unsigned init[T4_LIGHT_TAIL_WORDS];
+    for (int i = 0; i < T4_LIGHT_TAIL_WORDS; ++i) init[i] = (i == 12 || i == 13) ? ~0u : 0u;
+    HIPCHK(c, hipMalloc(&c->aqLightTail, sizeof init));
+    HIPCHK(c, hipMemcpy(c->aqLightTail, init, sizeof init, hipMemcpyHostToDevice));
+    c->wallClockKHz = 100000.0;
+#ifdef __HIPCC__
+    int khz = 0;
+    if (hipDeviceGetAttribute(&khz, hipDeviceAttributeWallClockRate, c->device) == hipSuccess && khz > 0) c->wallClockKHz = (double)khz;
+#endif
+  }
+  q.tf0 = std::chrono::steady_clock::now();
+  auto tl_ = q.tf0;
+  auto lapL = [&](int i) { const auto t = std::chrono::steady_clock::now(); c->aqSecLaunch[i] += std::chrono::duration<double>(t - tl_).count(); tl_ = t; };
+  unsigned *tail = c->aqLightTail;
+  {
+    T4CandArgs cs;
+    memset(&cs, 0, sizeof cs);
+    cs.stats8 = (int *)(c->aqOut + q.pS8);
+    if (q.hasForce) cs.forceMin = (const int *)(c->aqIn + q.oForce);
+    if (q.wantCands) {
+      cs.candOut = c->candPoolDev; cs.candCap = c->candCap; cs.candCursor = tail + 8; cs.candOverflow = (int *)(tail + 9);
+      cs.candBase = (int *)(c->aqOut + q.pCb); cs.candCnt = (int *)(c->aqOut + q.pCc);
+    }
+    memcpy(c->aqInHost + q.oCs, &cs, sizeof cs);
+  }
+  T4BatchView &bv = q.bv;
+  bv.pk = (const unsigned *)(c->aqIn + q.oPk); bv.nm = (const unsigned *)(c->aqIn + q.oNm); bv.len = (const int *)(c->aqIn + q.oLen);
+  bv.barcode = (const int *)(c->aqIn + q.oBc); bv.wpk = q.wpk; bv.wnm = q.wnm; bv.n = n;
+  T4QueryArgs &qa = q.qa;
+  memset(&qa, 0, sizeof qa);
+  qa.mode = 4; qa.skipRepeats = q.skipRepeats; qa.maxPerRead = 0;
+  qa.counts = (int *)(c->aqOut + q.pCnt);
+  qa.out = (T4OverlapOut *)c->aqPoolDev; qa.outExt = qa.out + rec; qa.ret = (int *)(qa.outExt + rec);
+  qa.outBase = (int *)(c->aqOut + q.pBase); qa.poolCursor = tail + 6; qa.poolCap = c->aqPoolCap;
+  qa.strandPerRead = (const int *)(c->aqIn + q.oSt); qa.factorPerRead = (const double *)(c->aqIn + q.oFa);
+  qa.readTicks = (int *)(c->aqOut + q.pTick);
+  qa.statsStable = (int *)(c->aqOut + q.pStab);
+  qa.aux = (int *)(c->aqOut + q.pAux); qa.n4 = (int *)(c->aqOut + q.pN4);
+  qa.onlySeq = (const int *)(c->aqIn + q.oOnly);
+  qa.cs = (const T4CandArgs *)(c->aqIn + q.oCs);
+  qa.leanExt = q.lean ? 1 : 0;
+  q.extendLater = false; q.threads = 512;
+  const int grid = n < c->cus * 2 ? n : c->cus * 2;
+  if ((r = ensureScratch(c, c->cus * 2 * 512))) return r;
+  T4Work &wk = q.wk;
+  memset(&wk, 0, sizeof wk);
+  wk.list = (const int *)(c->aqIn + q.oLs); wk.nList = n;
+  wk.nextCount = (int *)tail;
+  wk.status = (int *)(c->aqOut + q.pSta); wk.hitCounter = (unsigned long long *)(tail + 4);
+  wk.dpRows = c->dpRows; wk.dpDir = c->dpDir;
+  wk.capLimit = c->aqEnv.capLimit;
+  T4Light lt;
+  memset(&lt, 0, sizeof lt);
+  const int n2 = (n + 1) & ~1;
+  if (q.pS8 != sizeof(int) * (size_t)T4_LIGHT_HDR_ARRAYS * n2 || q.pTail != q.pS8 + sizeof(int) * T4_QSTATS * (size_t)n || q.oWide - q.oCs < sizeof(T4CandArgs))
+    return fail(c, T4_ERR_STATE, "the light round's kernel and aqBegin disagree about the header block's layout");
+  if (ix->deltaPending) { lt.staging = ix->stHostDev; lt.nDesc = (int)ix->deltaNd; }
+  lt.n = n; lt.n2 = n2; lt.wpk = q.wpk; lt.wnm = q.wnm;
+  lt.hostIn = c->aqInHostDev; lt.devIn = c->aqIn;
+  lt.oPk = (unsigned)q.oPk; lt.oNm = (unsigned)q.oNm; lt.oLen = (unsigned)q.oLen; lt.oBc = (unsigned)q.oBc; lt.oSt = (unsigned)q.oSt; lt.oLs = (unsigned)q.oLs;
+  lt.oVw = (unsigned)q.oVw; lt.oFa = (unsigned)q.oFa; lt.oOnly = (unsigned)q.oOnly; lt.oForce = (unsigned)q.oForce; lt.oCs = (unsigned)q.oCs;
+  lt.csBytes = (unsigned)((sizeof(T4CandArgs) + 7) & ~(size_t)7);
+  lt.devOut = c->aqOut; lt.hostOut = c->aqOutHostDev; lt.pTail = (unsigned)q.pTail; lt.outBytes = (unsigned)q.outBytes;
+  lt.tail = tail;
+  lt.hostTicks = (unsigned long long *)(c->aqFlagDev + 4);
+  lt.done = c->aqDoneCtr; lt.hostFlag = c->aqFlagDev;
+  ++c->aqSeq;
+  if (c->aqSeq == 0) c->aqSeq = 1;
+  lt.seq = c->aqSeq;
+  lapL(0);
+#ifndef __HIPCC__
+  const auto te0 = std::chrono::steady_clock::now();
+#endif
+  hipLaunchKernelGGL(t4k::lightQueryKernel, dim3(grid), dim3(512), 0, c->stream, q.base, bv, wk, qa, lt);
+  HIPCHK(c, hipGetLastError());
+#ifndef __HIPCC__
+  c->aqLightEmuMs = std::chrono::duration<double, std::milli>(std::chrono::steady_clock::now() - te0).count();
+#endif
+  if (ix->deltaPending) { ix->deltaPending = false; ix->stPending = true; ix->stEpoch = c->syncEpoch; }
+  lapL(3);
+  return T4_OK;
+}
+
+static inline void cpuRelax() {
+#if defined(__x86_64__) || defined(__i386__)
+  __builtin_ia32_pause();
+#elif defined(__aarch64__)
+  asm volatile("yield" ::: "memory");
+#endif
+}
 int aqWait(t4_ctx *c) {
   const unsigned want = c->aqSeq;
   for (unsigned long long spin = 1;; ++spin) {
     if (__atomic_load_n(c->aqFlagHost, __ATOMIC_ACQUIRE) == want) return T4_OK;
+    cpuRelax();
     if ((spin & 0xFFFFull) == 0) {
       const hipError_t e = hipStreamQuery(c->stream);
       if (e == hipSuccess) {
@@ -1995,7 +2156,26 @@
     if ((r = aqWait(c))) return r;
     if ((c->aqSeq & 255u) == 0) HIPCHK(c, hipStreamSynchronize(c->stream));
     ++c->syncEpoch;
-    {
+    const bool wasLight = q.light;
+    q.light = false;
+    if (wasLight) {
+#ifdef __HIPCC__
+      const unsigned long long *tk = (const unsigned long long *)(c->aqFlagHost + 4);
+      const double ms = tk[1] > tk[0] ? (double)(tk[1] - tk[0]) / c->wallClockKHz : 0.0;
+#else
+      const double ms = c->aqLightEmuMs;
+#endif
+      c->aqKernelMs += ms; c->aqLastMs = ms;
+      bool unfinished = *(const int *)(c->aqOutHost + pTail) > 0;
+      const int *st5 = (const int *)(c->aqOutHost + q.pSta);
+      for (int i = 0; i < n && !unfinished; ++i) unfinished = st5[i] == 5;
+      if (unfinished) {
+        ++c->lightFallback[3];
+        if ((r = aqLaunch(c))) return r;
+        continue;
+      }
+      ++c->lightRounds;
+    } else {
       float ms = 0;
       hipError_t ee = hipEventElapsedTime(&ms, c->ev[0], c->ev[1]);
       if (ee == hipErrorNotReady) { (void)hipEventSynchronize(c->ev[1]); ee = hipEventElapsedTime(&ms, c->ev[0], c->ev[1]); }
@@ -2271,6 +2451,8 @@
   if (getenv("T4_TIMING")) fprintf(stderr, "timing: AddRead query path host seconds: pack %.3f, first launch to sync %.3f, overflow tiers %.3f; result pool grown %d times\n", c->aqSecPack, c->aqSecFirst, c->aqSecGlobal, c->aqPoolGrows);
   if (getenv("T4_TIMING")) fprintf(stderr, "timing: AddRead query path, host seconds inside the launch: preparation %.3f, prologue %.3f, second stream %.3f, query kernel %.3f, wide + extension %.3f, two event records %.3f, epilogue %.3f\n",
                                    c->aqSecLaunch[0], c->aqSecLaunch[1], c->aqSecLaunch[2], c->aqSecLaunch[3], c->aqSecLaunch[4], c->aqSecLaunch[5], c->aqSecLaunch[6]);
+  if (getenv("T4_TIMING")) fprintf(stderr, "timing: light rounds: %lld restricted-only calls served in one dispatch (%lld of them behind a delta that needed its own kernel: new array, rebuilt table or copy engine); fell back to four dispatches: %lld for more than %d items, %lld for a delta beyond %zu bytes, %lld for an item that did not finish in the LDS arrays\n",
+                                   (long long)c->lightRounds, (long long)c->lightFallback[2], (long long)c->lightFallback[0], c->lightMaxItems, (long long)c->lightFallback[1], c->lightMaxBytes, (long long)c->lightFallback[3]);
   if (getenv("T4_TIMING")) fprintf(stderr, "timing: wide query: %lld calls with the wide pipeline behind the query kernel, %lld of them had a read deferred to it; %lld with reads on the second stream\n", (long long)c->wideCalls, (long long)c->wideCallsDeferred, (long long)c->wideCallsDirect);
   if (getenv("T4_TIMING")) fprintf(stderr, "timing: wide query: %lld calls repeated -- partition pool %lld, keys of a partition %lld, overlaps of a partition %lld, dependency records %lld; partitions planned %d/16 full at the end\n",
                                    (long long)c->wideRetries, (long long)c->wideFlagCounts[1], (long long)c->wideFlagCounts[2], (long long)c->wideFlagCounts[3], (long long)c->wideFlagCounts[4], 16 * 16 / (c->wideSafetyKeep > 0 ? c->wideSafetyKeep : 32));
@@ -2370,6 +2552,7 @@
   if (!ix || n <= 0 || !bases || !offsets || !strands || !factors || !counts || !base || !ov || !ext || !ext_ret) return T4_ERR_ARG;
   t4_ctx *c = ix->ctx;
   if (!ix->committed) return fail(c, T4_ERR_STATE, "index not committed");
+  { const int rf_ = flushPendingDelta(ix); if (rf_) return rf_; }
   if (ix->view.firstIsRef) return fail(c, T4_ERR_UNSUPPORTED, "t4_add_query needs a contig set");
   AqResult res;
   int r = addQueryPool(c, ix->view, nullptr, nullptr, false, n, bases, offsets, barcodes, strands, skip_repeats, factors, &res, tier_hint, true);
@@ -2384,7 +2567,16 @@
   t4_ctx *c = ix->ctx;
   if (!ix->committed) return fail(c, T4_ERR_STATE, "index not committed");
   if (ix->view.firstIsRef) return fail(c, T4_ERR_UNSUPPORTED, "t4_add_query needs a contig set");
-  return aqBegin(c, ix->view, nullptr, nullptr, false, n, bases, offsets, barcodes, strands, skip_repeats, factors, tier_hint, true, only_seq, force_min, want_cands);
+  bool light = only_seq != nullptr && !skip_repeats && ix->live && !c->lightOff && !c->aqEnv.lightOff && !c->aqEnv.forceGlobal;
+  for (int i = 0; light && i < n; ++i) light = only_seq[i] >= 0;
+  if (light) {
+    if (n > c->lightMaxItems) { light = false; ++c->lightFallback[0]; }
+    else if (ix->deltaPending && (ix->deltaBytes > c->lightMaxBytes || ix->deltaNd > T4_LIGHT_MAX_DESC)) { light = false; ++c->lightFallback[1]; }
+    else if (ix->deltaAppliedSinceQuery) { ++c->lightFallback[2]; }
+  }
+  ix->deltaAppliedSinceQuery = false;
+  if (!light) { const int rf_ = flushPendingDelta(ix); if (rf_) return rf_; }
+  return aqBegin(c, ix->view, nullptr, nullptr, false, n, bases, offsets, barcodes, strands, skip_repeats, factors, tier_hint, true, only_seq, force_min, want_cands, light ? ix : nullptr);
 }
 int t4_add_query_last_cands(t4_ctx *c, const t4_cand **pool, const int32_t **base, const int32_t **cnt, const int32_t **stats8, int *n) {
   if (!c || !c->aqOutHost) return T4_ERR_ARG;
@@ -2398,6 +2590,47 @@
   return T4_OK;
 }
 int t4_add_query_pool_done(t4_ctx *c) { return c ? aqDone(c) : 1; }
+int t4_add_query_light_stats(t4_ctx *c, int64_t *out5) {
+  if (!c || !out5) return T4_ERR_ARG;
+  out5[0] = c->lightRounds; out5[1] = c->lightFallback[2]; out5[2] = c->lightFallback[0]; out5[3] = c->lightFallback[1]; out5[4] = c->lightFallback[3];
+  return T4_OK;
+}
+#ifdef T4_TEST_KNOBS
+int t4_test_light_round(t4_ctx *c, int on, int max_items, int64_t max_bytes) {
+  if (!c) return T4_ERR_ARG;
+  c->lightOff = !on;
+  if (max_items > 0) c->lightMaxItems = max_items;
+  if (max_bytes > 0) c->lightMaxBytes = (size_t)max_bytes;
+  return T4_OK;
+}
+int t4_test_pending_delta(t4_index *ix, int64_t *out3) {
+  if (!ix || !out3) return T4_ERR_ARG;
+  out3[0] = ix->deltaPending ? 1 : 0; out3[1] = (int64_t)ix->deltaNd; out3[2] = (int64_t)ix->deltaBytes;
+  return T4_OK;
+}
+int t4_test_last_header(t4_ctx *c, const void **hdr, int64_t *out5) {
+  if (!c || !hdr || !out5 || !c->aqOutHost) return T4_ERR_ARG;
+  const AqCall &q = c->aq;
+  *hdr = c->aqOutHost;
+  out5[0] = (int64_t)q.outBytes; out5[1] = q.n; out5[2] = (int64_t)q.pBase; out5[3] = (int64_t)q.pCb; out5[4] = (int64_t)q.pTick;
+  return T4_OK;
+}
+int t4_test_read_image(t4_index *ix, void *buf, size_t cap, size_t *bytes, int64_t *sizes5) {
+  if (!ix || !bytes || !ix->live) return T4_ERR_ARG;
+  t4_ctx *c = ix->ctx;
+  { const int rf_ = flushPendingDelta(ix); if (rf_) return rf_; }
+  const size_t b[5] = {sizeof(T4HashEntC) * (size_t)ix->capTable, sizeof(int2) * (size_t)ix->capPost, sizeof(T4SeqInfo) * (size_t)ix->capSeq, (size_t)ix->capBase, (size_t)ix->capBase};
+  const void *src[5] = {ix->dCtab, ix->dPost, ix->dSeqs, ix->dCons, ix->dPw};
+  *bytes = b[0] + b[1] + b[2] + b[3] + b[4];
+  if (sizes5) for (int i = 0; i < 5; ++i) sizes5[i] = (int64_t)b[i];
+  if (!buf) return T4_OK;
+  if (cap < *bytes) return T4_ERR_ARG;
+  HIPCHK(c, hipStreamSynchronize(c->stream));
+  size_t at = 0;
+  for (int i = 0; i < 5; ++i) { if (b[i]) HIPCHK(c, hipMemcpy((unsigned char *)buf + at, src[i], b[i], hipMemcpyDeviceToHost)); at += b[i]; }
+  return T4_OK;
+}
+#endif
 int t4_add_query_pool_end(t4_ctx *c, const int32_t **counts, const int32_t **base, const t4_overlap **ov, const t4_overlap **ext, const int32_t **ext_ret) {
   if (!c || !counts || !base || !ov || !ext || !ext_ret) return T4_ERR_ARG;
   AqResult res;
@@ -2412,6 +2645,7 @@
   if (!ix || n < 0 || max_per_read <= 0 || (n > 0 && (!bases || !offsets || !strands || !factors || !counts || !ov || !ext || !ext_ret))) return T4_ERR_ARG;
   t4_ctx *c = ix->ctx;
   if (!ix->committed) return fail(c, T4_ERR_STATE, "index not committed");
+  { const int rf_ = flushPendingDelta(ix); if (rf_) return rf_; }
   if (ix->view.firstIsRef) return fail(c, T4_ERR_UNSUPPORTED, "t4_add_query needs a contig set");
   if (n == 0) return T4_OK;
   return addQueryImpl(c, ix->view, nullptr, nullptr, false, n, bases, offsets, barcodes, strands, skip_repeats, factors, max_per_read, counts, ov, ext, ext_ret);
diff --git a/trust4_amd/csrc/t4_assembler.cpp b/trust4_amd/csrc/t4_assembler.cpp
--- a/trust4_amd/csrc/t4_assembler.cpp
+++ b/trust4_amd/csrc/t4_assembler.cpp
@@ -791,12 +791,14 @@
   int64_t deltaVersion = 0;
   int64_t launches = 0, launchesUrgent = 0, headWaits = 0, killedInFlight = 0, lightRounds = 0, restrictedOnlyRounds = 0, wholeQueries = 0, restrictedQueries = 0;
   std::vector<float> roundKernelMs, roundWallMs;
+  std::vector<unsigned char> roundRestrictedOnly;
+  bool lastRoundRestrictedOnly = false;
   std::chrono::steady_clock::time_point laneT0;
   double secHeadWait = 0, secLaunch = 0, secHarvest = 0;
   int ensureLanes();
   int flushLive(Lane **out);
   int makeDelta();
-  int bringUpToDate(Lane &L);
+  int bringUpToDate(Lane &L, bool defer = false);
   int launchOn(Lane &L, const std::vector<int> &todo, int repetitive);
   int harvest(Lane &L);
   void abandonJobs();
@@ -1417,6 +1419,22 @@
   d.n_seqs = (int32_t)R.seqId.size(); d.seq_id = R.seqId.data(); d.seq = R.seqRec.data();
   d.n_base_runs = (int64_t)R.baseAt.size(); d.base_at = R.baseAt.data(); d.base_len = R.baseLen.data(); d.base_cons = R.baseCons.data(); d.base_pw = R.basePw.data();
   index.tabRebuilt = false; liveReset = false;
+#ifdef T4_TEST_KNOBS
+  {
+    std::vector<int64_t> sl(R.slot.begin(), R.slot.end());
+    std::sort(sl.begin(), sl.end());
+    bool clash = std::adjacent_find(sl.begin(), sl.end()) != sl.end();
+    std::vector<int> ids(R.seqId.begin(), R.seqId.end());
+    std::sort(ids.begin(), ids.end());
+    clash = clash || std::adjacent_find(ids.begin(), ids.end()) != ids.end();
+    for (size_t i = 1; i < R.postAt.size() && !clash; ++i) clash = (int64_t)R.postAt[i - 1] + R.postLen[i - 1] > (int64_t)R.postAt[i];
+    std::vector<std::pair<int64_t, int64_t>> runs;
+    for (size_t i = 0; i < R.baseAt.size(); ++i) runs.push_back({(int64_t)R.baseAt[i], (int64_t)R.baseLen[i]});
+    std::sort(runs.begin(), runs.end());
+    for (size_t i = 1; i < runs.size() && !clash; ++i) clash = runs[i - 1].first + runs[i - 1].second > runs[i].first;
+    if (clash) { err = "makeDelta: two runs of one delta overlap"; return T4_ERR_STATE; }
+  }
+#endif
   R.version = ++deltaVersion;
   ++deltas; deltaBytes += (int64_t)(R.slot.size() * 16 + R.postData.size() * 4 + R.seqRec.size() * sizeof(t4_seq_record) + R.baseCons.size() * 2);
   deltaLog.push_back(std::move(recp));
@@ -1437,13 +1455,13 @@
   return T4_OK;
 }
 
-int t4_assembler::bringUpToDate(Lane &L) {
+int t4_assembler::bringUpToDate(Lane &L, bool defer) {
   int r;
   if (!L.dev) { if ((r = t4_index_create(L.ctx, k, 0, &L.dev))) return r; }
   if ((r = t4_index_set_params(L.dev, hitLenRequired, radius, novelSim))) return r;
   for (const auto &rec : deltaLog) {
     if (rec->version <= L.version) continue;
-    if ((r = t4_index_apply_delta(L.dev, &rec->d))) return r;
+    if ((r = defer ? t4_index_apply_delta_deferred(L.dev, &rec->d) : t4_index_apply_delta(L.dev, &rec->d))) return r;
     L.version = rec->version;
   }
   int64_t minV = deltaVersion;
@@ -1927,7 +1945,7 @@
   int rc;
   ts.lap(TS_PUMP_OTHER);
   if ((rc = makeDelta())) return rc;
-  { auto t0 = std::chrono::steady_clock::now(); rc = bringUpToDate(L); secDelta += std::chrono::duration<double>(std::chrono::steady_clock::now() - t0).count(); if (rc) return rc; }
+  { auto t0 = std::chrono::steady_clock::now(); rc = bringUpToDate(L, true); secDelta += std::chrono::duration<double>(std::chrono::steady_clock::now() - t0).count(); if (rc) return rc; }
   const int m = (int)todo.size();
   ts.lap(TS_DELTA);
   wideQueries = knobs.wideQueries; wideHitLimit = knobs.wideHitLimit;
@@ -1954,7 +1972,7 @@
   const int mi = (int)L.slots.size();
   bool anyOnlyAll = true;
   for (int v : L.only) if (v < 0) { anyOnlyAll = false; break; }
-  { int nOnly = 0; for (int v : L.only) nOnly += v >= 0 ? 1 : 0; restrictedQueries += nOnly; wholeQueries += mi - nOnly; if (nOnly == mi) ++restrictedOnlyRounds; }
+  { int nOnly = 0; for (int v : L.only) nOnly += v >= 0 ? 1 : 0; restrictedQueries += nOnly; wholeQueries += mi - nOnly; if (nOnly == mi) ++restrictedOnlyRounds; lastRoundRestrictedOnly = nOnly == mi; }
   laneT0 = tl0_;
   if (L.bases.empty()) L.bases.push_back('A');
   ts.lap(TS_LAUNCH_PACK);
@@ -2297,6 +2315,7 @@
     double ms_ = 0; (void)t4_add_query_last_call(L.ctx, &ms_, nullptr, nullptr);
     roundKernelMs.push_back((float)ms_);
     roundWallMs.push_back((float)(std::chrono::duration<double>(std::chrono::steady_clock::now() - laneT0).count() * 1e3));
+    roundRestrictedOnly.push_back(lastRoundRestrictedOnly ? 1 : 0);
   }
   if (rc) {
     if (L.ctx != ctx) err = t4_last_error(L.ctx);
@@ -2796,6 +2815,12 @@
     }
     fprintf(stderr, "timing: query lanes %d: %lld launches (%lld for a head without a result, %lld of them without the whole queries of entries further back), %lld waits for the head's lane in %.3f s, %lld queries killed in flight\n",
             (int)a->lanes.size(), (long long)a->launches, (long long)a->launchesUrgent, (long long)a->lightRounds, (long long)a->headWaits, a->secHeadWait, (long long)a->killedInFlight);
+    {
+      std::vector<float> w, k;
+      for (size_t i = 0; i < a->roundRestrictedOnly.size(); ++i) if (a->roundRestrictedOnly[i]) { w.push_back(a->roundWallMs[i]); k.push_back(a->roundKernelMs[i]); }
+      auto pct = [](std::vector<float> &v, double p) { if (v.empty()) return 0.0; std::sort(v.begin(), v.end()); return (double)v[(size_t)(p * (double)(v.size() - 1))]; };
+      fprintf(stderr, "timing: restricted-only rounds: %zu, wall ms p05 %.4f / p50 %.4f, kernel ms p05 %.4f / p50 %.4f\n", w.size(), pct(w, 0.05), pct(w, 0.5), pct(k, 0.05), pct(k, 0.5));
+    }
     fprintf(stderr, "timing: rounds whose head waited for a WHOLE query: %lld never queried before, fallen to a change of: a key %lld, a list crossing 100 / 10000 postings %lld, a region %lld, a shift %lld, a whole contig %lld, the tolerance budget %lld, a restricted re-query that fell back %lld\n",
             (long long)a->headWholeWhy[0], (long long)a->headWholeWhy[1], (long long)a->headWholeWhy[2], (long long)a->headWholeWhy[3], (long long)a->headWholeWhy[4], (long long)a->headWholeWhy[5], (long long)a->headWholeWhy[6], (long long)a->headWholeWhy[7]);
     fprintf(stderr, "timing: thresholds checked after an edit of a small group by repeating the statistics loop: %lld entries, %lld of them fell (%lld of the checks for reads with lists beyond 10000 postings: removeOnlyRepeats and the head of the hit array as well)\n", (long long)a->toleranceChecks, (long long)a->toleranceCheckKills, (long long)a->fragileChecks);
diff --git a/trust4_amd/csrc/t4_device.h b/trust4_amd/csrc/t4_device.h
--- a/trust4_amd/csrc/t4_device.h
+++ b/trust4_amd/csrc/t4_device.h
@@ -209,4 +209,29 @@
 
 struct T4BytePatch { unsigned char *dst; unsigned long long val; };
 struct T4CopyDesc { unsigned long long srcOff; unsigned char *dst; unsigned long long bytes; };
+
+#ifndef T4_LIGHT_MAX_ITEMS
+#define T4_LIGHT_MAX_ITEMS 64
+#endif
+#ifndef T4_LIGHT_MAX_DELTA_BYTES
+#define T4_LIGHT_MAX_DELTA_BYTES (32 << 10)
+#endif
+#define T4_LIGHT_MAX_DESC 2048
+#define T4_LIGHT_HDR_ARRAYS 11
+#define T4_LIGHT_TAIL_WORDS 16
+struct T4Light {
+  const unsigned char *staging;
+  int nDesc;
+  int n, n2;
+  int wpk, wnm;
+  const unsigned char *hostIn;
+  unsigned char *devIn;
+  unsigned oPk, oNm, oLen, oBc, oSt, oLs, oVw, oFa, oOnly, oForce, oCs, csBytes;
+  unsigned char *devOut, *hostOut;
+  unsigned pTail, outBytes;
+  unsigned *tail;
+  unsigned long long *hostTicks;
+  unsigned *done, *hostFlag;
+  unsigned seq;
+};
 struct T4TableBuild { T4HashEntC *table; unsigned long long tableSlots, srcOff, nKeys; };
diff --git a/trust4_amd/csrc/t4_internal.h b/trust4_amd/csrc/t4_internal.h
--- a/trust4_amd/csrc/t4_internal.h
+++ b/trust4_amd/csrc/t4_internal.h
@@ -39,6 +39,14 @@
 typedef struct { int32_t seqIdx, ss, se; int16_t rs, re, m0, matchCnt, indelCnt; uint16_t flags; } t4_cand;
 int t4_add_query_pool_begin2(t4_index *ix, int n, const char *bases, const int64_t *offsets, const int32_t *barcodes, const int32_t *strands,
                              int skip_repeats, const double *factors, unsigned char *tier_hint, const int32_t *only_seq, const int32_t *force_min, int want_cands);
+int t4_index_apply_delta_deferred(t4_index *ix, const t4_index_delta *delta);
+int t4_add_query_light_stats(t4_ctx *ctx, int64_t *out5);
+#ifdef T4_TEST_KNOBS
+int t4_test_light_round(t4_ctx *ctx, int on, int max_items, int64_t max_bytes);
+int t4_test_pending_delta(t4_index *ix, int64_t *out3);
+int t4_test_last_header(t4_ctx *ctx, const void **hdr, int64_t *out5);
+int t4_test_read_image(t4_index *ix, void *buf, size_t cap, size_t *bytes, int64_t *sizes5);
+#endif
 int t4_add_query_last_cands(t4_ctx *ctx, const t4_cand **pool, const int32_t **base, const int32_t **cnt, const int32_t **stats8, int *n);
 int t4_add_query_last_aux(t4_ctx *ctx, const int32_t **aux, const int32_t **n4, const int32_t **status, int *n);
 int t4_add_query_pool_done(t4_ctx *ctx);
diff --git a/trust4_amd/csrc/t4_kernels.h b/trust4_amd/csrc/t4_kernels.h
--- a/trust4_amd/csrc/t4_kernels.h
+++ b/trust4_amd/csrc/t4_kernels.h
@@ -3909,6 +3909,169 @@
   }
 }
 
+__device__ __forceinline__ unsigned long long lightLoad(const unsigned long long *p) {
+#ifdef __HIPCC__
+  return __hip_atomic_load(p, __ATOMIC_RELAXED, __HIP_MEMORY_SCOPE_AGENT);
+#else
+  return __atomic_load_n(p, __ATOMIC_RELAXED);
+#endif
+}
+__device__ __forceinline__ void lightCopyRun(unsigned char *dst, const unsigned char *src, unsigned long long bytes, int lane) {
+  if ((((unsigned long long)dst | (unsigned long long)src | bytes) & 7ull) == 0) {
+    const unsigned long long n8 = bytes >> 3;
+    unsigned long long *d8 = (unsigned long long *)dst;
+    const unsigned long long *s8 = (const unsigned long long *)src;
+    for (unsigned long long i = lane; i < n8; i += 256) {
+      unsigned long long v[4];
+      for (int u = 0; u < 4; ++u) if (i + 64 * u < n8) v[u] = s8[i + 64 * u];
+      for (int u = 0; u < 4; ++u) if (i + 64 * u < n8) d8[i + 64 * u] = v[u];
+    }
+  } else {
+    for (unsigned long long i = lane; i < bytes; i += 256) {
+      unsigned char v[4];
+      for (int u = 0; u < 4; ++u) if (i + 64 * u < bytes) v[u] = src[i + 64 * u];
+      for (int u = 0; u < 4; ++u) if (i + 64 * u < bytes) dst[i + 64 * u] = v[u];
+    }
+  }
+}
+__global__ __launch_bounds__(512) __attribute__((amdgpu_waves_per_eu(1)))
+void lightQueryKernel(T4IndexView ixArg, T4BatchView bvArg, T4Work wkArg, T4QueryArgs qaArg, T4Light ltArg) {
+  constexpr int C = 8192, M = 512;
+  __shared__ unsigned long long s_keys[C];
+  __shared__ unsigned s_pairs[C + C / 3 + 2];
+  __shared__ OvRec s_ov[M];
+  __shared__ OvRec s_fin[M];
+  __shared__ unsigned short s_ord[M];
+  __shared__ char s_seg[T4_MAXL + 8];
+  __shared__ char s_rc[T4_MAXL + 8];
+  __shared__ WaveState s_ws;
+  __shared__ T4IndexView s_ix;
+  __shared__ T4BatchView s_bv;
+  __shared__ T4Work s_wk;
+  __shared__ T4QueryArgs s_qa;
+  __shared__ WaveMem s_wm;
+  __shared__ T4Light s_lt;
+  __shared__ int s_nLong, s_last;
+  if (threadIdx.x == 0) {
+    s_ix = ixArg; s_bv = bvArg; s_wk = wkArg; s_qa = qaArg; s_lt = ltArg; s_nLong = 0;
+    WaveMem &wm0 = s_wm;
+    wm0.keys = s_keys; wm0.pairs = s_pairs; wm0.cand = s_pairs + C; wm0.ov = s_ov; wm0.fin = s_fin; wm0.ord = s_ord;
+    wm0.cap = C; wm0.maxOv = M; wm0.maxFin = M; wm0.candCap = C / 3 + 2; wm0.ldsArrays = 1;
+    wm0.hitLimit = (wkArg.capLimit > 0 && wkArg.capLimit < C) ? wkArg.capLimit : C;
+    wm0.ldsSort = nullptr; wm0.ldsSortCap = 0;
+    wm0.dirBuf = (unsigned char *)s_keys; wm0.dirBytes = C * 8;
+    wm0.seg = s_seg; wm0.rc = s_rc;
+  }
+  __syncthreads();
+  const T4IndexView &ix = s_ix;
+  const T4BatchView &bv = s_bv;
+  const T4Work &wk = s_wk;
+  const T4QueryArgs &qa = s_qa;
+  const T4Light &lt = s_lt;
+  WaveMem &wm = s_wm;
+  const int t = threadIdx.x, lane = laneId(), nWaves = blockDim.x >> 6;
+  if (lt.nDesc > 0) {
+    const T4CopyDesc *desc = (const T4CopyDesc *)lt.staging;
+    T4CopyDesc *longRuns = (T4CopyDesc *)s_keys;
+    for (int d = t; d < lt.nDesc; d += blockDim.x) {
+      const T4CopyDesc cd = desc[d];
+      const unsigned char *src = lt.staging + cd.srcOff;
+      if (cd.bytes <= 32 && (((unsigned long long)cd.dst | (unsigned long long)src | cd.bytes) & 7ull) == 0) {
+        const int n8 = (int)(cd.bytes >> 3);
+        unsigned long long v[4];
+        for (int u = 0; u < 4; ++u) if (u < n8) v[u] = ((const unsigned long long *)src)[u];
+        for (int u = 0; u < 4; ++u) if (u < n8) ((unsigned long long *)cd.dst)[u] = v[u];
+      } else longRuns[atomicAdd(&s_nLong, 1)] = cd;
+    }
+    __syncthreads();
+    const int nLong = s_nLong;
+    for (int j = t >> 6; j < nLong; j += nWaves) lightCopyRun(longRuns[j].dst, lt.staging + longRuns[j].srcOff, longRuns[j].bytes, lane);
+    __threadfence();
+    __syncthreads();
+  }
+  {
+    int *hdr = (int *)lt.devOut;
+    if (t >= 448 && (unsigned)(t - 448) < lt.csBytes / 4) ((unsigned *)(lt.devIn + lt.oCs))[t - 448] = ((const unsigned *)(lt.hostIn + lt.oCs))[t - 448];
+    for (int w = blockIdx.x; w < lt.n; w += gridDim.x) {
+      int u = t;
+      unsigned off = 0, idx = 0;
+      bool copy = true;
+      if (u < lt.wpk) { off = lt.oPk; idx = (unsigned)(w * lt.wpk + u); }
+      else if ((u -= lt.wpk) < lt.wnm) { off = lt.oNm; idx = (unsigned)(w * lt.wnm + u); }
+      else if ((u -= lt.wnm) < 9) {
+        const unsigned offs[9] = {lt.oLen, lt.oBc, lt.oSt, lt.oLs, lt.oVw, lt.oOnly, lt.oForce, lt.oFa, lt.oFa};
+        off = offs[u]; idx = u < 7 ? (unsigned)w : (unsigned)(2 * w + (u - 7));
+      } else {
+        copy = false;
+        u -= 9;
+        if (u < T4_LIGHT_HDR_ARRAYS + T4_QSTATS) {
+          if (u < T4_LIGHT_HDR_ARRAYS) {
+            hdr[u * lt.n2 + w] = 0;
+            if (w == lt.n - 1 && lt.n2 > lt.n) hdr[u * lt.n2 + lt.n] = 0;
+          } else hdr[T4_LIGHT_HDR_ARRAYS * lt.n2 + T4_QSTATS * w + (u - T4_LIGHT_HDR_ARRAYS)] = 0;
+        }
+      }
+      if (copy) ((unsigned *)(lt.devIn + off))[idx] = ((const unsigned *)(lt.hostIn + off))[idx];
+    }
+    __threadfence();
+    __syncthreads();
+  }
+#ifdef __HIPCC__
+  if (t == 0) atomicMin((unsigned long long *)(lt.tail + 12), (unsigned long long)wall_clock64());
+#endif
+  DPScratch sc;
+  sc.rows = wk.dpRows + ((size_t)blockIdx.x * nWaves + (t >> 6)) * (6 * T4_ROWW * 64);
+  sc.dir = wk.dpDir + ((size_t)blockIdx.x * blockDim.x + t) * T4_DIR_BYTES;
+  for (int w = blockIdx.x; w < lt.n; w += gridDim.x) {
+#ifdef __HIPCC__
+    const unsigned long long tick0 = qa.readTicks ? wall_clock64() : 0ull;
+#endif
+    const bool done = processRead<1>(ix, bv, wk, qa, wm, &s_ws, w, sc);
+    if (t == 0) {
+#ifdef __HIPCC__
+      if (qa.readTicks) qa.readTicks[w] = (int)(wall_clock64() - tick0);
+#endif
+      if (!done) atomicAdd(wk.nextCount, 1);
+    }
+    __syncthreads();
+  }
+  __threadfence_system();
+  __syncthreads();
+  if (t == 0) {
+    const unsigned before = atomicAdd(lt.done, 1u);
+    s_last = before + 1u == gridDim.x ? 1 : 0;
+    if (s_last) {
+      __threadfence();
+#ifdef __HIPCC__
+      asm volatile("s_waitcnt vmcnt(0)" ::: "memory");
+#endif
+    }
+  }
+  __syncthreads();
+  if (!s_last) return;
+  {
+    unsigned long long tEnd = 0;
+#ifdef __HIPCC__
+    if (t == 0) tEnd = (unsigned long long)wall_clock64();
+#endif
+    const unsigned long long *dOut = (const unsigned long long *)lt.devOut, *tail8 = (const unsigned long long *)lt.tail;
+    unsigned long long *hOut = (unsigned long long *)lt.hostOut;
+    const unsigned tailW = lt.pTail >> 3, outW = lt.outBytes >> 3;
+    for (unsigned i = t; i < outW; i += blockDim.x)
+      hOut[i] = i < tailW ? lightLoad(dOut + i) : i < tailW + 6 ? lightLoad(tail8 + (i - tailW)) : 0ull;
+    if (t == 0) { lt.hostTicks[0] = lightLoad(tail8 + 6); lt.hostTicks[1] = tEnd; }
+    __syncthreads();
+    if (t < T4_LIGHT_TAIL_WORDS) lt.tail[t] = (t == 12 || t == 13) ? ~0u : 0u;
+    __threadfence_system();
+    __syncthreads();
+    if (t == 0) {
+      *lt.done = 0u;
+      __threadfence_system();
+      __atomic_store_n(lt.hostFlag, lt.seq, __ATOMIC_RELEASE);
+    }
+  }
+}
+
 __global__ __launch_bounds__(256) void patchKernel(const T4BytePatch *patches, int n) {
   for (int i = blockIdx.x * blockDim.x + threadIdx.x; i < n; i += gridDim.x * blockDim.x) *patches[i].dst = (unsigned char)patches[i].val;
 }
```
